# ParaGroup/WindFlow

Measured on NVIDIA H100. Metric: tuples/sec, Map_GPU->Filter_GPU->Ffat_Windows_GPU (CB win 4096 slide 64) pipeline, higher is better.
Workload: dtype i64+f64

## Files before the change

windflow_b200/csrc/wfb_kernels.cuh:

```cuda
#pragma once
#include <type_traits>
#include <cstdint>
#include <cuda.h>
#include <cuda_runtime.h>
#include "wfb_ptx.cuh"
#include "wfb_keys.cuh"

namespace wfb {

template <class P> using key_codec = KeyCodec<typename P::key_t>;
template <class P> using key_words_t = typename key_codec<P>::words_t;
template <class P>
__host__ __device__ __forceinline__ key_words_t<P> key_words(const typename P::tuple_t &t, const typename P::params_t &prm)
{
    return key_codec<P>::encode(P::key(t, prm));
}

constexpr int TILE = 256;
constexpr uint32_t OSW_TILE_POS = 4096;
#ifndef WFB_STAGES
#define WFB_STAGES 4
#endif
constexpr int STAGES = WFB_STAGES;
constexpr uint32_t FULL = 0xffffffffu;

enum { MODE_MAP = 0, MODE_FILTER = 1, MODE_INGEST = 2 };
constexpr uint32_t MAX_SHARDS = 8;

constexpr uint64_t ST_AGG = 1, ST_PREFIX = 2;
__host__ __device__ __forceinline__ uint64_t pack_state(uint32_t epoch, uint64_t status, uint32_t v)
{
    return (static_cast<uint64_t>(epoch & 0x3fffffffu) << 34) | (status << 32) | v;
}

struct DevBatch {
    const unsigned char *tuples;
    const uint64_t *ts;
    unsigned char *out;
    uint64_t *ts_out;
    uint32_t *n_out;
    uint64_t watermark;
    uint32_t n;
    uint32_t tile_begin;
};

struct Trigger { uint64_t key; uint64_t g; uint32_t slot; uint32_t last_pos; uint32_t obase; uint32_t pad; };

struct FfatDev {
    uint64_t *ht_keys;
    uint32_t *ht_slots;
    uint32_t ht_mask;
    uint32_t max_keys;
    uint32_t *n_slots;
    uint32_t *err_flags;
    unsigned long long *results_total;
    uint64_t defer_items;
    uint32_t dense;
    uint32_t grow;
    uint32_t key_div, key_rem;
    uint64_t *slot_key;
    uint64_t *cnt;
    unsigned char *acc;
    unsigned char *tree;
    uint32_t *seg_cnt;
    uint32_t *seg_off;
    struct Trigger *trig;
    uint32_t *n_trig;
    uint32_t trig_cap;
    uint32_t *heavy;
    uint32_t *n_heavy;
    uint32_t light_max;
    uint64_t win, slide, B;
    uint32_t nb;
    uint32_t pane;
    uint32_t wp, sp;
    uint32_t n_leaves;
    uint32_t log_leaves;
    uint32_t lazy;
};
constexpr uint64_t EMPTY_KEY = 0xffffffffffffffffull;
constexpr uint32_t INVALID_SLOT = 0xffffffffu;
constexpr uint32_t KEYS_GROW_FLAG = 8u;

struct TileArgs {
    const DevBatch *batches;
    DevBatch one;
    uint32_t nbatches;
    uint32_t num_tiles;
    uint64_t *tile_state;
    uint32_t *ticket;
    uint32_t ticket_base;
    uint32_t epoch;
    uint64_t tmap_base;
    uint32_t use_tmap;
    uint32_t max_ctas_per_sm;
    uint32_t sparse;
    uint32_t count_keys;
    uint16_t *wide_h16;
    uint32_t tiles_per_ticket;
    uint32_t pack_rank;
    const uint32_t *ext_slots;
    uint32_t inplace;
    uint32_t l2_hints;
    uint32_t nshards, region_cap;
    uint32_t shard_slots, shard_keys;
    uint32_t *shard_err;
    uint32_t *sort_ctl; uint32_t sort_passes, sort_shift, sort_dbits;
    unsigned char *lifted;
    uint32_t *slots;
    uint32_t *batch_off;
    uint32_t *n_total;
    FfatDev ff;
};

template <class T>
struct TileIO {
    static constexpr int TB = sizeof(T);
    static constexpr bool V16 = (TB % 16 == 0) && (TB / 16 == 1 || TB / 16 == 2 || TB / 16 == 4 || TB / 16 == 8);
    static constexpr int C = V16 ? TB / 16 : TB / 8;

    __device__ __forceinline__ static void load(const unsigned char *base, uint32_t idx, T &out)
    {
        if constexpr (V16) {
            uint4 v[C];
            const uint4 *p = reinterpret_cast<const uint4 *>(base + static_cast<size_t>(idx) * TB);
            const uint32_t rot = (C > 1) ? ((idx * C / 8) % C) : 0;
#pragma unroll
            for (int j = 0; j < C; j++) v[j] = p[(j + rot) & (C - 1)];
#pragma unroll
            for (int s = 1; s < C; s <<= 1) {
                if (rot & s) {
                    uint4 t[C];
#pragma unroll
                    for (int k = 0; k < C; k++) t[k] = v[(k - s) & (C - 1)];
#pragma unroll
                    for (int k = 0; k < C; k++) v[k] = t[k];
                }
            }
            uint4 *o = reinterpret_cast<uint4 *>(&out);
#pragma unroll
            for (int k = 0; k < C; k++) o[k] = v[k];
        } else {
            const uint64_t *p = reinterpret_cast<const uint64_t *>(base + static_cast<size_t>(idx) * TB);
            uint64_t *o = reinterpret_cast<uint64_t *>(&out);
#pragma unroll
            for (int k = 0; k < C; k++) o[k] = p[k];
        }
    }

    __device__ __forceinline__ static void store(unsigned char *base, uint32_t idx, const T &in)
    {
        if constexpr (V16) {
            uint4 v[C];
            const uint4 *src = reinterpret_cast<const uint4 *>(&in);
#pragma unroll
            for (int k = 0; k < C; k++) v[k] = src[k];
            const uint32_t rot = (C > 1) ? ((idx * C / 8) % C) : 0;
#pragma unroll
            for (int s = 1; s < C; s <<= 1) {
                if (rot & s) {
                    uint4 t[C];
#pragma unroll
                    for (int k = 0; k < C; k++) t[k] = v[(k + s) & (C - 1)];
#pragma unroll
                    for (int k = 0; k < C; k++) v[k] = t[k];
                }
            }
            uint4 *p = reinterpret_cast<uint4 *>(base + static_cast<size_t>(idx) * TB);
#pragma unroll
            for (int j = 0; j < C; j++) p[(j + rot) & (C - 1)] = v[j];
        } else {
            uint64_t *p = reinterpret_cast<uint64_t *>(base + static_cast<size_t>(idx) * TB);
            const uint64_t *s = reinterpret_cast<const uint64_t *>(&in);
#pragma unroll
            for (int k = 0; k < C; k++) p[k] = s[k];
        }
    }
};

__device__ __forceinline__ bool bulk_ok(const void *g, uint32_t bytes)
{
    return ((reinterpret_cast<uintptr_t>(g) | bytes) & 15u) == 0;
}

__device__ __forceinline__ uint64_t mix64(uint64_t x)
{
    x ^= x >> 33; x *= 0xff51afd7ed558ccdull; x ^= x >> 33; x *= 0xc4ceb9fe1a85ec53ull; x ^= x >> 33;
    return x;
}

template <class P>
__device__ __forceinline__ key_words_t<P> key_of_slot(const FfatDev &ff, uint32_t slot)
{
    if constexpr (key_codec<P>::words == 2) return reinterpret_cast<const Key128 *>(ff.slot_key)[slot];
    else return ff.dense ? (ff.key_div > 1 ? static_cast<uint64_t>(slot) * ff.key_div + ff.key_rem : static_cast<uint64_t>(slot)) : ff.slot_key[slot];
}
__device__ __forceinline__ uint64_t trig_word(uint64_t key) { return key; }
__device__ __forceinline__ uint64_t trig_word(const Key128 &) { return 0; }
template <class P>
__device__ __forceinline__ key_words_t<P> trig_key(const FfatDev &ff, const Trigger &tr)
{
    if constexpr (key_codec<P>::words == 2) return key_of_slot<P>(ff, tr.slot); else return tr.key;
}

__device__ __forceinline__ uint32_t slot_of_key(const FfatDev &ff, const Key128 &key)
{
    if (key.lo == EMPTY_KEY && key.hi == EMPTY_KEY) { atomicOr(ff.err_flags, 1u); return INVALID_SLOT; }
    uint32_t h = static_cast<uint32_t>(mix64(key.lo ^ mix64(key.hi))) & ff.ht_mask;
    for (uint32_t probe = 0; probe <= ff.ht_mask; probe++) {
        uint64_t *e = ff.ht_keys + 2 * static_cast<size_t>(h);
        Key128 k;
        ld_relaxed_v2u64(e, k.lo, k.hi);
        if (k.lo == EMPTY_KEY || k.hi == EMPTY_KEY) {
            atom_cas_b128(e, EMPTY_KEY, EMPTY_KEY, key.lo, key.hi, k.lo, k.hi);
            if (k.lo == EMPTY_KEY && k.hi == EMPTY_KEY) {
                uint32_t s = atomicAdd(ff.n_slots, 1u);
                if (s < ff.max_keys) reinterpret_cast<Key128 *>(ff.slot_key)[s] = key;
                else if (ff.grow) atomicOr(ff.err_flags, KEYS_GROW_FLAG);
                else { atomicOr(ff.err_flags, 1u); s = INVALID_SLOT - 1; }
                st_release_u32(&ff.ht_slots[h], s);
                return s >= ff.max_keys ? INVALID_SLOT : s;
            }
        }
        if (k == key) {
            uint32_t s;
            while ((s = ld_acquire_u32(&ff.ht_slots[h])) == INVALID_SLOT) { }
            if (s >= ff.max_keys) { if (ff.grow) atomicOr(ff.err_flags, KEYS_GROW_FLAG); return INVALID_SLOT; }
            return s;
        }
        h = (h + 1) & ff.ht_mask;
    }
    atomicOr(ff.err_flags, ff.grow ? KEYS_GROW_FLAG : 1u);
    return INVALID_SLOT;
}

__device__ __forceinline__ uint32_t slot_of_key(const FfatDev &ff, uint64_t key)
{
    if (ff.dense) {
        if (ff.key_div > 1) {
            if (key % ff.key_div != ff.key_rem) { atomicOr(ff.err_flags, 1u); return INVALID_SLOT; }
            key /= ff.key_div;
        }
        if (key >= ff.max_keys) { atomicOr(ff.err_flags, 1u); return INVALID_SLOT; }
        return static_cast<uint32_t>(key);
    }
    if (ff.grow && key == EMPTY_KEY) { atomicOr(ff.err_flags, 1u); return INVALID_SLOT; }
    uint32_t h = static_cast<uint32_t>(mix64(key)) & ff.ht_mask;
    for (uint32_t probe = 0; probe <= ff.ht_mask; probe++) {
        uint64_t k = ld_relaxed_u64(&ff.ht_keys[h]);
        if (k == EMPTY_KEY) {
            unsigned long long old = atomicCAS(reinterpret_cast<unsigned long long *>(&ff.ht_keys[h]),
                                               static_cast<unsigned long long>(EMPTY_KEY),
                                               static_cast<unsigned long long>(key));
            if (old == EMPTY_KEY) {
                uint32_t s = atomicAdd(ff.n_slots, 1u);
                if (s < ff.max_keys) ff.slot_key[s] = key;
                else if (ff.grow) atomicOr(ff.err_flags, KEYS_GROW_FLAG);
                else { atomicOr(ff.err_flags, 1u); s = INVALID_SLOT - 1; }
                st_release_u32(&ff.ht_slots[h], s);
                return s >= ff.max_keys ? INVALID_SLOT : s;
            }
            k = old;
        }
        if (k == key) {
            uint32_t s;
            while ((s = ld_acquire_u32(&ff.ht_slots[h])) == INVALID_SLOT) { }
            if (s >= ff.max_keys) { if (ff.grow) atomicOr(ff.err_flags, KEYS_GROW_FLAG); return INVALID_SLOT; }
            return s;
        }
        h = (h + 1) & ff.ht_mask;
    }
    atomicOr(ff.err_flags, ff.grow ? KEYS_GROW_FLAG : 1u);
    return INVALID_SLOT;
}

static __global__ void __launch_bounds__(256) k_key_table_rebuild(const uint64_t *__restrict__ old_keys, const uint32_t *__restrict__ old_slots,
                                                           uint32_t old_mask, uint64_t *new_keys, uint32_t *__restrict__ new_slots, uint32_t new_mask,
                                                           uint64_t *__restrict__ slot_key, uint32_t old_max_keys, uint32_t words, uint32_t *err_flags)
{
    if (blockIdx.x == 0 && threadIdx.x == 0) atomicAnd(err_flags, ~KEYS_GROW_FLAG);
    for (uint32_t i = blockIdx.x * blockDim.x + threadIdx.x; i <= old_mask; i += gridDim.x * blockDim.x) {
        uint32_t h;
        const uint32_t s = old_slots[i];
        if (words == 2) {
            const Key128 k = reinterpret_cast<const Key128 *>(old_keys)[i];
            if (k.lo == EMPTY_KEY && k.hi == EMPTY_KEY) continue;
            h = static_cast<uint32_t>(mix64(k.lo ^ mix64(k.hi))) & new_mask;
            for (;; h = (h + 1) & new_mask) {
                uint64_t lo, hi;
                atom_cas_b128(new_keys + 2 * static_cast<size_t>(h), EMPTY_KEY, EMPTY_KEY, k.lo, k.hi, lo, hi);
                if (lo == EMPTY_KEY && hi == EMPTY_KEY) break;
            }
            if (s >= old_max_keys) reinterpret_cast<Key128 *>(slot_key)[s] = k;
        } else {
            const uint64_t k = old_keys[i];
            if (k == EMPTY_KEY) continue;
            h = static_cast<uint32_t>(mix64(k)) & new_mask;
            while (atomicCAS(reinterpret_cast<unsigned long long *>(&new_keys[h]), static_cast<unsigned long long>(EMPTY_KEY),
                             static_cast<unsigned long long>(k)) != EMPTY_KEY) h = (h + 1) & new_mask;
            if (s >= old_max_keys) slot_key[s] = k;
        }
        new_slots[h] = s;
    }
}

constexpr uint32_t TP_THREADS = TILE + 64;
constexpr uint32_t TILE_SENTINEL = 0x7fffffffu;
enum { TF_SWZ = 1u, TF_FALLBACK = 2u, TF_TS_SMEM = 4u, TF_WIDE_LAST = 8u };

struct StageMeta {
    uint32_t tile, batch, first, cnt, flags, count;
    uint32_t wide, pad;
};

template <class P, int MODE>
struct TilePassSmem {
    using T = typename P::tuple_t;
    using R = typename P::result_t;
    static constexpr uint32_t rec_bytes = (MODE == MODE_INGEST && sizeof(R) > sizeof(T)) ? sizeof(R) : sizeof(T);
    static constexpr uint32_t tile_bytes = (TILE * rec_bytes + 1023u) & ~1023u;
    static constexpr uint32_t aux_bytes = (MODE == MODE_INGEST) ? TILE * 4u : (MODE == MODE_FILTER ? TILE * 16u : 0u);
    static constexpr uint32_t stage_bytes = tile_bytes + aux_bytes;
    static constexpr uint32_t hist_bytes = (MODE == MODE_INGEST) ? 4u * 256u * 4u : 0u;
    static constexpr uint32_t total = STAGES * stage_bytes + 1024  + 1024  + hist_bytes;
};

__device__ __forceinline__ void mbar_arrive(uint64_t *bar)
{
    asm volatile("mbarrier.arrive.shared::cta.b64 _, [%0];" ::"r"(smem_u32(bar)) : "memory");
}
__device__ __forceinline__ void tma_load_2d(void *smem_dst, const void *tmap, int32_t c0, int32_t c1, uint64_t *bar)
{
    asm volatile("cp.async.bulk.tensor.2d.shared::cluster.global.tile.mbarrier::complete_tx::bytes [%0], [%1, {%3, %4}], [%2];"
                 ::"r"(smem_u32(smem_dst)), "l"(tmap), "r"(smem_u32(bar)), "r"(c0), "r"(c1) : "memory");
}
__device__ __forceinline__ void tma_load_2d_hint(void *smem_dst, const void *tmap, int32_t c0, int32_t c1, uint64_t *bar, uint64_t policy)
{
    asm volatile("cp.async.bulk.tensor.2d.shared::cluster.global.tile.mbarrier::complete_tx::bytes.L2::cache_hint [%0], [%1, {%3, %4}], [%2], %5;"
                 ::"r"(smem_u32(smem_dst)), "l"(tmap), "r"(smem_u32(bar)), "r"(c0), "r"(c1), "l"(policy) : "memory");
}
__device__ __forceinline__ void tma_store_2d(const void *tmap, int32_t c0, int32_t c1, const void *smem_src)
{
    asm volatile("cp.async.bulk.tensor.2d.global.shared::cta.tile.bulk_group [%0, {%2, %3}], [%1];"
                 ::"l"(tmap), "r"(smem_u32(smem_src)), "r"(c0), "r"(c1) : "memory");
}
__device__ __forceinline__ void consumer_bar() { asm volatile("bar.sync 1, %0;" ::"n"(TILE) : "memory"); }

template <class P, int MODE>
__global__ void __launch_bounds__(TP_THREADS) k_tile_pass(const __grid_constant__ CUtensorMap tmap, const TileArgs a,
                                                          const __grid_constant__ typename P::params_t prm)
{
    using T = typename P::tuple_t;
    using R = typename P::result_t;
    using SM = TilePassSmem<P, MODE>;
    constexpr uint32_t TB = sizeof(T);
    constexpr uint32_t RB = sizeof(R);
    static_assert(TB % 8 == 0 && RB % 8 == 0, "records must be multiples of 8 bytes");
    constexpr bool CAN_SWZ = (TB == 64);

    extern __shared__ unsigned char smem_raw[];
    unsigned char *smem = reinterpret_cast<unsigned char *>((reinterpret_cast<uintptr_t>(smem_raw) + 1023) & ~static_cast<uintptr_t>(1023));
    unsigned char *ctl = smem + STAGES * SM::stage_bytes;
    uint64_t *full = reinterpret_cast<uint64_t *>(ctl);
    uint64_t *staged = full + STAGES;
    uint64_t *empty = staged + STAGES;
    StageMeta *meta = reinterpret_cast<StageMeta *>(empty + STAGES);
    uint32_t *warp_tot = reinterpret_cast<uint32_t *>(meta + STAGES);
    uint32_t *s_hist = reinterpret_cast<uint32_t *>(ctl + 1024);

    const uint32_t tid = threadIdx.x, lane = tid & 31, warp = tid >> 5;
    auto stage_buf = [&](uint32_t s) { return smem + s * SM::stage_bytes; };
    auto stage_aux = [&](uint32_t s) { return smem + s * SM::stage_bytes + SM::tile_bytes; };

    if (tid == 0) {
        for (int s = 0; s < STAGES; s++) { mbar_init(&full[s], 1); mbar_init(&staged[s], TILE / 32); mbar_init(&empty[s], 1); }
        mbar_fence_init();
    }
    if constexpr (MODE == MODE_INGEST) { for (uint32_t i = tid; i < 4u * 256u; i += TP_THREADS) s_hist[i] = 0; }
    __syncthreads();

    if (warp == 0) {
        if (lane == 0) {
            const uint64_t pol_first = l2_policy_evict_first();
            DevBatch b = a.one; uint32_t bi = 0, b_end = 0;
            bool have_batch = false;
            const uint32_t tpt = a.tiles_per_ticket ? a.tiles_per_ticket : 1u;
            uint32_t t_next = 0, t_end = 0, claim = 0;
            for (uint32_t it = 0;; it++) {
                const uint32_t s = it % STAGES, par = (it / STAGES) & 1u;
                mbar_wait(&empty[s], par ^ 1u);
                StageMeta &m = meta[s];
                if (t_next == t_end) {
                    claim = atomicAdd(a.ticket, 1u) - a.ticket_base;
                    t_next = claim * tpt;
                    if (claim >= (a.num_tiles + tpt - 1) / tpt) { m.tile = TILE_SENTINEL; mbar_arrive(&full[s]); break; }
                    t_end = min(t_next + tpt, a.num_tiles);
                }
                const uint32_t t = t_next++;
                if (a.batches != nullptr && !(have_batch && t >= b.tile_begin && t < b_end)) {
                    uint32_t lo = 0, hi = a.nbatches - 1;
                    while (lo < hi) { const uint32_t mid = (lo + hi + 1) >> 1; if (a.batches[mid].tile_begin <= t) lo = mid; else hi = mid - 1; }
                    bi = lo; b = a.batches[lo];
                    b_end = (lo + 1 < a.nbatches) ? a.batches[lo + 1].tile_begin : a.num_tiles;
                    have_batch = true;
                }
                const uint32_t first = (t - b.tile_begin) * TILE;
                const uint32_t cnt = min(static_cast<uint32_t>(TILE), b.n - first);
                const unsigned char *src = b.tuples + static_cast<size_t>(first) * TB;
                uint32_t flags = 0, tx = 0;
                const uint64_t off = reinterpret_cast<uint64_t>(src) - a.tmap_base;
                if (CAN_SWZ && a.use_tmap && cnt == TILE && (off & 63u) == 0 && (off >> 6) < 0x7fffff00ull) flags = TF_SWZ;
                else if (!bulk_ok(src, cnt * TB)) flags = TF_FALLBACK;
                if (!(flags & TF_FALLBACK)) tx += cnt * TB;
                const uint64_t *tsp = (MODE == MODE_FILTER && b.ts != nullptr) ? b.ts + first : nullptr;
                if (tsp != nullptr && bulk_ok(tsp, cnt * 8u)) { flags |= TF_TS_SMEM; tx += cnt * 8u; }
                if (t_next == t_end) flags |= TF_WIDE_LAST;
                m.tile = t; m.batch = bi; m.first = first; m.cnt = cnt; m.flags = flags; m.wide = claim;
                if (tx) mbar_expect_tx(&full[s], tx); else mbar_arrive(&full[s]);
                if (a.l2_hints) {
                    if (flags & TF_SWZ) tma_load_2d_hint(stage_buf(s), &tmap, 0, static_cast<int32_t>(off >> 6), &full[s], pol_first);
                    else if (!(flags & TF_FALLBACK)) bulk_g2s_hint(stage_buf(s), src, cnt * TB, &full[s], pol_first);
                } else if (flags & TF_SWZ) tma_load_2d(stage_buf(s), &tmap, 0, static_cast<int32_t>(off >> 6), &full[s]);
                else if (!(flags & TF_FALLBACK)) bulk_g2s(stage_buf(s), src, cnt * TB, &full[s]);
                if (flags & TF_TS_SMEM) bulk_g2s(stage_aux(s), tsp, cnt * 8u, &full[s]);
            }
        }
    } else if (warp <= TILE / 32) {
        const uint32_t ctid = tid - 32, cwarp = warp - 1;
        uint32_t wpar = 0;
        for (uint32_t it = 0;; it++) {
            const uint32_t s = it % STAGES, par = (it / STAGES) & 1u;
            unsigned char *buf = stage_buf(s);
            mbar_wait(&full[s], par);
            const StageMeta m = meta[s];
            if (m.tile == TILE_SENTINEL) {
                __syncwarp();
                if (lane == 0) mbar_arrive(&staged[s]);
                if constexpr (MODE == MODE_INGEST) {
                    if (a.sort_ctl != nullptr) {
                        consumer_bar();
                        for (uint32_t i = ctid; i < (a.sort_passes << a.sort_dbits); i += TILE) { const uint32_t c = s_hist[i]; if (c) atomicAdd(&a.sort_ctl[i], c); }
                    }
                }
                break;
            }
            DevBatch b;
            if (a.batches == nullptr) b = a.one; else b = a.batches[m.batch];
            const uint32_t cnt = m.cnt;
            const bool active = ctid < cnt;
            if (m.flags & TF_FALLBACK) {
                const uint64_t *src = reinterpret_cast<const uint64_t *>(b.tuples + static_cast<size_t>(m.first) * TB);
                uint64_t *dst = reinterpret_cast<uint64_t *>(buf);
                for (uint32_t w = ctid; w < cnt * (TB / 8); w += TILE) dst[w] = src[w];
                consumer_bar();
            }
            alignas(16) T tup;
            uint64_t ts = 0;
            bool keep = false;
            if (active) {
                if constexpr (CAN_SWZ) {
                    if (m.flags & TF_SWZ) {
                        const uint4 *p = reinterpret_cast<const uint4 *>(buf + static_cast<size_t>(ctid) * 64);
                        const uint32_t x = (ctid >> 1) & 3u;
                        uint4 *o = reinterpret_cast<uint4 *>(&tup);
#pragma unroll
                        for (uint32_t jj = 0; jj < 4; jj++) o[jj] = p[jj ^ x];
                    } else TileIO<T>::load(buf, ctid, tup);
                } else TileIO<T>::load(buf, ctid, tup);
                if constexpr (MODE == MODE_FILTER) {
                    if (b.ts != nullptr)
                        ts = (m.flags & TF_TS_SMEM) ? reinterpret_cast<const uint64_t *>(stage_aux(s))[ctid] : b.ts[m.first + ctid];
                }
                P::map(tup, prm);
                keep = (MODE == MODE_MAP) ? true : P::filter(tup, prm);
            }
            uint32_t slot = INVALID_SLOT;
            alignas(16) R res;
            if constexpr (MODE == MODE_INGEST) {
                if (keep) {
                    P::lift(tup, res, prm);
                    if (a.nshards && a.shard_slots) {
                        const uint64_t key = key_word0(key_words<P>(tup, prm)), q = key / a.nshards;
                        if (q < a.shard_keys) slot = static_cast<uint32_t>(key - q * a.nshards) * a.shard_slots + static_cast<uint32_t>(q);
                        else atomicOr(a.shard_err, 2u);
                    } else if (a.nshards) slot = static_cast<uint32_t>(key_word0(key_words<P>(tup, prm)) % a.nshards);
                    else {
                        if (a.ext_slots != nullptr) { slot = a.ext_slots[m.tile * TILE + ctid]; if (slot >= a.ff.max_keys) slot = INVALID_SLOT; }
                        else slot = slot_of_key(a.ff, key_words<P>(tup, prm));
                        if (slot != INVALID_SLOT && a.count_keys) atomicAdd(&a.ff.seg_cnt[slot], 1u);
                    }
                    if (a.wide_h16 != nullptr) {
                        if (slot != INVALID_SLOT) {
                            const uint32_t d = (slot >> a.sort_shift) & 1023u;
                            const uint32_t before = atomicAdd(&s_hist[wpar * 512u + (d >> 1)], 1u << ((d & 1u) * 16u));
                            if (a.pack_rank) slot |= ((before >> ((d & 1u) * 16u)) & 0xffffu) << 16;
                        }
                    } else if (a.sort_ctl != nullptr && !(a.sparse && slot == INVALID_SLOT)) {
                        for (uint32_t ps = 0; ps < a.sort_passes; ps++)
                            atomicAdd(&s_hist[(ps << a.sort_dbits) + ((slot >> (a.sort_shift + a.sort_dbits * ps)) & ((1u << a.sort_dbits) - 1u))], 1u);
                    }
                }
            }
            if constexpr (MODE == MODE_MAP) {
                consumer_bar();
                if (active) {
                    if constexpr (CAN_SWZ) {
                        if (m.flags & TF_SWZ) {
                            uint4 *p = reinterpret_cast<uint4 *>(buf + static_cast<size_t>(ctid) * 64);
                            const uint32_t x = (ctid >> 1) & 3u;
                            const uint4 *o = reinterpret_cast<const uint4 *>(&tup);
#pragma unroll
                            for (uint32_t jj = 0; jj < 4; jj++) p[jj ^ x] = o[jj];
                        } else TileIO<T>::store(buf, ctid, tup);
                    } else TileIO<T>::store(buf, ctid, tup);
                }
                if (ctid == 0) meta[s].count = cnt;
            } else {
                const uint32_t bal = __ballot_sync(FULL, keep);
                uint32_t *wt = warp_tot + (it & 1u) * (TILE / 32);
                if (lane == 0) wt[cwarp] = __popc(bal);
                consumer_bar();
                if constexpr (MODE == MODE_INGEST) {
                    if (a.wide_h16 != nullptr && (m.flags & TF_WIDE_LAST)) {
                        uint32_t *hrow = s_hist + wpar * 512u;
                        const uint2 c = reinterpret_cast<const uint2 *>(hrow)[ctid];
                        reinterpret_cast<uint2 *>(hrow)[ctid] = make_uint2(0, 0);
                        reinterpret_cast<uint2 *>(a.wide_h16 + static_cast<size_t>(m.wide) * 1024u)[ctid] = c;
                        wpar ^= 1u;
                    }
                }
                uint32_t wbase = 0, total = 0;
#pragma unroll
                for (uint32_t w = 0; w < TILE / 32; w++) { const uint32_t c = wt[w]; if (w < cwarp) wbase += c; total += c; }
                const uint32_t local = wbase + __popc(bal & lanemask_lt());
                if (ctid == 0) {
                    meta[s].count = total;
                    const uint32_t chain_begin = (MODE == MODE_FILTER) ? b.tile_begin : 0u;
                    if (m.tile != chain_begin && !(MODE == MODE_INGEST && a.sparse)) st_relaxed_u64(&a.tile_state[m.tile], pack_state(a.epoch, ST_AGG, total));
                }
                if (keep) {
                    if constexpr (MODE == MODE_FILTER) {
                        TileIO<T>::store(buf, local, tup);
                        if (b.ts_out != nullptr) reinterpret_cast<uint64_t *>(stage_aux(s) + TILE * 8)[local] = ts;
                    } else if (MODE == MODE_INGEST && a.inplace) {
                        reinterpret_cast<uint32_t *>(stage_aux(s))[ctid] = slot;
                    } else {
                        TileIO<R>::store(buf, local, res);
                        reinterpret_cast<uint32_t *>(stage_aux(s))[local] = slot;
                    }
                } else if (MODE == MODE_INGEST && a.inplace) reinterpret_cast<uint32_t *>(stage_aux(s))[ctid] = INVALID_SLOT;
            }
            fence_async_smem();
            __syncwarp();
            if (lane == 0) mbar_arrive(&staged[s]);
        }
    } else {
        for (uint32_t it = 0;; it++) {
            const uint32_t s = it % STAGES, par = (it / STAGES) & 1u;
            unsigned char *buf = stage_buf(s);
            mbar_wait(&staged[s], par);
            const StageMeta m = meta[s];
            if (m.tile == TILE_SENTINEL) break;
            DevBatch b;
            if (a.batches == nullptr) b = a.one; else b = a.batches[m.batch];
            const uint32_t t = m.tile, tile_count = m.count;
            uint32_t excl = 0;
            if (MODE == MODE_INGEST && a.sparse) {
                excl = t * TILE;
                if (lane == 0 && t == 0 && a.ff.n_trig != nullptr) { *a.ff.n_trig = 0; *a.ff.n_heavy = 0; }
            } else if constexpr (MODE != MODE_MAP) {
                const uint32_t chain_begin = (MODE == MODE_FILTER) ? b.tile_begin : 0u;
                if (t != chain_begin) {
                    int64_t idx = static_cast<int64_t>(t) - 1;
                    while (true) {
                        const int64_t my = idx - lane;
                        uint64_t w = pack_state(a.epoch, ST_PREFIX, 0);
                        bool valid;
                        do {
                            valid = true;
                            if (my >= static_cast<int64_t>(chain_begin)) {
                                w = ld_relaxed_u64(&a.tile_state[my]);
                                valid = ((w >> 34) == (a.epoch & 0x3fffffffu)) && (((w >> 32) & 3u) != 0);
                            }
                        } while (!__all_sync(FULL, valid));
                        const uint32_t status = static_cast<uint32_t>(w >> 32) & 3u;
                        const uint32_t pmask = __ballot_sync(FULL, status == ST_PREFIX);
                        const uint32_t firstp = pmask ? (__ffs(pmask) - 1) : 32;
                        uint32_t v = (lane <= firstp) ? static_cast<uint32_t>(w) : 0u;
#pragma unroll
                        for (int o = 16; o > 0; o >>= 1) v += __shfl_xor_sync(FULL, v, o);
                        excl += v;
                        if (pmask) break;
                        idx -= 32;
                    }
                }
                if (lane == 0) {
                    st_relaxed_u64(&a.tile_state[t], pack_state(a.epoch, ST_PREFIX, excl + tile_count));
                    if constexpr (MODE == MODE_FILTER) {
                        const uint32_t last_tile = b.tile_begin + (b.n + TILE - 1) / TILE - 1;
                        if (t == last_tile && b.n_out != nullptr) *b.n_out = excl + tile_count;
                    } else {
                        if (t == 0) { *a.ff.n_trig = 0; *a.ff.n_heavy = 0; }
                        if (t == b.tile_begin) a.batch_off[m.batch] = excl;
                        if (t == a.num_tiles - 1) { a.batch_off[a.nbatches] = excl + tile_count; *a.n_total = excl + tile_count; }
                    }
                }
            }
            unsigned char *dst;
            uint32_t bytes;
            if constexpr (MODE == MODE_MAP) { dst = b.out + static_cast<size_t>(m.first) * TB; bytes = m.cnt * TB; }
            else if constexpr (MODE == MODE_FILTER) { dst = b.out + static_cast<size_t>(excl) * TB; bytes = tile_count * TB; }
            else { dst = a.lifted + static_cast<size_t>(excl) * RB; bytes = a.inplace ? 0u : tile_count * RB; }
            if (MODE == MODE_MAP && (m.flags & TF_SWZ)) {
                if (lane == 0) tma_store_2d(&tmap, 0, static_cast<int32_t>((reinterpret_cast<uint64_t>(dst) - a.tmap_base) >> 6), buf);
            } else if (bulk_ok(dst, bytes)) {
                if (lane == 0 && bytes) {
                    if ((MODE == MODE_INGEST) && a.l2_hints) bulk_s2g_hint(dst, buf, bytes, l2_policy_evict_last());
                    else bulk_s2g(dst, buf, bytes);
                }
            } else {
                uint64_t *d8 = reinterpret_cast<uint64_t *>(dst);
                const uint64_t *s8 = reinterpret_cast<const uint64_t *>(buf);
                for (uint32_t w = lane; w < bytes / 8; w += 32) d8[w] = s8[w];
            }
            if constexpr (MODE == MODE_FILTER) {
                if (b.ts_out != nullptr) {
                    const uint64_t *sts = reinterpret_cast<const uint64_t *>(stage_aux(s) + TILE * 8);
                    for (uint32_t i = lane; i < tile_count; i += 32) b.ts_out[excl + i] = sts[i];
                }
            }
            if constexpr (MODE == MODE_INGEST) {
                const uint32_t *ssl = reinterpret_cast<const uint32_t *>(stage_aux(s));
                if (a.sparse) for (uint32_t i = lane; i < TILE; i += 32) a.slots[excl + i] = i < (a.inplace ? m.cnt : tile_count) ? ssl[i] : INVALID_SLOT;
                else for (uint32_t i = lane; i < tile_count; i += 32) a.slots[excl + i] = ssl[i];
            }
            __syncwarp();
            if (lane == 0) {
                bulk_commit();
                bulk_wait_read<0>();
                mbar_arrive(&empty[s]);
            }
        }
        if (lane == 0) bulk_wait_all<0>();
    }
}

template <class R>
__device__ __forceinline__ void ld_rec(const unsigned char *p, R &r)
{
    if constexpr (sizeof(R) % 16 == 0) {
        const uint4 *s = reinterpret_cast<const uint4 *>(p);
        uint4 *d = reinterpret_cast<uint4 *>(&r);
#pragma unroll
        for (uint32_t k = 0; k < sizeof(R) / 16; k++) d[k] = s[k];
    } else {
        const uint64_t *s = reinterpret_cast<const uint64_t *>(p);
        uint64_t *d = reinterpret_cast<uint64_t *>(&r);
#pragma unroll
        for (uint32_t k = 0; k < sizeof(R) / 8; k++) d[k] = s[k];
    }
}
template <class R>
__device__ __forceinline__ void st_rec(unsigned char *p, const R &r)
{
    if constexpr (sizeof(R) % 16 == 0) {
        uint4 *d = reinterpret_cast<uint4 *>(p);
        const uint4 *s = reinterpret_cast<const uint4 *>(&r);
#pragma unroll
        for (uint32_t k = 0; k < sizeof(R) / 16; k++) d[k] = s[k];
    } else {
        uint64_t *d = reinterpret_cast<uint64_t *>(p);
        const uint64_t *s = reinterpret_cast<const uint64_t *>(&r);
#pragma unroll
        for (uint32_t k = 0; k < sizeof(R) / 8; k++) d[k] = s[k];
    }
}
template <class R>
__device__ __forceinline__ R shfl_down_rec(const R &r, uint32_t delta)
{
    alignas(16) R o;
    const uint32_t *s = reinterpret_cast<const uint32_t *>(&r);
    uint32_t *d = reinterpret_cast<uint32_t *>(&o);
#pragma unroll
    for (uint32_t k = 0; k < sizeof(R) / 4; k++) d[k] = __shfl_down_sync(FULL, s[k], delta);
    return o;
}
template <class R>
__device__ __forceinline__ R shfl_rec(const R &r, uint32_t src)
{
    alignas(16) R o;
    const uint32_t *s = reinterpret_cast<const uint32_t *>(&r);
    uint32_t *d = reinterpret_cast<uint32_t *>(&o);
#pragma unroll
    for (uint32_t k = 0; k < sizeof(R) / 4; k++) d[k] = __shfl_sync(FULL, s[k], src);
    return o;
}

static __global__ void __launch_bounds__(1024) k_scan_u32(const uint32_t *in, uint32_t *out, uint32_t total, uint32_t *sum_out)
{
    __shared__ uint32_t warp_sums[32];
    const uint32_t tid = threadIdx.x, lane = tid & 31, warp = tid >> 5;
    const uint32_t per = (total + 1023) / 1024;
    const uint32_t begin = min(tid * per, total), end = min(begin + per, total);
    uint32_t sum = 0;
    for (uint32_t i = begin; i < end; i++) sum += in[i];
    uint32_t incl = sum;
#pragma unroll
    for (int o = 1; o < 32; o <<= 1) { const uint32_t v = __shfl_up_sync(FULL, incl, o); if (lane >= o) incl += v; }
    if (lane == 31) warp_sums[warp] = incl;
    __syncthreads();
    if (warp == 0) {
        uint32_t w = warp_sums[lane], wi = w;
#pragma unroll
        for (int o = 1; o < 32; o <<= 1) { const uint32_t v = __shfl_up_sync(FULL, wi, o); if (lane >= o) wi += v; }
        warp_sums[lane] = wi - w;
        if (lane == 31 && sum_out != nullptr) *sum_out = wi;
    }
    __syncthreads();
    uint32_t run = warp_sums[warp] + incl - sum;
    for (uint32_t i = begin; i < end; i++) { const uint32_t v = in[i]; out[i] = run; run += v; }
}


constexpr int OS_THREADS = 256;
constexpr int OS_MAX_PASSES = 8;
constexpr int OS_ITEMS = 8;

template <class K>
__global__ void __launch_bounds__(256) k_radix_ghist(const K *__restrict__ keys, const uint32_t *__restrict__ n_ptr, uint32_t n_host,
                                                     uint32_t passes, uint32_t *__restrict__ ctl, uint32_t base_shift)
{
    __shared__ uint32_t h[OS_MAX_PASSES * 256];
    const uint32_t n = n_ptr ? *n_ptr : n_host;
    for (uint32_t i = threadIdx.x; i < passes * 256; i += blockDim.x) h[i] = 0;
    __syncthreads();
    for (uint32_t i = blockIdx.x * blockDim.x + threadIdx.x; i < n; i += gridDim.x * blockDim.x) {
        const K k = keys[i];
        for (uint32_t p = 0; p < passes; p++) atomicAdd(&h[p * 256 + (static_cast<uint32_t>(k >> (base_shift + 8 * p)) & 255u)], 1u);
    }
    __syncthreads();
    for (uint32_t i = threadIdx.x; i < passes * 256; i += blockDim.x) if (h[i]) atomicAdd(&ctl[i], h[i]);
}

template <class K>
__global__ void __launch_bounds__(OS_THREADS) k_onesweep_pass(const K *__restrict__ keys_in, const uint32_t *__restrict__ vals_in,
                                                              K *__restrict__ keys_out, uint32_t *__restrict__ vals_out,
                                                              const uint32_t *__restrict__ n_ptr, uint32_t n_host, uint32_t pass,
                                                              uint32_t passes, uint32_t *__restrict__ ctl,
                                                              uint64_t *__restrict__ tile_state, uint32_t epoch,
                                                              uint32_t *__restrict__ seg_first, uint32_t seg_first_n,
                                                              uint32_t base_shift)
{
    __shared__ uint32_t cntw[OS_THREADS / 32][256];
    __shared__ uint32_t dig_off[256];
    __shared__ uint32_t bin_base[256];
    __shared__ uint32_t wsum[OS_THREADS / 32];
    __shared__ uint32_t s_tile;
    constexpr int OS_TILE = OS_THREADS * OS_ITEMS;
    __shared__ K skeys[OS_TILE];
    __shared__ uint32_t svals[OS_TILE];

    const uint32_t tid = threadIdx.x, lane = tid & 31, warp = tid >> 5;
    const uint32_t n = n_ptr ? *n_ptr : n_host;
    const uint32_t num_tiles = (n + OS_TILE - 1) / OS_TILE;
    const uint32_t shift = base_shift + 8 * pass;
    if (tid == 0) s_tile = atomicAdd(&ctl[passes * 256 + pass], 1u);
#pragma unroll
    for (int w = 0; w < OS_THREADS / 32; w++) cntw[w][tid] = 0;
    __syncthreads();
    const uint32_t tile = s_tile;
    if (tile >= num_tiles) return;
    const uint32_t start = tile * OS_TILE;

    K k[OS_ITEMS];
    uint32_t rk[OS_ITEMS];
#pragma unroll
    for (int r = 0; r < OS_ITEMS; r++) {
        const uint32_t idx = start + warp * (32 * OS_ITEMS) + r * 32 + lane;
        const bool valid = idx < n;
        k[r] = valid ? keys_in[idx] : K(0);
        const uint32_t d = valid ? (static_cast<uint32_t>(k[r] >> shift) & 255u) : 256u;
        const uint32_t mask = __match_any_sync(FULL, d);
        rk[r] = valid ? (cntw[warp][d] + __popc(mask & lanemask_lt())) : 0u;
        __syncwarp();
        if (valid && lane == static_cast<uint32_t>(__ffs(mask) - 1)) cntw[warp][d] += __popc(mask);
        __syncwarp();
    }
    __syncthreads();

    uint32_t total = 0;
#pragma unroll
    for (int w = 0; w < OS_THREADS / 32; w++) { const uint32_t c = cntw[w][tid]; cntw[w][tid] = total; total += c; }
    uint64_t *my_state = tile_state + static_cast<size_t>(tile) * 256 + tid;
    st_relaxed_u64(my_state, pack_state(epoch, tile == 0 ? ST_PREFIX : ST_AGG, total));
    const uint32_t gcount = ctl[pass * 256 + tid];
    uint32_t incl = gcount;
#pragma unroll
    for (int o = 1; o < 32; o <<= 1) { const uint32_t v = __shfl_up_sync(FULL, incl, o); if (lane >= o) incl += v; }
    if (lane == 31) wsum[warp] = incl;
    uint32_t tincl = total;
#pragma unroll
    for (int o = 1; o < 32; o <<= 1) { const uint32_t v = __shfl_up_sync(FULL, tincl, o); if (lane >= o) tincl += v; }
    __shared__ uint32_t twsum[OS_THREADS / 32];
    if (lane == 31) twsum[warp] = tincl;
    __syncthreads();
    uint32_t gbase = incl - gcount, tbase = tincl - total;
#pragma unroll
    for (uint32_t w = 0; w < OS_THREADS / 32; w++) if (w < warp) { gbase += wsum[w]; tbase += twsum[w]; }
    uint32_t excl = 0;
    if (tile > 0) {
        int64_t t2 = static_cast<int64_t>(tile) - 1;
        bool found = false;
        while (!found) {
            uint64_t w[8];
#pragma unroll
            for (int q = 0; q < 8; q++) w[q] = (t2 - q >= 0) ? ld_relaxed_u64(tile_state + static_cast<size_t>(t2 - q) * 256 + tid) : 0ull;
#pragma unroll
            for (int q = 0; q < 8; q++) {
                if (found || t2 - q < 0) continue;
                if ((w[q] >> 34) != (epoch & 0x3fffffffu) || ((w[q] >> 32) & 3u) == 0) { t2 -= q; goto next_round; }
                excl += static_cast<uint32_t>(w[q]);
                if (((w[q] >> 32) & 3u) == ST_PREFIX) found = true;
            }
            t2 -= 8;
        next_round:;
        }
        st_relaxed_u64(my_state, pack_state(epoch, ST_PREFIX, excl + total));
    }
    dig_off[tid] = tbase;
    bin_base[tid] = gbase + excl;
    __syncthreads();

#pragma unroll
    for (int r = 0; r < OS_ITEMS; r++) {
        const uint32_t idx = start + warp * (32 * OS_ITEMS) + r * 32 + lane;
        if (idx < n) {
            const uint32_t d = static_cast<uint32_t>(k[r] >> shift) & 255u;
            const uint32_t lp = dig_off[d] + cntw[warp][d] + rk[r];
            skeys[lp] = k[r];
            svals[lp] = vals_in ? vals_in[idx] : idx;
        }
    }
    __syncthreads();
    const uint32_t cnt = min(static_cast<uint32_t>(OS_TILE), n - start);
    for (uint32_t i = tid; i < cnt; i += OS_THREADS) {
        const K kk = skeys[i];
        const uint32_t d = static_cast<uint32_t>(kk >> shift) & 255u;
        const uint32_t dst = bin_base[d] + (i - dig_off[d]);
        keys_out[dst] = kk;
        vals_out[dst] = svals[i];
        if (seg_first != nullptr && static_cast<uint64_t>(kk) < seg_first_n) atomicMin(&seg_first[static_cast<uint32_t>(kk)], dst);
    }
}

template <class P>
__global__ void __launch_bounds__(256) k_slots_inplace(const TileArgs a, const typename P::params_t prm)
{
    using T = typename P::tuple_t;
    __shared__ uint32_t s_h[512];
    const uint32_t tid = threadIdx.x;
    const uint32_t npos = a.num_tiles * TILE;
    if (blockIdx.x == 0 && tid == 0 && a.ff.n_trig != nullptr) { *a.ff.n_trig = 0; *a.ff.n_heavy = 0; }
    auto slot_at = [&](uint32_t p) -> uint32_t {
        const uint32_t t = p / TILE;
        uint32_t lo = 0, hi = a.nbatches - 1;
        while (lo < hi) { const uint32_t mid = (lo + hi + 1) >> 1; if (a.batches[mid].tile_begin <= t) lo = mid; else hi = mid - 1; }
        const DevBatch &b = a.batches[lo];
        const uint32_t local = p - b.tile_begin * TILE;
        uint32_t slot = INVALID_SLOT;
        if (local < b.n) {
            if (a.ext_slots != nullptr) { slot = a.ext_slots[p]; if (slot >= a.ff.max_keys) slot = INVALID_SLOT; }
            else {
                const T *rec = reinterpret_cast<const T *>(b.tuples + static_cast<size_t>(local) * sizeof(T));
                slot = slot_of_key(a.ff, key_words<P>(*rec, prm));
            }
            if (slot != INVALID_SLOT && a.count_keys) atomicAdd(&a.ff.seg_cnt[slot], 1u);
        }
        return slot;
    };
    const uint32_t nwide = (npos + OSW_TILE_POS - 1) / OSW_TILE_POS;
    for (uint32_t wt = blockIdx.x; wt < nwide; wt += gridDim.x) {
        for (uint32_t i = tid; i < 512; i += blockDim.x) s_h[i] = 0;
        __syncthreads();
        for (uint32_t p = wt * OSW_TILE_POS + tid; p < min(npos, (wt + 1) * OSW_TILE_POS); p += blockDim.x) {
            uint32_t slot = slot_at(p);
            if (slot != INVALID_SLOT) {
                const uint32_t d = (slot >> a.sort_shift) & 1023u;
                const uint32_t before = atomicAdd(&s_h[d >> 1], 1u << ((d & 1u) * 16u));
                if (a.pack_rank) slot |= ((before >> ((d & 1u) * 16u)) & 0xffffu) << 16;
            }
            a.slots[p] = slot;
        }
        __syncthreads();
        for (uint32_t i = tid; i < 512; i += blockDim.x) reinterpret_cast<uint32_t *>(a.wide_h16 + static_cast<size_t>(wt) * 1024u)[i] = s_h[i];
        __syncthreads();
    }
}

#ifndef WFB_OSW_MINBLOCKS
#define WFB_OSW_MINBLOCKS 5
#endif
constexpr uint32_t OSW_BITS = 10, OSW_DIGITS = 1u << OSW_BITS;
constexpr uint32_t OSW_THREADS = 256, OSW_ITEMS = 16, OSW_TILE = OSW_THREADS * OSW_ITEMS;
static_assert(OSW_TILE == OSW_TILE_POS, "the tile pass files its digit counts per wide tile");

template <class K>
__global__ void __launch_bounds__(OSW_THREADS) k_wide_tile_hist(const K *__restrict__ keys, const uint32_t *__restrict__ n_ptr, uint32_t n_host,
                                                                uint32_t shift, uint32_t chunk_shift, uint16_t *__restrict__ H,
                                                                uint32_t *__restrict__ C, uint32_t *__restrict__ ctl_counts, uint32_t skip_invalid)
{
    static_assert(OSW_THREADS * 4 == OSW_DIGITS, "four digits per thread");
    __shared__ __align__(16) uint32_t h[OSW_DIGITS];
    const uint32_t tid = threadIdx.x, tile = blockIdx.x;
    const uint32_t n = n_ptr ? *n_ptr : n_host;
    const uint32_t start = tile * OSW_TILE;
    if (start >= n) return;
    reinterpret_cast<uint4 *>(h)[tid] = make_uint4(0, 0, 0, 0);
    __syncthreads();
#pragma unroll
    for (uint32_t r = 0; r < OSW_ITEMS; r++) {
        const uint32_t idx = start + r * OSW_THREADS + tid;
        if (idx < n) { const K kk = keys[idx]; if (!(skip_invalid && kk == static_cast<K>(~K(0)))) atomicAdd(&h[static_cast<uint32_t>(kk >> shift) & (OSW_DIGITS - 1u)], 1u); }
    }
    __syncthreads();
    const uint4 c = reinterpret_cast<const uint4 *>(h)[tid];
    reinterpret_cast<ushort4 *>(H + static_cast<size_t>(tile) * OSW_DIGITS)[tid] =
        make_ushort4(static_cast<uint16_t>(c.x), static_cast<uint16_t>(c.y), static_cast<uint16_t>(c.z), static_cast<uint16_t>(c.w));
    uint32_t *crow = C + static_cast<size_t>(tile >> chunk_shift) * OSW_DIGITS + tid * 4;
    if (c.x) atomicAdd(crow + 0, c.x);
    if (c.y) atomicAdd(crow + 1, c.y);
    if (c.z) atomicAdd(crow + 2, c.z);
    if (c.w) atomicAdd(crow + 3, c.w);
    if (ctl_counts != nullptr) {
        if (c.x) atomicAdd(ctl_counts + tid * 4 + 0, c.x);
        if (c.y) atomicAdd(ctl_counts + tid * 4 + 1, c.y);
        if (c.z) atomicAdd(ctl_counts + tid * 4 + 2, c.z);
        if (c.w) atomicAdd(ctl_counts + tid * 4 + 3, c.w);
    }
}

static __global__ void __launch_bounds__(OSW_THREADS) k_wide_chunk_sums16(const uint16_t *__restrict__ H, uint32_t tiles, uint32_t chunk_shift, uint32_t *__restrict__ C,
                                                                          uint32_t *__restrict__ ctl_counts = nullptr)
{
    const uint32_t chunk = blockIdx.x, tid = threadIdx.x;
    const uint32_t t0 = chunk << chunk_shift, t1 = min(tiles, t0 + (1u << chunk_shift));
    uint4 acc = make_uint4(0, 0, 0, 0);
    const ushort4 *row = reinterpret_cast<const ushort4 *>(H) + tid;
#pragma unroll 16
    for (uint32_t t = t0; t < t1; t++) { const ushort4 v = row[static_cast<size_t>(t) * (OSW_DIGITS / 4)]; acc.x += v.x; acc.y += v.y; acc.z += v.z; acc.w += v.w; }
    reinterpret_cast<uint4 *>(C + static_cast<size_t>(chunk) * OSW_DIGITS)[tid] = acc;
    if (ctl_counts != nullptr) {
        if (acc.x) atomicAdd(ctl_counts + tid * 4 + 0, acc.x);
        if (acc.y) atomicAdd(ctl_counts + tid * 4 + 1, acc.y);
        if (acc.z) atomicAdd(ctl_counts + tid * 4 + 2, acc.z);
        if (acc.w) atomicAdd(ctl_counts + tid * 4 + 3, acc.w);
    }
}

static __global__ void __launch_bounds__(OSW_THREADS) k_wide_tile_bases(const uint16_t *__restrict__ H, uint32_t tiles, uint32_t chunk_shift, uint32_t chunks,
                                                                        uint32_t *__restrict__ C, uint32_t *__restrict__ T, uint32_t *__restrict__ ctl_counts,
                                                                        uint32_t *__restrict__ done)
{
    static_assert(OSW_THREADS * 4 == OSW_DIGITS, "four digits per thread");
    constexpr uint32_t NW = OSW_THREADS / 32;
    __shared__ uint32_t wsum[NW];
    __shared__ uint32_t s_last;
    const uint32_t chunk = blockIdx.x, tid = threadIdx.x, lane = tid & 31, warp = tid >> 5;
    const uint32_t t0 = chunk << chunk_shift, t1 = min(tiles, t0 + (1u << chunk_shift));
    uint4 acc = make_uint4(0, 0, 0, 0);
    const ushort4 *row = reinterpret_cast<const ushort4 *>(H) + tid;
    uint4 *trow = reinterpret_cast<uint4 *>(T) + tid;
#pragma unroll 8
    for (uint32_t t = t0; t < t1; t++) {
        const ushort4 v = row[static_cast<size_t>(t) * (OSW_DIGITS / 4)];
        trow[static_cast<size_t>(t) * (OSW_DIGITS / 4)] = acc;
        acc.x += v.x; acc.y += v.y; acc.z += v.z; acc.w += v.w;
    }
    uint4 *C4 = reinterpret_cast<uint4 *>(C);
    C4[static_cast<size_t>(chunk) * (OSW_DIGITS / 4) + tid] = acc;
    __threadfence();
    __syncthreads();
    if (tid == 0) s_last = atomicAdd(done, 1u) == chunks - 1u;
    __syncthreads();
    if (!s_last) return;
    __threadfence();
    uint4 tot = make_uint4(0, 0, 0, 0);
#pragma unroll 8
    for (uint32_t c = 0; c < chunks; c++) { const uint4 v = __ldcg(C4 + static_cast<size_t>(c) * (OSW_DIGITS / 4) + tid); tot.x += v.x; tot.y += v.y; tot.z += v.z; tot.w += v.w; }
    reinterpret_cast<uint4 *>(ctl_counts)[tid] = tot;
    const uint32_t sum = tot.x + tot.y + tot.z + tot.w;
    uint32_t incl = sum;
#pragma unroll
    for (int o = 1; o < 32; o <<= 1) { const uint32_t v = __shfl_up_sync(FULL, incl, o); if (lane >= static_cast<uint32_t>(o)) incl += v; }
    if (lane == 31) wsum[warp] = incl;
    __syncthreads();
    uint32_t base = incl - sum;
#pragma unroll
    for (uint32_t q = 0; q < NW; q++) if (q < warp) base += wsum[q];
    uint4 run = make_uint4(base, base + tot.x, base + tot.x + tot.y, base + tot.x + tot.y + tot.z);
#pragma unroll 8
    for (uint32_t c = 0; c < chunks; c++) {
        uint4 *p = C4 + static_cast<size_t>(c) * (OSW_DIGITS / 4) + tid;
        const uint4 v = __ldcg(p);
        *p = run;
        run.x += v.x; run.y += v.y; run.z += v.z; run.w += v.w;
    }
    if (tid == 0) *done = 0;
}

#ifndef WFB_OSR_MINBLOCKS
#define WFB_OSR_MINBLOCKS 6
#endif
template <int RBYTES>
static __global__ void __launch_bounds__(OSW_THREADS, WFB_OSR_MINBLOCKS) k_wide_scatter_ranked(const uint32_t *__restrict__ packed, uint32_t *__restrict__ keys_out,
                                                                            uint32_t *__restrict__ vals_out, uint32_t n, uint32_t shift, uint32_t chunk_shift,
                                                                            const uint16_t *__restrict__ H, const uint32_t *__restrict__ Cx, const uint32_t *__restrict__ T,
                                                                            const unsigned char *__restrict__ payload_in, unsigned char *__restrict__ payload_out)
{
    constexpr uint32_t NW = OSW_THREADS / 32;
    constexpr uint32_t LPOS = OSW_TILE + OSW_DIGITS;
    constexpr uint32_t LPAD = 0x0fffu;
    static_assert(OSW_TILE <= 4096 && LPOS % (2 * OSW_THREADS) == 0, "16-bit packed position compare");
    __shared__ __align__(16) uint32_t sw[OSW_TILE];
    __shared__ __align__(16) uint32_t bin_base[OSW_DIGITS];
    __shared__ __align__(8) uint16_t cnt_row[OSW_DIGITS], cell_start[OSW_DIGITS];
    __shared__ __align__(4) uint16_t lpos[LPOS];
    __shared__ uint32_t wsum[NW];
    const uint32_t tid = threadIdx.x, lane = tid & 31, warp = tid >> 5, tile = blockIdx.x;
    const uint32_t start = tile * OSW_TILE;
    if (start >= n) return;
#pragma unroll
    for (uint32_t r = 0; r < OSW_ITEMS; r++) {
        const uint32_t i = r * OSW_THREADS + tid, idx = start + i;
        const uint32_t w = idx < n ? packed[idx] : INVALID_SLOT;
        sw[i] = w;
        if constexpr (RBYTES != 0)
            if (w != INVALID_SLOT) asm volatile("prefetch.global.L2 [%0];" ::"l"(payload_in + static_cast<size_t>(idx) * RBYTES));
    }
    {
        const uint4 cb = reinterpret_cast<const uint4 *>(Cx)[static_cast<size_t>(tile >> chunk_shift) * (OSW_DIGITS / 4) + tid];
        const uint4 tb = reinterpret_cast<const uint4 *>(T)[static_cast<size_t>(tile) * (OSW_DIGITS / 4) + tid];
        reinterpret_cast<uint4 *>(bin_base)[tid] = make_uint4(cb.x + tb.x, cb.y + tb.y, cb.z + tb.z, cb.w + tb.w);
        const ushort4 c = reinterpret_cast<const ushort4 *>(H)[static_cast<size_t>(tile) * (OSW_DIGITS / 4) + tid];
        reinterpret_cast<ushort4 *>(cnt_row)[tid] = c;
        const uint32_t p0 = (c.x + 1u) & ~1u, p1 = (c.y + 1u) & ~1u, p2 = (c.z + 1u) & ~1u, p3 = (c.w + 1u) & ~1u;
        const uint32_t sum = p0 + p1 + p2 + p3;
        uint32_t incl = sum;
#pragma unroll
        for (int o = 1; o < 32; o <<= 1) { const uint32_t v = __shfl_up_sync(FULL, incl, o); if (lane >= static_cast<uint32_t>(o)) incl += v; }
        if (lane == 31) wsum[warp] = incl;
#pragma unroll
        for (uint32_t i = 0; i < LPOS / (2 * OSW_THREADS); i++) reinterpret_cast<uint32_t *>(lpos)[i * OSW_THREADS + tid] = LPAD | (LPAD << 16);
        __syncthreads();
        uint32_t base = incl - sum;
#pragma unroll
        for (uint32_t q = 0; q < NW; q++) if (q < warp) base += wsum[q];
        reinterpret_cast<ushort4 *>(cell_start)[tid] = make_ushort4(static_cast<uint16_t>(base), static_cast<uint16_t>(base + p0), static_cast<uint16_t>(base + p0 + p1),
                                                                     static_cast<uint16_t>(base + p0 + p1 + p2));
    }
    __syncthreads();
#pragma unroll
    for (uint32_t r = 0; r < OSW_ITEMS; r++) {
        const uint32_t i = r * OSW_THREADS + tid, w = sw[i];
        if (w != INVALID_SLOT) lpos[cell_start[((w & 0xffffu) >> shift) & (OSW_DIGITS - 1u)] + (w >> 16)] = static_cast<uint16_t>(i);
    }
    __syncthreads();
#pragma unroll 2
    for (uint32_t e = tid; e < LPOS; e += OSW_THREADS) {
        const uint32_t mine = lpos[e], w = sw[mine];
        if (w == INVALID_SLOT) continue;
        const uint32_t slot = w & 0xffffu, d = (slot >> shift) & (OSW_DIGITS - 1u);
        const uint32_t cs = cell_start[d], cnt = cnt_row[d];
        if (e - cs >= cnt) continue;
        const uint32_t mm = (mine | (mine << 16)) + 0x7fff7fffu;
        const uint32_t *cell = reinterpret_cast<const uint32_t *>(lpos + cs);
        uint32_t less = 0;
        for (uint32_t j = 0; j < cnt; j += 2) less += __popc((mm - cell[j >> 1]) & 0x80008000u);
        const uint32_t dst = bin_base[d] + less;
        keys_out[dst] = slot;
        if (RBYTES == 0 || vals_out != nullptr) vals_out[dst] = start + mine;
        if constexpr (RBYTES != 0) {
            static_assert(RBYTES % 8 == 0, "record size");
            using W = typename std::conditional<RBYTES % 16 == 0, uint4, uint2>::type;
            const W *src = reinterpret_cast<const W *>(payload_in + static_cast<size_t>(start + mine) * RBYTES);
            W *dstp = reinterpret_cast<W *>(payload_out + static_cast<size_t>(dst) * RBYTES);
            W v[RBYTES / sizeof(W)];
#pragma unroll
            for (uint32_t q = 0; q < RBYTES / sizeof(W); q++) v[q] = src[q];
#pragma unroll
            for (uint32_t q = 0; q < RBYTES / sizeof(W); q++) dstp[q] = v[q];
        }
    }
}

static __global__ void k_shard_bin_counts(const uint32_t *__restrict__ bin_counts, uint32_t nshards, uint32_t bps, uint32_t *__restrict__ counts_out,
                                          uint64_t *__restrict__ send_meta, uint64_t watermark)
{
    const uint32_t d = threadIdx.x >> 5, lane = threadIdx.x & 31;
    uint32_t c = 0;
    if (d < nshards) for (uint32_t b = lane; b < bps; b += 32) c += bin_counts[d * bps + b];
#pragma unroll
    for (int o = 16; o > 0; o >>= 1) c += __shfl_xor_sync(FULL, c, o);
    if (lane == 0 && d < MAX_SHARDS) counts_out[d] = d < nshards ? c : 0u;
    if (lane == 0 && d < nshards && send_meta != nullptr) { send_meta[2 * d] = c; send_meta[2 * d + 1] = watermark; }
}

struct MgRuns { uint32_t off[MAX_SHARDS + 1]; };
constexpr uint32_t MG_THREADS = 256;
__device__ __forceinline__ uint32_t mg_run_start(const uint32_t *__restrict__ cnt, uint32_t s, uint32_t bps, uint32_t b, uint32_t *sh)
{
    uint32_t c = 0;
    for (uint32_t q = threadIdx.x; q < b; q += MG_THREADS) c += cnt[s * bps + q];
#pragma unroll
    for (int o = 16; o > 0; o >>= 1) c += __shfl_xor_sync(FULL, c, o);
    if ((threadIdx.x & 31) == 0) sh[threadIdx.x >> 5] = c;
    __syncthreads();
    uint32_t t = 0;
#pragma unroll
    for (uint32_t w = 0; w < MG_THREADS / 32; w++) t += sh[w];
    __syncthreads();
    return t;
}
static __global__ void __launch_bounds__(MG_THREADS) k_mg_count(const uint32_t *__restrict__ cnt, uint32_t nsrc, uint32_t bps, const MgRuns runs,
                                                                const uint32_t *__restrict__ recv_slots, uint32_t slot_mask, uint32_t shift2, uint32_t nsub,
                                                                uint32_t *__restrict__ cnt3, uint32_t *__restrict__ run_starts,
                                                                uint32_t *__restrict__ n_trig, uint32_t *__restrict__ n_heavy)
{
    __shared__ uint32_t sh[8], c[MAX_SHARDS];
    const uint32_t b = blockIdx.x, s = blockIdx.y, tid = threadIdx.x, lane = tid & 31;
    if (b == 0 && s == 0 && tid == 0) { *n_trig = 0; *n_heavy = 0; }
    if (tid < MAX_SHARDS) c[tid] = 0;
    const uint32_t rs = mg_run_start(cnt, s, bps, b, sh), m = cnt[s * bps + b];
    if (tid == 0) run_starts[s * bps + b] = rs;
    const uint32_t *sl = recv_slots + runs.off[s] + rs;
    for (uint32_t i0 = 0; i0 < m; i0 += MG_THREADS) {
        const uint32_t i = i0 + tid;
        const uint32_t j = i < m ? ((sl[i] & slot_mask) >> shift2) & (nsub - 1u) : nsub;
        for (uint32_t jj = 0; jj < nsub; jj++) { const uint32_t bal = __ballot_sync(FULL, j == jj); if (lane == 0 && bal) atomicAdd(&c[jj], __popc(bal)); }
    }
    __syncthreads();
    if (tid < nsub) cnt3[(b * nsub + tid) * nsrc + s] = c[tid];
}
static __global__ void __launch_bounds__(1024) k_mg_scan(const uint32_t *__restrict__ cnt3, uint32_t n, uint32_t nsrc, uint32_t *__restrict__ off3,
                                                         uint32_t *__restrict__ digit_counts)
{
    __shared__ uint32_t wsum[32];
    const uint32_t tid = threadIdx.x, lane = tid & 31, warp = tid >> 5;
    const uint32_t per = (n + 1023u) / 1024u, lo = tid * per;
    uint32_t v[MAX_SHARDS], sum = 0;
#pragma unroll
    for (uint32_t q = 0; q < MAX_SHARDS; q++) { v[q] = (q < per && lo + q < n) ? cnt3[lo + q] : 0u; sum += v[q]; }
    uint32_t incl = sum;
#pragma unroll
    for (int o = 1; o < 32; o <<= 1) { const uint32_t x = __shfl_up_sync(FULL, incl, o); if (lane >= static_cast<uint32_t>(o)) incl += x; }
    if (lane == 31) wsum[warp] = incl;
    __syncthreads();
    if (warp == 0) {
        uint32_t w = wsum[lane], wi = w;
#pragma unroll
        for (int o = 1; o < 32; o <<= 1) { const uint32_t x = __shfl_up_sync(FULL, wi, o); if (lane >= static_cast<uint32_t>(o)) wi += x; }
        wsum[lane] = wi - w;
    }
    __syncthreads();
    uint32_t run = wsum[warp] + incl - sum;
#pragma unroll
    for (uint32_t q = 0; q < MAX_SHARDS; q++) if (q < per && lo + q < n) { off3[lo + q] = run; run += v[q]; }
    for (uint32_t d = tid; d * nsrc < n; d += 1024) { uint32_t t = 0; for (uint32_t q = 0; q < nsrc; q++) t += cnt3[d * nsrc + q]; digit_counts[d] = t; }
}
static __global__ void __launch_bounds__(MG_THREADS) k_mg_split(const uint32_t *__restrict__ cnt, uint32_t nsrc, uint32_t bps, const MgRuns runs,
                                                                const uint32_t *__restrict__ recv_slots, uint32_t slot_mask, uint32_t shift2, uint32_t nsub,
                                                                const uint32_t *__restrict__ off3, const uint32_t *__restrict__ run_starts,
                                                                uint32_t *__restrict__ out_slots, uint32_t *__restrict__ out_pos)
{
    __shared__ uint32_t wc[MG_THREADS / 32][MAX_SHARDS], fill[MAX_SHARDS];
    const uint32_t b = blockIdx.x, s = blockIdx.y, tid = threadIdx.x, lane = tid & 31, warp = tid >> 5;
    const uint32_t m = cnt[s * bps + b], src0 = runs.off[s] + run_starts[s * bps + b];
    if (tid < nsub) fill[tid] = off3[(b * nsub + tid) * nsrc + s];
    __syncthreads();
    for (uint32_t i0 = 0; i0 < m; i0 += MG_THREADS) {
        const uint32_t i = i0 + tid;
        uint32_t slot = 0, j = nsub, before = 0;
        if (i < m) { slot = recv_slots[src0 + i] & slot_mask; j = (slot >> shift2) & (nsub - 1u); }
        for (uint32_t jj = 0; jj < nsub; jj++) {
            const uint32_t bal = __ballot_sync(FULL, j == jj);
            if (lane == 0) wc[warp][jj] = __popc(bal);
            if (j == jj) before = __popc(bal & lanemask_lt());
        }
        __syncthreads();
        if (i < m) {
            uint32_t dst = fill[j] + before;
            for (uint32_t w = 0; w < warp; w++) dst += wc[w][j];
            out_slots[dst] = slot; out_pos[dst] = src0 + i;
        }
        __syncthreads();
        if (tid < nsub) { uint32_t t = 0; for (uint32_t w = 0; w < MG_THREADS / 32; w++) t += wc[w][tid]; fill[tid] += t; }
        __syncthreads();
    }
}

template <class K, int RBYTES>
__global__ void __launch_bounds__(OSW_THREADS, WFB_OSW_MINBLOCKS) k_wide_scatter(const K *__restrict__ keys_in, K *__restrict__ keys_out, uint32_t *__restrict__ vals_out,
                                                              const uint32_t *__restrict__ n_ptr, uint32_t n_host, uint32_t shift,
                                                              uint32_t chunk_shift, const uint16_t *__restrict__ H, const uint32_t *__restrict__ C,
                                                              const uint32_t *__restrict__ ctl_counts,
                                                              const unsigned char *__restrict__ payload_in, unsigned char *__restrict__ payload_out,
                                                              uint32_t payload_bytes, uint32_t skip_invalid, uint32_t region_stride)
{
    constexpr uint32_t NW = OSW_THREADS / 32;
    __shared__ __align__(16) uint16_t cntw[NW][OSW_DIGITS];
    __shared__ uint32_t bin_base[OSW_DIGITS];
    __shared__ uint32_t wsum[NW];
    const uint32_t tid = threadIdx.x, lane = tid & 31, warp = tid >> 5, tile = blockIdx.x;
    const uint32_t n = n_ptr ? *n_ptr : n_host;
    const uint32_t start = tile * OSW_TILE;
    if (start >= n) return;
    {
        uint4 *z = reinterpret_cast<uint4 *>(&cntw[0][0]);
        for (uint32_t i = tid; i < NW * OSW_DIGITS / 8; i += OSW_THREADS) z[i] = make_uint4(0, 0, 0, 0);
    }
    uint32_t acc[4] = {0, 0, 0, 0};
    {
        const uint32_t chunk = tile >> chunk_shift;
        const uint4 *crow = reinterpret_cast<const uint4 *>(C) + tid;
#pragma unroll 8
        for (uint32_t c = 0; c < chunk; c++) { const uint4 v = crow[static_cast<size_t>(c) * (OSW_DIGITS / 4)]; acc[0] += v.x; acc[1] += v.y; acc[2] += v.z; acc[3] += v.w; }
        const ushort4 *hrow = reinterpret_cast<const ushort4 *>(H) + tid;
#pragma unroll 16
        for (uint32_t t = chunk << chunk_shift; t < tile; t++) { const ushort4 v = hrow[static_cast<size_t>(t) * (OSW_DIGITS / 4)]; acc[0] += v.x; acc[1] += v.y; acc[2] += v.z; acc[3] += v.w; }
    }
    const uint4 g4 = reinterpret_cast<const uint4 *>(ctl_counts)[tid];
    const uint32_t gsum = g4.x + g4.y + g4.z + g4.w;
// ... 176 lines not shown
        for (; i < n; i += stride) dst[i] = src[i];
    }
    {
        const uint32_t *src = a.slot_src[peer]; uint32_t *dst = a.slot_dst[peer]; const uint32_t n = a.slot_n[peer];
        for (uint32_t i = t; i < n; i += stride) dst[i] = src[i];
    }
    if (part == 0) for (uint32_t i = threadIdx.x; i < a.bin_n; i += MG_PUSH_THREADS) a.bin_dst[peer][i] = a.bin_src[peer][i];
}

static __global__ void k_shard_counts(const uint32_t *__restrict__ digit_counts, uint32_t nshards, uint32_t region_cap, uint32_t *__restrict__ counts_out)
{
    const uint32_t d = threadIdx.x;
    const uint32_t c = d < nshards ? digit_counts[d] : 0u;
    if (d < MAX_SHARDS) counts_out[d] = c;
    const uint32_t over = __ballot_sync(FULL, c > region_cap);
    if (d == 0) counts_out[MAX_SHARDS] = over ? 1u : 0u;
}


__device__ __forceinline__ uint32_t level_off(uint32_t n_leaves, uint32_t level);
__device__ __forceinline__ uint64_t batch_watermark(const uint32_t *__restrict__ batch_off, const DevBatch *__restrict__ batches,
                                                    uint32_t nbatches, uint32_t pos);
template <class P>
__device__ __forceinline__ void ffat_eval_window(const FfatDev &ff, const unsigned char *tree, key_words_t<P> key, uint64_t gwid, uint64_t wm,
                                                 uint32_t opos, unsigned char *__restrict__ out_res, uint64_t *__restrict__ out_ts,
                                                 uint32_t out_cap, const typename P::params_t &prm);

template <class P>
__global__ void __launch_bounds__(128) k_ffat_update_lanes(const FfatDev ff, const unsigned char *__restrict__ lifted,
                                                           const uint32_t *__restrict__ sorted_pos,
                                                           const uint32_t *__restrict__ batch_off, const DevBatch *__restrict__ batches,
                                                           uint32_t nbatches, unsigned char *__restrict__ out_res,
                                                           uint64_t *__restrict__ out_ts, uint32_t out_cap, uint32_t *__restrict__ n_out,
                                                           const typename P::params_t prm)
{
    using R = typename P::result_t;
    constexpr uint32_t RB = sizeof(R);
    constexpr uint32_t U = 4;
    const uint32_t nslots = ff.dense ? ff.max_keys : min(*ff.n_slots, ff.max_keys);
    const uint32_t n = ff.n_leaves, logn = ff.log_leaves;
    const uint64_t P_ = ff.pane;
    const uint64_t group_items = ff.slide * ff.nb;
    const size_t tree_stride = static_cast<size_t>(2 * n - 1) * RB;

    for (uint32_t base = blockIdx.x * blockDim.x; base < nslots; base += gridDim.x * blockDim.x) {
        const uint32_t slot = base + threadIdx.x;
        uint32_t m = (slot < nslots) ? ff.seg_cnt[slot] : 0u;
        if (m > ff.light_max) {
            const uint32_t hi = atomicAdd(ff.n_heavy, 1u);
            if (hi < ff.max_keys) ff.heavy[hi] = slot;
            m = 0;
        }
        const bool act = m > 0;
        uint32_t off = 0; uint64_t c = 0, g = 0, trig = 0;
        key_words_t<P> key{};
        alignas(16) R acc;
        unsigned char *tree = ff.tree + static_cast<size_t>(slot) * tree_stride;
        if (act) {
            off = ff.seg_off[slot]; c = ff.cnt[slot];
            key = key_of_slot<P>(ff, slot);
            if (c % P_ != 0) ld_rec<R>(ff.acc + static_cast<size_t>(slot) * RB, acc);
            g = (c < ff.B) ? 0 : 1 + (c - ff.B) / group_items;
            trig = ff.B + g * group_items;
        }
        uint32_t j = 0;
        while (__any_sync(FULL, act && j < m)) {
            bool completed = false;
            while (act && j < m && !completed) {
                uint32_t p[U];
                alignas(16) R it[U];
                const uint32_t k = min(U, m - j);
#pragma unroll
                for (uint32_t q = 0; q < U; q++) if (q < k) p[q] = sorted_pos[off + j + q];
#pragma unroll
                for (uint32_t q = 0; q < U; q++) if (q < k) ld_rec<R>(lifted + static_cast<size_t>(p[q]) * RB, it[q]);
#pragma unroll
                for (uint32_t q = 0; q < U; q++) {
                    if (q < k && !completed) {
                        if (c % P_ == 0) acc = it[q]; else P::comb(acc, it[q], acc, prm);
                        c++; j++;
                        completed = (c % P_ == 0);
                    }
                }
            }
            if (completed) {
                const uint32_t leaf = static_cast<uint32_t>((c / P_ - 1) & (n - 1));
                const uint32_t plev = ff.lazy ? 0u : logn;
                for (uint32_t l = 0; l < plev; l++)
                    asm volatile("prefetch.global.L2 [%0];" ::"l"(tree + static_cast<size_t>(level_off(n, l) + ((leaf >> l) ^ 1u)) * RB));
                alignas(16) R cur = acc;
                st_rec<R>(tree + static_cast<size_t>(leaf) * RB, cur);
                for (uint32_t l = 0; l < plev; l++) {
                    alignas(16) R s;
                    ld_rec<R>(tree + static_cast<size_t>(level_off(n, l) + ((leaf >> l) ^ 1u)) * RB, s);
                    alignas(16) R parent = cur;
                    if ((leaf >> l) & 1u) P::comb(s, cur, parent, prm); else P::comb(cur, s, parent, prm);
                    cur = parent;
                    st_rec<R>(tree + static_cast<size_t>(level_off(n, l + 1) + (leaf >> (l + 1))) * RB, cur);
                }
                if (c == trig) {
                    const uint32_t last_pos = sorted_pos[off + j - 1];
                    const uint32_t obase = atomicAdd(n_out, ff.nb);
                    bool deferred = (m - j) < ff.defer_items;
                    if (deferred) {
                        const uint32_t ti = atomicAdd(ff.n_trig, 1u);
                        if (ti < ff.trig_cap) { Trigger tr; tr.key = trig_word(key); tr.g = g; tr.slot = slot; tr.last_pos = last_pos; tr.obase = obase; tr.pad = 0; ff.trig[ti] = tr; }
                        else deferred = false;
                    }
                    if (!deferred) {
                        const uint64_t wm = batch_watermark(batch_off, batches, nbatches, last_pos);
                        for (uint32_t i = 0; i < ff.nb; i++)
                            ffat_eval_window<P>(ff, tree, key, g * ff.nb + i, wm, obase + i, out_res, out_ts, out_cap, prm);
                    }
                    g++; trig += group_items;
                }
            }
        }
        if (act) {
            ff.cnt[slot] = c;
            if (c % P_ != 0) st_rec<R>(ff.acc + static_cast<size_t>(slot) * RB, acc);
            ff.seg_cnt[slot] = 0;
            ff.seg_off[slot] = 0xffffffffu;
        }
    }
}

#ifdef WFB_BK_TRACE
__device__ unsigned long long g_bk_trace[1024 * 8];
__device__ __forceinline__ unsigned long long bk_now() { unsigned long long t; asm volatile("mov.u64 %0, %%globaltimer;" : "=l"(t)); return t; }
#define BK_TRACE_STATE unsigned long long bk_t = 0
#define BK_MARK(i) do { if (threadIdx.x == 0) { const unsigned long long t_ = bk_now(); unsigned long long *r_ = g_bk_trace + blockIdx.x * 8; \
    if ((i) == 0) { r_[0] = t_; for (int q_ = 1; q_ < 8; q_++) r_[q_] = 0; } else if ((i) == 7) r_[7] = t_; else r_[i] += t_ - bk_t; bk_t = t_; } } while (0)
#else
#define BK_TRACE_STATE do { } while (0)
#define BK_MARK(i) do { } while (0)
#endif
constexpr uint32_t BK_KEYS = 64;
constexpr uint32_t BK_THREADS = 128;
#ifndef WFB_BK_REC_BYTES
#define WFB_BK_REC_BYTES 16384
#endif
constexpr uint32_t BK_REC_BYTES = WFB_BK_REC_BYTES;
constexpr uint32_t BK_CNT_U = 16;
__device__ __forceinline__ uint32_t bk_opaque(uint32_t v) { asm volatile("" : "+r"(v)); return v; }
template <uint32_t RB>
constexpr uint32_t bk_items_per_thread() { return BK_REC_BYTES / (BK_THREADS * RB) < 1 ? 1 : (BK_REC_BYTES / (BK_THREADS * RB) > 8 ? 8 : BK_REC_BYTES / (BK_THREADS * RB)); }
#ifndef WFB_BK_MINBLOCKS
#define WFB_BK_MINBLOCKS 4
#endif
#ifndef WFB_BK_MINBLOCKS_LAZY
#define WFB_BK_MINBLOCKS_LAZY 4
#endif

template <class P, bool LAZY>
__global__ void __launch_bounds__(BK_THREADS, LAZY ? WFB_BK_MINBLOCKS_LAZY : WFB_BK_MINBLOCKS) k_ffat_update_buckets(const FfatDev ff, const unsigned char *__restrict__ lifted,
                                                                       const uint32_t *__restrict__ bk_slots, const uint32_t *__restrict__ bk_pos,
                                                                       const uint32_t *__restrict__ digit_counts, uint32_t shift, uint32_t moved,
                                                                       const uint32_t *__restrict__ batch_off, const DevBatch *__restrict__ batches,
                                                                       uint32_t nbatches, unsigned char *__restrict__ out_res,
                                                                       uint64_t *__restrict__ out_ts, uint32_t out_cap, uint32_t *__restrict__ n_out,
                                                                       const typename P::params_t prm)
{
    using R = typename P::result_t;
    constexpr uint32_t RB = sizeof(R);
    constexpr uint32_t NW = BK_THREADS / 32;
    constexpr uint32_t DPT = OSW_DIGITS / BK_THREADS;
    constexpr uint32_t IT = bk_items_per_thread<RB>();
    constexpr uint32_t CAP = BK_THREADS * IT;
    constexpr uint32_t NCOL = IT * NW;
    constexpr uint32_t CS = NCOL + 2;
    constexpr uint32_t CPB = (RB % 16 == 0) ? 16 : 8;
    constexpr uint32_t BK_SIBL = RB <= 32 ? 8 : (RB <= 48 ? 4 : (RB <= 128 ? 2 : 1));
    static_assert(DPT % 4 == 0 && BK_KEYS == 64 && BK_THREADS == 128 && RB % 8 == 0, "layout");
    __shared__ __align__(16) unsigned char s_rec[CAP * RB];
    __shared__ uint32_t s_idx[CAP];
    __shared__ uint32_t s_lslot[CAP], s_lpos[CAP];
    __shared__ __align__(16) uint16_t s_col[BK_KEYS][CS];
    __shared__ uint32_t kcnt[BK_KEYS], koff[BK_KEYS];
    __shared__ uint32_t kleft[BK_KEYS];
    __shared__ uint32_t kcp[BK_KEYS], kleaf[BK_KEYS];
    __shared__ uint64_t kc[BK_KEYS], kg[BK_KEYS], ktt[BK_KEYS];
    __shared__ __align__(16) unsigned char kacc[BK_KEYS * RB];
    __shared__ __align__(16) unsigned char s_sib[LAZY ? 16 : BK_KEYS * BK_SIBL * RB];
    __shared__ uint32_t s_heavy[BK_KEYS];
    __shared__ uint32_t ksegb[BK_KEYS];
    __shared__ uint32_t seg_desc[BK_THREADS];
    __shared__ uint32_t misc[NW], s_boff[2], s_nheavy, s_hnext, s_nseg;

    const uint32_t tid = threadIdx.x, lane = tid & 31, warp = tid >> 5;
    const uint32_t bucket = blockIdx.x;
    const uint32_t kpc = min(BK_KEYS, 1u << shift);
    const uint32_t key_lo = bucket << shift;
    const uint32_t n = ff.n_leaves, logn = ff.log_leaves;
    const uint32_t P32 = static_cast<uint32_t>(ff.pane);
    const uint64_t group_items = ff.slide * ff.nb;
    const size_t tree_stride = static_cast<size_t>(2 * n - 1) * RB;
    BK_TRACE_STATE;

    BK_MARK(0);
    uint32_t my_total = 0;
    uint64_t st_c = 0;
    const bool has_key = tid < kpc && key_lo + tid < ff.max_keys;
    if (has_key) {
        const uint32_t slot = key_lo + tid;
        st_c = ff.cnt[slot];
#pragma unroll
        for (uint32_t q = 0; q < RB / CPB; q++) cp_async<CPB>(kacc + tid * RB + q * CPB, ff.acc + static_cast<size_t>(slot) * RB + q * CPB);
    }
    if (tid < BK_KEYS) kleft[tid] = 0;
    {
        uint32_t cc[DPT];
#pragma unroll
        for (uint32_t q = 0; q < DPT / 4; q++) {
            const uint4 v = reinterpret_cast<const uint4 *>(digit_counts)[tid * (DPT / 4) + q];
            cc[4 * q] = v.x; cc[4 * q + 1] = v.y; cc[4 * q + 2] = v.z; cc[4 * q + 3] = v.w;
        }
        uint32_t sum = 0;
#pragma unroll
        for (uint32_t q = 0; q < DPT; q++) sum += cc[q];
        uint32_t incl = sum;
#pragma unroll
        for (int o = 1; o < 32; o <<= 1) { const uint32_t v = __shfl_up_sync(FULL, incl, o); if (lane >= static_cast<uint32_t>(o)) incl += v; }
        if (lane == 31) misc[warp] = incl;
        __syncthreads();
        if (tid == bucket / DPT) {
            uint32_t base = incl - sum;
            for (uint32_t w = 0; w < warp; w++) base += misc[w];
            for (uint32_t q = bucket - bucket % DPT; q < bucket; q++) base += digit_counts[q];
            s_boff[0] = base; s_boff[1] = base + digit_counts[bucket];
        }
        __syncthreads();
    }
    const uint32_t bbeg = s_boff[0], bend = s_boff[1];
    const auto fetch_list = [&](uint32_t at, uint32_t end) {
#pragma unroll
        for (uint32_t r = 0; r < IT; r++) {
            const uint32_t i = r * BK_THREADS + tid;
            if (at + i < end) {
                cp_async<4>(s_lslot + i, bk_slots + at + i);
                if (!moved) cp_async<4>(s_lpos + i, bk_pos + at + i);
            }
        }
    };
    fetch_list(bbeg, bend);
    for (uint32_t base = bbeg; base < bend; base += BK_CNT_U * BK_THREADS) {
        uint32_t lk[BK_CNT_U];
#pragma unroll
        for (uint32_t q = 0; q < BK_CNT_U; q++) {
            const uint32_t i = base + q * BK_THREADS + tid;
            lk[q] = i < bend ? bk_slots[i] - key_lo : 0xffffffffu;
        }
#pragma unroll
        for (uint32_t q = 0; q < BK_CNT_U; q++) if (lk[q] < kpc) atomicAdd(&kleft[lk[q]], 1u);
    }
    __syncthreads();
    if (tid < BK_KEYS) {
        const uint32_t m = has_key ? kleft[tid] : 0u;
        my_total = m;
        const uint64_t c = st_c;
        uint64_t g = 0, tt = 0; uint32_t cp = 0, leaf = 0;
        if (m) {
            cp = static_cast<uint32_t>(c % P32); leaf = static_cast<uint32_t>((c / P32) & (n - 1));
            if (c < ff.B) { g = 0; tt = ff.B - c; }
            else { g = 1 + (c - ff.B) / group_items; tt = ff.B + g * group_items - c; }
        }
        kleft[tid] = m; kc[tid] = c; kg[tid] = g; ktt[tid] = tt; kcp[tid] = cp; kleaf[tid] = leaf;
    }
    const uint32_t any_items = __syncthreads_or(my_total != 0);
    BK_MARK(1);
    if (!any_items) { cp_async_wait_all(); BK_MARK(7); return; }
    if (moved)
        for (size_t o = static_cast<size_t>(tid) * 128; o < static_cast<size_t>(bend - bbeg) * RB; o += BK_THREADS * 128)
            asm volatile("prefetch.global.L2 [%0];" ::"l"(lifted + static_cast<size_t>(bbeg) * RB + o));

    for (uint32_t cursor = s_boff[0]; cursor < s_boff[1]; cursor = s_boff[0]) {
        const uint32_t nsel = min(CAP, s_boff[1] - cursor);
        uint32_t ek[IT], ep[IT];
        cp_async_wait_all();
#pragma unroll
        for (uint32_t r = 0; r < IT; r++) {
            const uint32_t i = r * BK_THREADS + tid;
            ek[r] = BK_KEYS; ep[r] = cursor + i;
            if (i < nsel) {
                const uint32_t lk = s_lslot[i] - key_lo;
                if (!moved) ep[r] = s_lpos[i];
                if (lk < kpc) ek[r] = lk;
            }
        }
        {
            uint32_t *z = reinterpret_cast<uint32_t *>(&s_col[0][0]);
            for (uint32_t i = tid; i < BK_KEYS * CS / 2; i += BK_THREADS) z[i] = 0;
        }
        __syncthreads();
        fetch_list(cursor + CAP, s_boff[1]);
#pragma unroll
        for (uint32_t r = 0; r < IT; r++) {
            const uint32_t k = ek[r];
            const uint32_t peers = __match_any_sync(FULL, k);
            const uint32_t rank = __popc(peers & lanemask_lt());
            if (k < BK_KEYS && rank == 0) s_col[k][r * NW + warp] = static_cast<uint16_t>(__popc(peers));
            ek[r] = k | rank << 8;
        }
        __syncthreads();
        BK_MARK(2);
        if (warp == 0) {
            uint32_t a0 = 0, a1 = 0;
#pragma unroll
            for (uint32_t c = 0; c < NCOL; c++) {
                const uint32_t v0 = s_col[lane][c], v1 = s_col[lane + 32][c];
                s_col[lane][c] = static_cast<uint16_t>(a0); s_col[lane + 32][c] = static_cast<uint16_t>(a1);
                a0 += v0; a1 += v1;
            }
            uint32_t i0 = a0, i1 = a1;
#pragma unroll
            for (int o = 1; o < 32; o <<= 1) {
                const uint32_t v0 = __shfl_up_sync(FULL, i0, o), v1 = __shfl_up_sync(FULL, i1, o);
                if (lane >= static_cast<uint32_t>(o)) { i0 += v0; i1 += v1; }
            }
            const uint32_t t0 = __shfl_sync(FULL, i0, 31);
            kcnt[lane] = a0; kcnt[lane + 32] = a1;
            koff[lane] = i0 - a0; koff[lane + 32] = t0 + i1 - a1;
            const uint32_t c0 = kcp[lane], c1 = kcp[lane + 32];
            const uint32_t f0 = min(a0, P32 - c0), f1 = min(a1, P32 - c1);
            const uint32_t n0 = a0 ? 1u + (a0 - f0 + P32 - 1) / P32 : 0u, n1 = a1 ? 1u + (a1 - f1 + P32 - 1) / P32 : 0u;
            uint32_t s0 = n0, s1 = n1;
#pragma unroll
            for (int o = 1; o < 32; o <<= 1) {
                const uint32_t v0 = __shfl_up_sync(FULL, s0, o), v1 = __shfl_up_sync(FULL, s1, o);
                if (lane >= static_cast<uint32_t>(o)) { s0 += v0; s1 += v1; }
            }
            const uint32_t st0 = __shfl_sync(FULL, s0, 31), nseg = st0 + __shfl_sync(FULL, s1, 31);
            ksegb[lane] = s0 - n0; ksegb[lane + 32] = st0 + s1 - n1;
            const bool fallback = nseg > BK_THREADS;
            const bool h0 = fallback && a0 != 0, h1 = fallback && a1 != 0;
            const uint32_t b0 = __ballot_sync(FULL, h0), b1 = __ballot_sync(FULL, h1);
            if (h0) s_heavy[__popc(b0 & lanemask_lt())] = lane;
            if (h1) s_heavy[__popc(b0) + __popc(b1 & lanemask_lt())] = lane + 32;
            if (lane == 0) { s_nheavy = __popc(b0) + __popc(b1); s_hnext = 0; s_nseg = fallback ? 0u : nseg; }
        }
        __syncthreads();
#pragma unroll
        for (uint32_t r = 0; r < IT; r++) {
            const uint32_t k = ek[r] & 255u;
            if (k < BK_KEYS) {
                const uint32_t at = koff[k] + s_col[k][r * NW + warp] + (ek[r] >> 8);
                s_idx[at] = ep[r];
                const unsigned char *src = lifted + static_cast<size_t>(ep[r]) * RB;
#pragma unroll
                for (uint32_t q = 0; q < RB / CPB; q++) {
                    if constexpr (CPB == 16) cp_async_cg16(s_rec + at * RB + q * CPB, src + q * CPB);
                    else cp_async<CPB>(s_rec + at * RB + q * CPB, src + q * CPB);
                }
            }
        }
        const uint32_t nseg = s_nseg;
        bool sib_staged = false;
        if (tid < BK_KEYS && nseg != 0) {
            const uint32_t m = kcnt[tid];
            if (m != 0) {
                const uint32_t cp0 = kcp[tid], first = min(m, P32 - cp0), ns = 1u + (m - first + P32 - 1) / P32, sb = ksegb[tid];
                for (uint32_t j = 0; j < ns; j++) seg_desc[sb + j] = tid | (j << 8);
                if (!LAZY && cp0 + first == P32) {
                    const uint32_t leaf = kleaf[tid];
                    const unsigned char *tr = ff.tree + static_cast<size_t>(key_lo + tid) * tree_stride;
                    for (uint32_t l = 0; l < min(logn, BK_SIBL); l++) {
                        const unsigned char *src = tr + static_cast<size_t>(level_off(n, l) + ((leaf >> l) ^ 1u)) * RB;
                        unsigned char *dst = s_sib + (tid * BK_SIBL + l) * RB;
#pragma unroll
                        for (uint32_t q = 0; q < RB / CPB; q++) cp_async<CPB>(dst + q * CPB, src + q * CPB);
                    }
                    sib_staged = true;
                }
            }
        }
        cp_async_wait_all();
        __syncthreads();
        BK_MARK(3);
        if (tid < nseg) {
            const uint32_t d = seg_desc[tid], k = d & 255u, j = d >> 8;
            const uint32_t m = kcnt[k], cp0 = kcp[k], first = min(m, P32 - cp0);
            const uint32_t start = j == 0 ? 0u : first + (j - 1) * P32;
            const uint32_t seg = j == 0 ? first : min(P32, m - start);
            unsigned char *rp = s_rec + (koff[k] + start) * RB;
            alignas(16) R acc;
            uint32_t i = 1;
            if (j == 0 && cp0 != 0) { ld_rec<R>(kacc + k * RB, acc); i = 0; }
            else ld_rec<R>(rp, acc);
#pragma unroll 4
            for (; i < seg; i++) { alignas(16) R it; ld_rec<R>(rp + i * RB, it); P::comb(acc, it, acc, prm); }
            st_rec<R>(rp, acc);
        }
        __syncthreads();
        BK_MARK(4);
        if (tid < BK_KEYS && nseg != 0) {
            const uint32_t k = bk_opaque(tid), m = kcnt[k];
            const uint32_t cp0 = kcp[k];
            uint32_t leafi = kleaf[k], new_cp = cp0, consumed = 0;
            uint64_t g = kg[k], tt = ktt[k];
            while (__any_sync(FULL, consumed < m)) {
                bool eval_now = false;
                uint32_t ev_obase = 0, ev_pos = 0;
                uint64_t ev_g = 0;
                if (consumed < m) {
                    const uint32_t open = consumed == 0 ? cp0 : 0u;
                    const uint32_t len = min(m - consumed, P32 - open);
                    alignas(16) R cur;
                    ld_rec<R>(s_rec + (koff[k] + consumed) * RB, cur);
                    consumed += len;
                    const bool completes = open + len == P32;
                    if (!completes) { st_rec<R>(kacc + k * RB, cur); new_cp = open + len; }
                    else {
                        new_cp = 0;
                        const uint32_t slot = key_lo + k, leaf = leafi;
                        unsigned char *tree = ff.tree + static_cast<size_t>(slot) * tree_stride;
                        leafi = (leafi + 1) & (n - 1);
                        st_rec<R>(tree + static_cast<size_t>(leaf) * RB, cur);
                        for (uint32_t l0 = 0; l0 < (LAZY ? 0u : logn); l0 += 4) {
                            alignas(16) R sbl[4];
#pragma unroll
                            for (uint32_t q = 0; q < 4; q++) {
                                const uint32_t l = l0 + q;
                                if (l < logn) {
                                    if (sib_staged && l < BK_SIBL) ld_rec<R>(s_sib + (k * BK_SIBL + l) * RB, sbl[q]);
                                    else ld_rec<R>(tree + static_cast<size_t>(level_off(n, l) + ((leaf >> l) ^ 1u)) * RB, sbl[q]);
                                }
                            }
#pragma unroll
                            for (uint32_t q = 0; q < 4; q++) {
                                const uint32_t l = l0 + q;
                                if (l < logn) {
                                    alignas(16) R parent = cur;
                                    if ((leaf >> l) & 1u) P::comb(sbl[q], cur, parent, prm); else P::comb(cur, sbl[q], parent, prm);
                                    cur = parent;
                                    st_rec<R>(tree + static_cast<size_t>(level_off(n, l + 1) + (leaf >> (l + 1))) * RB, cur);
                                }
                            }
                        }
                        sib_staged = false;
// ... 1208 lines not shown
```

windflow_b200/csrc/wfb_launch.cuh:

```cuda
#pragma once
#include <type_traits>
#include <algorithm>
#include <cstring>
#include <cuda.h>
#include <cuda_runtime.h>
#include "../../include/wfb200.h"
#include "wfb_kernels.cuh"

#define WFB_CK(call) do { cudaError_t e__ = (call); if (e__ != cudaSuccess) return static_cast<int>(e__); } while (0)

namespace wfb {

inline int num_sms()
{
    static int n = 0;
    if (n == 0) { int dev = 0; if (cudaGetDevice(&dev) == cudaSuccess) cudaDeviceGetAttribute(&n, cudaDevAttrMultiProcessorCount, dev); }
    return n;
}


typedef CUresult (*PFN_encodeTiled)(CUtensorMap *, CUtensorMapDataType, cuuint32_t, void *, const cuuint64_t *, const cuuint64_t *,
                                    const cuuint32_t *, const cuuint32_t *, CUtensorMapInterleave, CUtensorMapSwizzle,
                                    CUtensorMapL2promotion, CUtensorMapFloatOOBfill);
inline PFN_encodeTiled get_encode_tiled()
{
    static PFN_encodeTiled fn = nullptr;
    static bool tried = false;
    if (!tried) {
        tried = true;
        void *p = nullptr;
        cudaDriverEntryPointQueryResult q;
        if (cudaGetDriverEntryPoint("cuTensorMapEncodeTiled", &p, cudaEnableDefault, &q) == cudaSuccess && q == cudaDriverEntryPointSuccess)
            fn = reinterpret_cast<PFN_encodeTiled>(p);
        cudaGetLastError();
    }
    return fn;
}

inline bool make_tuple_tmap(CUtensorMap *m, uint64_t base, uint64_t end)
{
    std::memset(m, 0, sizeof(*m));
    PFN_encodeTiled enc = get_encode_tiled();
    if (!enc || (base & 63u) || end <= base) return false;
    const uint64_t rows = (end - base) / 64;
    if (rows == 0 || rows > 0xffffffffull) return false;
    cuuint64_t gdim[2] = {64, rows};
    cuuint64_t gstr[1] = {64};
    cuuint32_t box[2] = {64, TILE};
    cuuint32_t estr[2] = {1, 1};
    return enc(m, CU_TENSOR_MAP_DATA_TYPE_UINT8, 2, reinterpret_cast<void *>(base), gdim, gstr, box, estr, CU_TENSOR_MAP_INTERLEAVE_NONE,
               CU_TENSOR_MAP_SWIZZLE_64B, CU_TENSOR_MAP_L2_PROMOTION_L2_128B, CU_TENSOR_MAP_FLOAT_OOB_FILL_NONE) == CUDA_SUCCESS;
}

struct ProgramOps {
    uint32_t tuple_bytes, result_bytes, params_bytes, reserved;
    int (*tile_pass)(int mode, TileArgs &a, const void *params, uint32_t want_grid, cudaStream_t s, uint32_t *grid_used,
                     uint64_t span_begin, uint64_t span_end);
    int (*ffat_update)(const FfatDev &ff, const unsigned char *lifted, const uint32_t *sorted_pos, const uint32_t *batch_off,
                       const DevBatch *batches, uint32_t nbatches, unsigned char *out_res, uint64_t *out_ts,
                       uint32_t out_cap, uint32_t *n_out, uint32_t grid, cudaStream_t s, const void *params, uint32_t lanes_grid);
    int (*ffat_buckets)(const FfatDev &ff, const unsigned char *lifted, const uint32_t *bk_slots, const uint32_t *bk_pos,
                        const uint32_t *digit_counts, uint32_t shift, uint32_t moved, const uint32_t *batch_off, const DevBatch *batches,
                        uint32_t nbatches, unsigned char *out_res, uint64_t *out_ts, uint32_t out_cap, uint32_t *n_out, cudaStream_t s,
                        const void *params);
    int (*ffat_windows)(const FfatDev &ff, const uint32_t *batch_off, const DevBatch *batches, uint32_t nbatches,
                        unsigned char *out_res, uint64_t *out_ts, uint32_t out_cap, uint32_t grid, cudaStream_t s, const void *params, uint32_t *n_out);
    int (*extract_keys)(const unsigned char *tuples, uint32_t n, uint64_t *keys, uint32_t *dest, uint32_t num_shards, cudaStream_t s,
                        const void *params);
    int (*reduce_segments)(const unsigned char *tuples, const uint64_t *ts, const uint32_t *sidx, const uint32_t *seg_begin,
                           const uint32_t *n_keys, unsigned char *out_tuples, uint64_t *out_ts, uint32_t n, cudaStream_t s, const void *params);
    int (*reduce_all)(const unsigned char *tuples, const uint64_t *ts, uint32_t n, unsigned char *out_tuple, uint64_t *out_ts, cudaStream_t s,
                      const void *params);
    int (*gather)(const unsigned char *tuples, const uint64_t *ts, const uint32_t *perm, uint32_t n, unsigned char *out_tuples,
                  uint64_t *out_ts, cudaStream_t s);
    int (*tb_lift)(const unsigned char *tuples, const uint64_t *ts, uint32_t n, const FfatDev &ff, const TbDev &tb, uint64_t first_incomplete,
                   unsigned char *lifted, uint64_t *ckeys, cudaStream_t s, const void *params);
    int (*tb_reduce)(const unsigned char *lifted, const uint64_t *skeys, const uint32_t *sidx, const uint32_t *seg_begin, const uint32_t *n_segs,
                     unsigned char *part, uint32_t n, uint32_t kbits, uint32_t max_keys, cudaStream_t s, const void *params);
    int (*tb_merge)(const uint64_t *skeys, const uint32_t *seg_begin, const uint32_t *n_segs, const unsigned char *part, const FfatDev &ff,
                    const TbDev &tb, uint32_t n, cudaStream_t s, const void *params);
    int (*tb_pop_write)(const FfatDev &ff, const TbDev &tb, uint64_t first_incomplete, const uint32_t *offs, unsigned char *popped,
                        uint32_t *popped_slots, uint32_t popped_cap, uint32_t max_present, cudaStream_t s, const void *params);
    const void *(*lifted_ops)();
    int (*slots_inplace)(const TileArgs &a, const void *params, cudaStream_t s);
    uint32_t state_bytes, reserved2;
    int (*ks_slots)(const DevBatch *batches, const uint32_t *boff, uint32_t nb, uint32_t total, const FfatDev &ff, uint32_t *slots, cudaStream_t s,
                    const void *params);
    int (*ks_apply)(int filter, const FfatDev &ff, const DevBatch *batches, const uint32_t *boff, uint32_t nb, const uint32_t *bk_slots,
                    const uint32_t *bk_pos, const uint32_t *digit_counts, uint32_t shift, unsigned char *states, unsigned char *keep, cudaStream_t s,
                    const void *params);
    int (*ks_apply_runs)(int filter, const FfatDev &ff, const DevBatch *batches, const uint32_t *boff, uint32_t nb, uint32_t n,
                         const uint32_t *sorted_slots, const uint32_t *sorted_pos, unsigned char *states, unsigned char *keep, cudaStream_t s,
                         const void *params);
    int (*flag_scatter)(const unsigned char *keep, const uint32_t *tile_base, const uint32_t *boff, uint32_t nb, uint32_t n,
                        const uint32_t *rank_start, const DevBatch *batches, cudaStream_t s);
    int (*extract_keys_batches)(const DevBatch *batches, const uint32_t *boff, uint32_t nb, uint32_t total, uint32_t key_bits, uint64_t *keys,
                                cudaStream_t s, const void *params);
    int (*reduce_segments_batches)(const DevBatch *batches, const uint32_t *boff, const uint64_t *skeys, const uint32_t *sidx,
                                   const uint32_t *seg_begin, const uint32_t *first_seg, const uint32_t *n_segs, uint32_t key_bits,
                                   uint32_t total, uint32_t *long_list, uint32_t *n_long, cudaStream_t s, const void *params);
    uint32_t key_bytes, key_kind, key_size;
    int (*key_order_words)(const DevBatch *batches, const uint32_t *boff, uint32_t nb, const unsigned char *tuples, uint32_t total, uint64_t *lo,
                           uint64_t *hi, cudaStream_t s, const void *params);
};

template <class P, class = void> struct program_passthrough : std::false_type {};
template <class P> struct program_passthrough<P, std::void_t<decltype(P::passthrough)>> : std::integral_constant<bool, P::passthrough && std::is_same<typename P::tuple_t, typename P::result_t>::value> {};

template <class P>
inline typename P::params_t load_params(const void *params)
{
    typename P::params_t prm;
    if (params) std::memcpy(&prm, params, sizeof(prm)); else std::memset(&prm, 0, sizeof(prm));
    return prm;
}

template <class P, int MODE>
int launch_tile_pass(TileArgs &a, const void *params, uint32_t want_grid, cudaStream_t s, uint32_t *grid_used,
                     uint64_t span_begin, uint64_t span_end)
{
    static int max_grid = -1;
    constexpr uint32_t smem = TilePassSmem<P, MODE>::total;
    if (max_grid < 0) {
        WFB_CK(cudaFuncSetAttribute(k_tile_pass<P, MODE>, cudaFuncAttributeMaxDynamicSharedMemorySize, static_cast<int>(smem)));
        int per_sm = 0;
        WFB_CK(cudaOccupancyMaxActiveBlocksPerMultiprocessor(&per_sm, k_tile_pass<P, MODE>, TP_THREADS, smem));
        if (per_sm < 1) per_sm = 1;
        max_grid = per_sm * wfb::num_sms();
    }
    uint32_t grid = std::max(1u, std::min(want_grid, static_cast<uint32_t>(max_grid)));
    if (a.max_ctas_per_sm) grid = std::max(1u, std::min(grid, a.max_ctas_per_sm * static_cast<uint32_t>(wfb::num_sms())));
    const typename P::params_t prm = load_params<P>(params);
    alignas(64) CUtensorMap tmap;
    a.use_tmap = 0; a.tmap_base = span_begin;
    if (sizeof(typename P::tuple_t) == 64 && make_tuple_tmap(&tmap, span_begin, span_end)) a.use_tmap = 1;
    else std::memset(&tmap, 0, sizeof(tmap));
    k_tile_pass<P, MODE><<<grid, TP_THREADS, smem, s>>>(tmap, a, prm);
    WFB_CK(cudaGetLastError());
    *grid_used = grid;
    return 0;
}

template <class P>
int tile_pass_dispatch(int mode, TileArgs &a, const void *params, uint32_t want_grid, cudaStream_t s, uint32_t *grid_used,
                       uint64_t span_begin, uint64_t span_end)
{
    switch (mode) {
    case MODE_MAP: return launch_tile_pass<P, MODE_MAP>(a, params, want_grid, s, grid_used, span_begin, span_end);
    case MODE_FILTER: return launch_tile_pass<P, MODE_FILTER>(a, params, want_grid, s, grid_used, span_begin, span_end);
    case MODE_INGEST: return launch_tile_pass<P, MODE_INGEST>(a, params, want_grid, s, grid_used, span_begin, span_end);
    }
    return WFB_E_BADARG;
}

template <class P>
int ffat_update_dispatch(const FfatDev &ff, const unsigned char *lifted, const uint32_t *sorted_pos, const uint32_t *batch_off,
                         const DevBatch *batches, uint32_t nbatches, unsigned char *out_res, uint64_t *out_ts,
                         uint32_t out_cap, uint32_t *n_out, uint32_t grid, cudaStream_t s, const void *params, uint32_t lanes_grid)
{
    const typename P::params_t prm = load_params<P>(params);
    k_ffat_update_lanes<P><<<lanes_grid, 128, 0, s>>>(ff, lifted, sorted_pos, batch_off, batches, nbatches, out_res, out_ts, out_cap, n_out, prm);
    k_ffat_update<P><<<std::max(1u, std::min(grid, static_cast<uint32_t>(wfb::num_sms()) * 2u)), 256, 0, s>>>(
        ff, lifted, sorted_pos, batch_off, batches, nbatches, out_res, out_ts, out_cap, n_out, prm);
    WFB_CK(cudaGetLastError());
    return 0;
}

template <class P>
int ffat_buckets_dispatch(const FfatDev &ff, const unsigned char *lifted, const uint32_t *bk_slots, const uint32_t *bk_pos,
                          const uint32_t *digit_counts, uint32_t shift, uint32_t moved, const uint32_t *batch_off, const DevBatch *batches,
                          uint32_t nbatches, unsigned char *out_res, uint64_t *out_ts, uint32_t out_cap, uint32_t *n_out, cudaStream_t s,
                          const void *params)
{
    if (ff.lazy) k_ffat_update_buckets<P, true><<<OSW_DIGITS, BK_THREADS, 0, s>>>(ff, lifted, bk_slots, bk_pos, digit_counts, shift, moved, batch_off, batches,
                                                                                 nbatches, out_res, out_ts, out_cap, n_out, load_params<P>(params));
    else k_ffat_update_buckets<P, false><<<OSW_DIGITS, BK_THREADS, 0, s>>>(ff, lifted, bk_slots, bk_pos, digit_counts, shift, moved, batch_off, batches,
                                                                          nbatches, out_res, out_ts, out_cap, n_out, load_params<P>(params));
    WFB_CK(cudaGetLastError());
    return 0;
}

template <class P>
int ffat_windows_dispatch(const FfatDev &ff, const uint32_t *batch_off, const DevBatch *batches, uint32_t nbatches,
                          unsigned char *out_res, uint64_t *out_ts, uint32_t out_cap, uint32_t grid, cudaStream_t s, const void *params, uint32_t *n_out)
{
    if (ff.lazy) {
        const size_t per_warp = static_cast<size_t>(2) * ff.n_leaves * sizeof(typename P::result_t);
        const uint32_t wpb = static_cast<uint32_t>(std::max<size_t>(1, std::min<size_t>(4, (32u << 10) / per_warp)));
        k_ffat_windows_lazy<P><<<grid, 32 * wpb, wpb * per_warp, s>>>(ff, batch_off, batches, nbatches, out_res, out_ts, out_cap, load_params<P>(params), n_out);
    } else
    k_ffat_windows<P><<<grid, 256, 0, s>>>(ff, batch_off, batches, nbatches, out_res, out_ts, out_cap, load_params<P>(params), n_out);
    WFB_CK(cudaGetLastError());
    return 0;
}

inline uint32_t grid_for(uint32_t n, uint32_t per_block) { return std::max(1u, std::min((n + per_block - 1) / per_block, static_cast<uint32_t>(wfb::num_sms()) * 16u)); }

template <class P>
int extract_keys_dispatch(const unsigned char *tuples, uint32_t n, uint64_t *keys, uint32_t *dest, uint32_t num_shards, cudaStream_t s,
                          const void *params)
{
    k_extract_keys<P><<<grid_for(n, 256), 256, 0, s>>>(tuples, n, keys, dest, num_shards, load_params<P>(params));
    WFB_CK(cudaGetLastError());
    return 0;
}
template <class P>
int reduce_segments_dispatch(const unsigned char *tuples, const uint64_t *ts, const uint32_t *sidx, const uint32_t *seg_begin,
                             const uint32_t *n_keys, unsigned char *out_tuples, uint64_t *out_ts, uint32_t n, cudaStream_t s,
                             const void *params)
{
    k_reduce_segments<P><<<grid_for(n, 8), 256, 0, s>>>(tuples, ts, sidx, seg_begin, n_keys, out_tuples, out_ts, load_params<P>(params));
    WFB_CK(cudaGetLastError());
    return 0;
}
template <class P>
int slots_inplace_dispatch(const TileArgs &a, const void *params, cudaStream_t s)
{
    const uint32_t npos = a.num_tiles * TILE;
    k_slots_inplace<P><<<std::max(1u, std::min((npos + 2047u) / 2048u, static_cast<uint32_t>(wfb::num_sms()) * 8u)), 256, 0, s>>>(a, load_params<P>(params));
    WFB_CK(cudaGetLastError());
    return 0;
}

template <class P, class = void> struct program_has_state : std::false_type {};
template <class P> struct program_has_state<P, std::void_t<typename P::state_t>> : std::true_type {};

template <class P>
int ks_slots_dispatch(const DevBatch *batches, const uint32_t *boff, uint32_t nb, uint32_t total, const FfatDev &ff, uint32_t *slots, cudaStream_t s,
                      const void *params)
{
    k_ks_slots<P><<<grid_for(total, 256), 256, 0, s>>>(batches, boff, nb, total, ff, slots, load_params<P>(params));
    WFB_CK(cudaGetLastError());
    return 0;
}
template <class P>
int ks_apply_dispatch(int filter, const FfatDev &ff, const DevBatch *batches, const uint32_t *boff, uint32_t nb, const uint32_t *bk_slots,
                      const uint32_t *bk_pos, const uint32_t *digit_counts, uint32_t shift, unsigned char *states, unsigned char *keep, cudaStream_t s,
                      const void *params)
{
    if constexpr (program_has_state<P>::value) {
        if (filter) k_ks_apply<P, true><<<OSW_DIGITS, KS_THREADS, 0, s>>>(ff, batches, boff, nb, bk_slots, bk_pos, digit_counts, shift, states, keep, load_params<P>(params));
        else k_ks_apply<P, false><<<OSW_DIGITS, KS_THREADS, 0, s>>>(ff, batches, boff, nb, bk_slots, bk_pos, digit_counts, shift, states, keep, load_params<P>(params));
        WFB_CK(cudaGetLastError());
        return 0;
    } else return WFB_E_UNSUPPORTED;
}
template <class P>
int ks_apply_runs_dispatch(int filter, const FfatDev &ff, const DevBatch *batches, const uint32_t *boff, uint32_t nb, uint32_t n,
                           const uint32_t *sorted_slots, const uint32_t *sorted_pos, unsigned char *states, unsigned char *keep, cudaStream_t s,
                           const void *params)
{
    if constexpr (program_has_state<P>::value) {
        if (filter) k_ks_apply_runs<P, true><<<grid_for(n, 256), 256, 0, s>>>(ff, batches, boff, nb, n, sorted_slots, sorted_pos, states, keep, load_params<P>(params));
        else k_ks_apply_runs<P, false><<<grid_for(n, 256), 256, 0, s>>>(ff, batches, boff, nb, n, sorted_slots, sorted_pos, states, keep, load_params<P>(params));
        WFB_CK(cudaGetLastError());
        return 0;
    } else return WFB_E_UNSUPPORTED;
}
template <class P>
int flag_scatter_dispatch(const unsigned char *keep, const uint32_t *tile_base, const uint32_t *boff, uint32_t nb, uint32_t n,
                          const uint32_t *rank_start, const DevBatch *batches, cudaStream_t s)
{
    k_flag_scatter<P><<<(n + SEGT - 1) / SEGT, 256, 0, s>>>(keep, tile_base, boff, nb, n, rank_start, batches);
    WFB_CK(cudaGetLastError());
    return 0;
}
template <class P> constexpr uint32_t program_state_bytes() { if constexpr (program_has_state<P>::value) return sizeof(typename P::state_t); else return 0; }

template <class P>
int tb_lift_dispatch(const unsigned char *tuples, const uint64_t *ts, uint32_t n, const FfatDev &ff, const TbDev &tb, uint64_t first_incomplete,
                     unsigned char *lifted, uint64_t *ckeys, cudaStream_t s, const void *params)
{
    k_tb_lift<P><<<grid_for(n, 256), 256, 0, s>>>(tuples, ts, n, ff, tb, first_incomplete, lifted, ckeys, load_params<P>(params));
    WFB_CK(cudaGetLastError());
    return 0;
}
template <class P>
int tb_reduce_dispatch(const unsigned char *lifted, const uint64_t *skeys, const uint32_t *sidx, const uint32_t *seg_begin, const uint32_t *n_segs,
                       unsigned char *part, uint32_t n, uint32_t kbits, uint32_t max_keys, cudaStream_t s, const void *params)
{
    k_tb_reduce<P><<<grid_for(n, 128), 128, 0, s>>>(lifted, skeys, sidx, seg_begin, n_segs, part, kbits, max_keys, load_params<P>(params));
    WFB_CK(cudaGetLastError());
    return 0;
}
template <class P>
int tb_merge_dispatch(const uint64_t *skeys, const uint32_t *seg_begin, const uint32_t *n_segs, const unsigned char *part, const FfatDev &ff,
                      const TbDev &tb, uint32_t n, cudaStream_t s, const void *params)
{
    k_tb_merge<P><<<grid_for(n, 128), 128, 0, s>>>(skeys, seg_begin, n_segs, part, ff, tb, load_params<P>(params));
    WFB_CK(cudaGetLastError());
    return 0;
}
template <class P>
int tb_pop_write_dispatch(const FfatDev &ff, const TbDev &tb, uint64_t first_incomplete, const uint32_t *offs, unsigned char *popped,
                          uint32_t *popped_slots, uint32_t popped_cap, uint32_t max_present, cudaStream_t s, const void *params)
{
    k_tb_pop_write<P><<<grid_for(max_present, 128), 128, 0, s>>>(ff, tb, first_incomplete, offs, popped, popped_slots, popped_cap, load_params<P>(params));
    WFB_CK(cudaGetLastError());
    return 0;
}
template <class P>
int extract_keys_batches_dispatch(const DevBatch *batches, const uint32_t *boff, uint32_t nb, uint32_t total, uint32_t key_bits, uint64_t *keys,
                                  cudaStream_t s, const void *params)
{
    k_extract_keys_batches<P><<<grid_for(total, 256), 256, 0, s>>>(batches, boff, nb, total, key_bits, keys, load_params<P>(params));
    WFB_CK(cudaGetLastError());
    return 0;
}
template <class P>
int key_order_words_dispatch(const DevBatch *batches, const uint32_t *boff, uint32_t nb, const unsigned char *tuples, uint32_t total, uint64_t *lo,
                             uint64_t *hi, cudaStream_t s, const void *params)
{
    k_key_order_words<P><<<grid_for(total, 256), 256, 0, s>>>(batches, boff, nb, tuples, total, lo, hi, load_params<P>(params));
    WFB_CK(cudaGetLastError());
    return 0;
}
template <class P>
int reduce_segments_batches_dispatch(const DevBatch *batches, const uint32_t *boff, const uint64_t *skeys, const uint32_t *sidx,
                                     const uint32_t *seg_begin, const uint32_t *first_seg, const uint32_t *n_segs, uint32_t key_bits,
                                     uint32_t total, uint32_t *long_list, uint32_t *n_long, cudaStream_t s, const void *params)
{
    k_reduce_segments_batches_short<P><<<grid_for(total, 128), 128, 0, s>>>(batches, boff, skeys, sidx, seg_begin, first_seg, n_segs, key_bits,
                                                                            long_list, n_long, load_params<P>(params));
    k_reduce_segments_batches<P><<<std::max(1u, std::min(grid_for(total / RB_LONG + 1, 8), static_cast<uint32_t>(wfb::num_sms()) * 8u)), 256, 0, s>>>(
        batches, boff, skeys, sidx, seg_begin, first_seg, n_segs, key_bits, long_list, n_long, load_params<P>(params));
    WFB_CK(cudaGetLastError());
    return 0;
}
template <class P>
int reduce_all_dispatch(const unsigned char *tuples, const uint64_t *ts, uint32_t n, unsigned char *out_tuple, uint64_t *out_ts, cudaStream_t s,
// ... 99 lines not shown
```

windflow_b200/csrc/wfb_lib.cu:

```cuda
#include <cstdio>
#include <cstdlib>
#include <cstring>
#include <ctime>
#include <mutex>
#include <vector>
#include <algorithm>
#include <new>
#include <cuda.h>
#include <cuda_runtime.h>
#include "../../include/wfb200.h"
#include "wfb_kernels.cuh"
#include "wfb_launch.cuh"
#include "wfb_programs.cuh"

using namespace wfb;

#define CK(call) do { cudaError_t e__ = (call); if (e__ != cudaSuccess) return static_cast<int>(e__); } while (0)

namespace {

int g_num_sms = 0;

int device_ready()
{
// ... 286 lines not shown
    }
    int64_t grown_bytes() const { int64_t d = 0; for (const Array &a : arrays) if (a.counted) d += static_cast<int64_t>(a.bytes) - static_cast<int64_t>(a.old_bytes); return d; }
    int alloc()
    {
        for (Array &a : arrays)
            if (cudaMalloc(&a.fresh, a.bytes) != cudaSuccess) { cudaGetLastError(); release(); return WFB_E_CAPACITY; }
        return 0;
    }
    void release() { for (Array &a : arrays) { cudaFree(a.fresh); a.fresh = nullptr; } }
    int fill(cudaStream_t s)
    {
        for (Array &a : arrays) {
            const size_t keep = a.copy ? a.old_bytes : 0;
            if (keep) CK(cudaMemcpyAsync(a.fresh, *a.ptr, keep, cudaMemcpyDeviceToDevice, s));
            if (a.fill >= 0 && a.bytes > keep) CK(cudaMemsetAsync(static_cast<unsigned char *>(a.fresh) + keep, a.fill, a.bytes - keep, s));
        }
        return 0;
    }
    void commit() { for (Array &a : arrays) { cudaFree(*a.ptr); *a.ptr = a.fresh; a.fresh = nullptr; } }
};

struct GrowCheck {
    uint32_t *host = nullptr; cudaEvent_t ev = nullptr;
    int init() { CK(cudaMallocHost(reinterpret_cast<void **>(&host), 2 * sizeof(uint32_t))); CK(cudaEventCreateWithFlags(&ev, cudaEventDisableTiming)); return 0; }
    void destroy() { if (host) cudaFreeHost(host); if (ev) cudaEventDestroy(ev); host = nullptr; ev = nullptr; }
};

template <class AddState, class Derive>
int grow_keys(FfatDev &ff, uint32_t key_bytes, GrowCheck &gc, uint32_t ceiling, uint32_t limit, cudaStream_t s, bool *grew, AddState add_state,
              Derive derive)
{
    *grew = false;
    CK(cudaMemcpyAsync(gc.host, ff.n_slots, 2 * sizeof(uint32_t), cudaMemcpyDeviceToHost, s));
    CK(cudaEventRecord(gc.ev, s));
    CK(cudaEventSynchronize(gc.ev));
    if (!(gc.host[1] & KEYS_GROW_FLAG)) return 0;
    const uint32_t old = ff.max_keys;
    uint64_t cap = 1; while (cap < 2ull * std::max(gc.host[0], old)) cap <<= 1;
    if (cap > ceiling && old < ceiling && gc.host[0] <= ceiling) cap = ceiling;
    if (cap > limit) return WFB_E_CAPACITY;
    uint64_t entries = 1; while (entries < 2 * cap) entries <<= 1;
    GrowPlan plan;
    plan.add(ff.ht_keys, static_cast<size_t>(key_bytes) * (ff.ht_mask + 1ull), key_bytes * entries, false, 0xff);
    plan.add(ff.ht_slots, sizeof(uint32_t) * (ff.ht_mask + 1ull), sizeof(uint32_t) * entries, false, 0xff);
    plan.add(ff.slot_key, static_cast<size_t>(key_bytes) * old, static_cast<size_t>(key_bytes) * cap, true, -1);
    int rc = add_state(plan, static_cast<uint32_t>(cap)); if (rc) return rc;
    rc = plan.alloc(); if (rc) return rc;
    rc = plan.fill(s);
    if (!rc) {
        k_key_table_rebuild<<<grid_for(ff.ht_mask + 1, 256), 256, 0, s>>>(ff.ht_keys, ff.ht_slots, ff.ht_mask, plan.fresh(ff.ht_keys), plan.fresh(ff.ht_slots),
                                                                        static_cast<uint32_t>(entries - 1), plan.fresh(ff.slot_key), old, key_bytes / 8, ff.err_flags);
        rc = static_cast<int>(cudaGetLastError());
    }
    if (!rc) rc = static_cast<int>(cudaStreamSynchronize(s));
    if (rc) { cudaStreamSynchronize(s); plan.release(); return rc; }
    plan.commit();
    ff.ht_mask = static_cast<uint32_t>(entries - 1); ff.max_keys = static_cast<uint32_t>(cap);
    rc = derive(static_cast<uint32_t>(cap), plan); if (rc) return rc;
    *grew = true;
    return 0;
}

}

struct wfb_engine {
    int prog = 0;
    const ProgramOps *ops = nullptr;
    std::vector<unsigned char> params;
    const void *pp() const { return params.empty() ? nullptr : params.data(); }
    TileScratch ts;
    uint64_t launches = 0;
    uint32_t key_bits = 64;
    uint32_t cap = 0;
    uint64_t *keysA = nullptr, *keysB = nullptr;
    uint32_t *idxA = nullptr, *idxB = nullptr, *destA = nullptr, *destB = nullptr;
    uint32_t *head = nullptr, *seg_begin = nullptr;
    unsigned char *sh_lifted = nullptr; uint32_t *sh_dest = nullptr, *sh_ctl = nullptr; uint64_t sh_cap = 0;
    uint32_t *rb_off = nullptr, *rb_first = nullptr, *rb_total = nullptr; uint32_t rb_cap = 0;
    uint32_t *rb_long = nullptr; uint32_t rb_long_cap = 0;
    RadixSorter sorter;
    uint64_t *wlo = nullptr, *whi = nullptr; uint32_t *wperm = nullptr; uint32_t wcap = 0;

    int ensure_sort(uint32_t n, cudaStream_t s)
    {
        if (n <= cap) return 0;
        CK(cudaStreamSynchronize(s));
        cudaFree(keysA); cudaFree(keysB); cudaFree(idxA); cudaFree(idxB); cudaFree(destA); cudaFree(destB);
        cudaFree(head); cudaFree(seg_begin);
        cap = std::max(n, 2 * cap);
        CK(cudaMalloc(&keysA, sizeof(uint64_t) * cap)); CK(cudaMalloc(&keysB, sizeof(uint64_t) * cap));
        CK(cudaMalloc(&idxA, sizeof(uint32_t) * cap)); CK(cudaMalloc(&idxB, sizeof(uint32_t) * cap));
        CK(cudaMalloc(&destA, sizeof(uint32_t) * cap)); CK(cudaMalloc(&destB, sizeof(uint32_t) * cap));
        CK(cudaMalloc(&head, sizeof(uint32_t) * cap)); CK(cudaMalloc(&seg_begin, sizeof(uint32_t) * (static_cast<size_t>(cap) + 1)));
        return 0;
    }
    int sort64(uint32_t n, uint32_t bits, cudaStream_t s, const uint64_t **skeys, const uint32_t **sidx)
    {
        const uint64_t before = sorter.launches;
        int rc = sorter.sort<uint64_t>(keysA, keysB, idxA, idxB, nullptr, n, n, (bits + 7) / 8, s, skeys, sidx);
        launches += sorter.launches - before;
        return rc;
    }
    int rank_keys(const DevBatch *batches, const uint32_t *boff, uint32_t nb, const void *tuples, uint32_t n, cudaStream_t s)
    {
        const bool two = ops->key_bytes == 16;
        const uint32_t bits = 8u * ops->key_size, lo_bits = std::min(bits, 64u), hi_bits = two ? bits - 64u : 0u;
        if (n > wcap) {
            CK(cudaStreamSynchronize(s));
            cudaFree(wlo); cudaFree(whi); cudaFree(wperm); wlo = whi = nullptr; wperm = nullptr;
            wcap = std::max(n, cap);
            CK(cudaMalloc(&wlo, sizeof(uint64_t) * wcap));
            if (two) { CK(cudaMalloc(&whi, sizeof(uint64_t) * wcap)); CK(cudaMalloc(&wperm, sizeof(uint32_t) * wcap)); }
        }
        int rc = ops->key_order_words(batches, boff, nb, static_cast<const unsigned char *>(tuples), n, wlo, whi, s, pp()); if (rc) return rc;
        CK(cudaMemcpyAsync(keysA, wlo, sizeof(uint64_t) * n, cudaMemcpyDeviceToDevice, s));
        const uint64_t *sk; const uint32_t *perm;
        rc = sort64(n, lo_bits, s, &sk, &perm); if (rc) return rc;
        const uint32_t g = grid_for(n, 256);
        if (two) {
            CK(cudaMemcpyAsync(wperm, perm, sizeof(uint32_t) * n, cudaMemcpyDeviceToDevice, s));
            k_gather_u64<<<g, 256, 0, s>>>(whi, wperm, n, keysA);
            const uint32_t *p2;
            rc = sort64(n, hi_bits, s, &sk, &p2); if (rc) return rc;
            k_compose_perm<<<g, 256, 0, s>>>(wperm, p2, n, destA);
            perm = destA;
            launches += 2;
        }
        k_rank_heads<<<g, 256, 0, s>>>(wlo, whi, perm, n, head);
        k_scan_u32<<<1, 1024, 0, s>>>(head, head, n, nullptr);
        k_rank_scatter<<<g, 256, 0, s>>>(wlo, whi, perm, head, n, boff, nb, keysA);
        CK(cudaGetLastError());
        launches += 4;
        return 0;
    }
    void free_sort()
    {
        cudaFree(keysA); cudaFree(keysB); cudaFree(idxA); cudaFree(idxB); cudaFree(destA); cudaFree(destB);
        cudaFree(head); cudaFree(seg_begin);
        cudaFree(sh_lifted); cudaFree(sh_dest); cudaFree(sh_ctl);
        cudaFree(rb_off); cudaFree(rb_first); cudaFree(rb_total); cudaFree(rb_long);
        cudaFree(wlo); cudaFree(whi); cudaFree(wperm);
        sorter.destroy();
    }
};

struct SegScratch {
    uint32_t cap = 0;
    unsigned char *lifted = nullptr, *lifted_sorted = nullptr;
    uint32_t *slotsA = nullptr, *slotsB = nullptr, *posA = nullptr, *posB = nullptr;
    uint32_t *batch_off = nullptr; uint32_t batch_off_cap = 0;
    DevBatch *d_batches = nullptr; uint32_t batch_cap = 0;
    uint32_t *n_total = nullptr;
    uint16_t *h16 = nullptr; uint32_t h16_tiles = 0;
    const unsigned char *lifted_src = nullptr;
    uint32_t *seg_cnt = nullptr;
    Trigger *trig = nullptr; uint32_t *n_trig = nullptr; uint32_t trig_cap = 0;
    uint32_t *n_heavy = nullptr;
    uint32_t *sort_ctl = nullptr;
    unsigned char *res = nullptr; uint64_t *res_ts = nullptr; uint32_t *res_n = nullptr; uint32_t res_cap = 0;
    cudaEvent_t ev_ingest = nullptr, ev_done = nullptr;
    bool pending = false;
    uint32_t nbatches = 0, total = 0;

    void destroy()
    {
        cudaFree(lifted); cudaFree(lifted_sorted); cudaFree(slotsA); cudaFree(slotsB); cudaFree(posA); cudaFree(posB);
        cudaFree(batch_off); cudaFree(d_batches); cudaFree(n_total); cudaFree(seg_cnt); cudaFree(trig); cudaFree(sort_ctl);
        cudaFree(res); cudaFree(res_ts); cudaFree(h16);
        if (ev_ingest) cudaEventDestroy(ev_ingest);
        if (ev_done) cudaEventDestroy(ev_done);
    }
};

struct wfb_ffat {
    int prog = 0;
    const ProgramOps *ops = nullptr;
    std::vector<unsigned char> params;
    const void *pp() const { return params.empty() ? nullptr : params.data(); }
    FfatDev ff{};
    TileScratch ts;
    uint32_t sort_passes = 1;
    SegScratch seg[2];
    RadixSorter sorter;
    bool pipelined = false;
    uint64_t call_no = 0;
    cudaStream_t s2 = nullptr;
    uint64_t launches = 0;
    size_t state_bytes = 0;
    int win_type = 0;
    TbDev tb{};
    wfb_ffat *cb = nullptr;
    uint64_t tb_lateness = 0;
    uint32_t tb_cap = 0, tb_pop_cap = 0;
    uint64_t *tb_kA = nullptr, *tb_kB = nullptr; uint32_t *tb_iA = nullptr, *tb_iB = nullptr;
    unsigned char *tb_lifted = nullptr, *tb_part = nullptr, *tb_popped = nullptr;
    uint32_t *tb_popped_slots = nullptr;
    bool shares_slot_key = false;
    uint32_t *own_n_slots = nullptr;
    uint32_t *tb_head = nullptr, *tb_seg = nullptr, *tb_misc = nullptr;
    GrowCheck growc;
    uint32_t *mg_scratch = nullptr;
    bool append_results = false;
    bool buckets = true;
    uint32_t bucket_shift = 0;
    bool bucket_move = false;
    bool timing = false;
    std::vector<cudaEvent_t> tev;
    uint32_t tev_used = 0;
    static constexpr uint32_t TEV_MAX = 512;
    void mark(int which, cudaStream_t s)
    {
        if (!timing || tev_used >= TEV_MAX) return;
        cudaEventRecord(tev[tev_used * 4 + which], s);
    }
};

extern "C" {

int wfb_abi_version(void) { return WFB_ABI_VERSION; }

const char *wfb_error_string(int code)
{
    switch (code) {
    case 0: return "success";
    case WFB_E_BADARG: return "wfb: bad argument";
    case WFB_E_NOPROG: return "wfb: unknown program id";
    case WFB_E_CAPACITY: return "wfb: capacity exceeded (keys or results)";
    case WFB_E_NOGPU: return "wfb: no CUDA device (libwfb200 has no CPU fallback)";
    case WFB_E_UNSUPPORTED: return "wfb: not supported";
    }
    if (code > 0) return cudaGetErrorString(static_cast<cudaError_t>(code));
    return "wfb: unknown error";
}

int wfb_device_count(void)
{
    int n = 0;
    if (cudaGetDeviceCount(&n) != cudaSuccess) { cudaGetLastError(); return 0; }
    return n;
}

int wfb_program_register(const void *ops, size_t ops_bytes)
{
    if (!ops || ops_bytes != sizeof(ProgramOps)) return WFB_E_BADARG;
    std::lock_guard<std::mutex> lock(registry_mutex());
    std::vector<ProgramOps> &t = registry();
    if (t.size() >= 4096) return WFB_E_CAPACITY;
    t.reserve(4096);
    t.push_back(*static_cast<const ProgramOps *>(ops));
    return static_cast<int>(t.size()) - 1;
}

int wfb_program_info(int prog, wfb_program_info_t *info)
{
    const ProgramOps *o = program(prog);
    if (!o) return WFB_E_NOPROG;
    if (!info) return WFB_E_BADARG;
    info->tuple_bytes = o->tuple_bytes; info->result_bytes = o->result_bytes; info->key_bytes = o->key_bytes; info->key_kind = o->key_kind;
    return 0;
}

int wfb_engine_create(wfb_engine_t **e, int prog)
{
    if (!e) return WFB_E_BADARG;
    const ProgramOps *o = program(prog);
    if (!o) return WFB_E_NOPROG;
    int rc = device_ready(); if (rc) return rc;
    wfb_engine *g = new (std::nothrow) wfb_engine();
    if (!g) return WFB_E_BADARG;
    g->prog = prog; g->ops = o;
    rc = g->ts.init(); if (rc) { delete g; return rc; }
    *e = g;
    return 0;
}

int wfb_engine_destroy(wfb_engine_t *e)
{
    if (!e) return 0;
    cudaDeviceSynchronize();
    e->ts.destroy();
    e->free_sort();
    delete e;
    return 0;
}

uint64_t wfb_engine_launches(const wfb_engine_t *e) { return e ? e->launches : 0; }

int wfb_engine_set_params(wfb_engine_t *e, const void *params, size_t bytes)
{
    if (!e || !params || bytes != e->ops->params_bytes) return WFB_E_BADARG;
    e->params.assign(static_cast<const unsigned char *>(params), static_cast<const unsigned char *>(params) + bytes);
    return 0;
}

static int run_single(wfb_engine_t *e, int mode, const wfb_functors_t *f, const DevBatch &b, cudaStream_t s)
{
    const uint32_t num_tiles = tiles_of(b.n);
    int rc = e->ts.enter(s); if (rc) return rc;
    rc = e->ts.ensure_tiles(num_tiles); if (rc) return rc;
    TileArgs a; std::memset(&a, 0, sizeof(a));
    a.batches = nullptr; a.one = b; a.nbatches = 1; a.num_tiles = num_tiles;
    e->ts.next_launch(a);
    uint32_t grid = 0;
    const uint64_t sb = reinterpret_cast<uint64_t>(b.tuples);
    rc = e->ops->tile_pass(mode, a, f, num_tiles, s, &grid, sb, sb + static_cast<uint64_t>(b.n) * e->ops->tuple_bytes); if (rc) return rc;
    e->ts.launched(num_tiles, grid);
    e->launches++;
    return 0;
}

int wfb_map(wfb_engine_t *e, const wfb_functors_t *f, void *tuples, uint32_t n, void *stream)
{
    if (!e || !f || (!tuples && n)) return WFB_E_BADARG;
    if (n == 0) return 0;
    DevBatch b; std::memset(&b, 0, sizeof(b));
    b.tuples = static_cast<const unsigned char *>(tuples); b.out = static_cast<unsigned char *>(tuples); b.n = n;
    return run_single(e, MODE_MAP, f, b, static_cast<cudaStream_t>(stream));
}

int wfb_map_filter(wfb_engine_t *e, const wfb_functors_t *f, const void *tuples_in, const uint64_t *ts_in, uint32_t n,
                   void *tuples_out, uint64_t *ts_out, uint32_t *n_out_dev, void *stream)
// ... 732 lines not shown
    h->prog = prog; h->ops = o; h->win_type = win_type;
    rc = h->ts.init(); if (rc) { delete h; return rc; }
    FfatDev &ff = h->ff;
    ff.win = win; ff.slide = slide; ff.nb = wins_per_batch;
    ff.B = static_cast<uint64_t>(wins_per_batch - 1) * slide + win;
    const uint64_t pane = gcd_u64(win, slide);
    const uint64_t bp = ff.B / pane;
    if (pane > 0xffffffffull || bp > (1ull << 30)) { delete h; return WFB_E_BADARG; }
    ff.pane = static_cast<uint32_t>(pane); ff.wp = static_cast<uint32_t>(win / pane); ff.sp = static_cast<uint32_t>(slide / pane);
    const uint64_t spare_min = std::min<uint64_t>(bp, 32);
    uint32_t n = 1, lg = 0; while (n < bp + spare_min) { n <<= 1; lg++; }
    ff.n_leaves = n; ff.log_leaves = lg;
    ff.defer_items = (static_cast<uint64_t>(n) - bp + 1) * pane;
    ff.max_keys = max_keys; ff.dense = (flags & WFB_FFAT_DENSE_KEYS) ? 1u : 0u;
    uint32_t cap = 1; while (cap < 2ull * max_keys) cap <<= 1;
    ff.ht_mask = cap - 1;
    const size_t RB = o->result_bytes;
    const size_t tree_bytes = static_cast<size_t>(max_keys) * (2ull * n - 1) * RB;
    size_t total = 0;
#define ALLOC(ptr, bytes) do { cudaError_t e_ = cudaMalloc(reinterpret_cast<void **>(&(ptr)), (bytes)); if (e_ != cudaSuccess) { wfb_ffat_destroy(h); return static_cast<int>(e_); } total += (bytes); } while (0)
    if (!ff.dense) {
        ALLOC(ff.ht_keys, static_cast<size_t>(o->key_bytes) * cap);
        ALLOC(ff.ht_slots, sizeof(uint32_t) * cap);
        CK(cudaMemset(ff.ht_keys, 0xff, static_cast<size_t>(o->key_bytes) * cap));
        CK(cudaMemset(ff.ht_slots, 0xff, sizeof(uint32_t) * cap));
    }
    ALLOC(ff.n_slots, sizeof(uint32_t) * 4);
    h->own_n_slots = ff.n_slots;
    ff.err_flags = ff.n_slots + 1;
    ff.results_total = reinterpret_cast<unsigned long long *>(ff.n_slots + 2);
    CK(cudaMemset(ff.n_slots, 0, sizeof(uint32_t) * 4));
    ALLOC(ff.slot_key, static_cast<size_t>(o->key_bytes) * max_keys);
    ALLOC(ff.cnt, sizeof(uint64_t) * max_keys);
    CK(cudaMemset(ff.cnt, 0, sizeof(uint64_t) * max_keys));
    ALLOC(ff.acc, RB * max_keys);
    CK(cudaMemset(ff.acc, 0, RB * max_keys));
    ALLOC(ff.tree, tree_bytes);
    CK(cudaMemset(ff.tree, 0, tree_bytes));
    ALLOC(ff.seg_off, sizeof(uint32_t) * (static_cast<size_t>(max_keys) + 1));
    CK(cudaMemset(ff.seg_off, 0xff, sizeof(uint32_t) * (static_cast<size_t>(max_keys) + 1)));
    ALLOC(ff.heavy, sizeof(uint32_t) * max_keys);
    ff.light_max = 256;
    h->pipelined = (flags & WFB_FFAT_PIPELINED) != 0;
    for (int p = 0; p < (h->pipelined ? 2 : 1); p++) {
        SegScratch &g = h->seg[p];
        ALLOC(g.seg_cnt, sizeof(uint32_t) * max_keys);
        CK(cudaMemset(g.seg_cnt, 0, sizeof(uint32_t) * max_keys));
        ALLOC(g.n_total, sizeof(uint32_t) * 4);
        CK(cudaMemset(g.n_total, 0, sizeof(uint32_t) * 4));
        g.n_trig = g.n_total + 1; g.res_n = nullptr; g.n_heavy = g.n_total + 3;
        ALLOC(g.sort_ctl, sizeof(uint32_t) * RadixSorter::CTL_WORDS);
        CK(cudaEventCreateWithFlags(&g.ev_ingest, cudaEventDisableTiming));
        CK(cudaEventCreateWithFlags(&g.ev_done, cudaEventDisableTiming));
    }
    if (h->pipelined) CK(cudaStreamCreateWithFlags(&h->s2, cudaStreamNonBlocking));
#undef ALLOC
    if (flags & WFB_KEYS_GROW) { ff.grow = 1; rc = h->growc.init(); if (rc) { wfb_ffat_destroy(h); return rc; } }
    { const char *e = std::getenv("WFB_BUCKET_MOVE"); h->bucket_move = e && std::atoi(e) != 0; }
    ffat_derive_paths(h);
    {
        const bool fits = h->buckets && static_cast<size_t>(2) * ff.n_leaves * RB <= (32u << 10);
        const bool pays = static_cast<uint64_t>(ff.n_leaves) <= 2ull * std::max(1u, ff.log_leaves) * ff.sp * ff.nb;
        ff.lazy = (fits && pays) ? 1u : 0u;
    }
    h->state_bytes = total;
    *hh = h;
    return 0;
}

int wfb_ffat_destroy(wfb_ffat_t *h)
{
    if (!h) return 0;
    cudaDeviceSynchronize();
    FfatDev &ff = h->ff;
    cudaFree(ff.ht_keys); cudaFree(ff.ht_slots); cudaFree(h->own_n_slots); if (!h->shares_slot_key) cudaFree(ff.slot_key); cudaFree(ff.cnt);
    cudaFree(ff.acc); cudaFree(ff.tree); cudaFree(ff.seg_off); cudaFree(ff.heavy); cudaFree(h->mg_scratch);
    for (int p = 0; p < 2; p++) h->seg[p].destroy();
    h->sorter.destroy();
    if (h->cb) wfb_ffat_destroy(h->cb);
    cudaFree(h->tb.first); cudaFree(h->tb.num); cudaFree(h->tb.num_new); cudaFree(h->tb.trig); cudaFree(h->tb.done); cudaFree(h->tb.ring);
    cudaFree(h->tb.present); cudaFree(h->tb.cnt); cudaFree(h->tb_misc);
    cudaFree(h->tb_kA); cudaFree(h->tb_kB); cudaFree(h->tb_iA); cudaFree(h->tb_iB); cudaFree(h->tb_lifted); cudaFree(h->tb_part);
    cudaFree(h->tb_popped); cudaFree(h->tb_popped_slots); cudaFree(h->tb_head); cudaFree(h->tb_seg);
    if (h->s2) cudaStreamDestroy(h->s2);
    for (auto &e : h->tev) cudaEventDestroy(e);
    h->ts.destroy(); h->growc.destroy();
    delete h;
    cudaGetLastError();
    return 0;
}

uint64_t wfb_ffat_launches(const wfb_ffat_t *h) { return h ? h->launches : 0; }

int wfb_ffat_set_params(wfb_ffat_t *h, const void *params, size_t bytes)
{
    if (!h || !params || bytes != h->ops->params_bytes) return WFB_E_BADARG;
    h->params.assign(static_cast<const unsigned char *>(params), static_cast<const unsigned char *>(params) + bytes);
    if (h->cb) h->cb->params = h->params;
    return 0;
}
uint64_t wfb_ffat_state_bytes(const wfb_ffat_t *h) { return h ? h->state_bytes : 0; }
uint32_t wfb_ffat_key_capacity(const wfb_ffat_t *h) { return h ? h->ff.max_keys : 0; }
int wfb_ffat_set_key_shard(wfb_ffat_t *h, uint32_t num_shards, uint32_t shard)
{
    if (!h || num_shards == 0 || shard >= num_shards || !h->ff.dense || h->call_no != 0) return WFB_E_BADARG;
    if (h->win_type == 1) {
        if (h->cb == nullptr || h->cb->call_no != 0) return WFB_E_BADARG;
        h->cb->ff.key_div = num_shards; h->cb->ff.key_rem = shard;
    }
    h->ff.key_div = num_shards; h->ff.key_rem = shard;
    return 0;
}

static double host_now_us() { timespec t; clock_gettime(CLOCK_MONOTONIC, &t); return t.tv_sec * 1e6 + t.tv_nsec * 1e-3; }
static int ffat_ensure_segment(wfb_ffat *h, SegScratch &g, uint32_t total, uint32_t nbatches, cudaStream_t s)
{
    if (total > g.cap) {
        CK(cudaStreamSynchronize(s));
        if (h->s2) CK(cudaStreamSynchronize(h->s2));
        cudaFree(g.lifted); cudaFree(g.lifted_sorted); cudaFree(g.slotsA); cudaFree(g.slotsB); cudaFree(g.posA); cudaFree(g.posB);
        cudaFree(g.trig); cudaFree(g.res); cudaFree(g.res_ts);
        g.cap = std::max(total, 2 * g.cap);
        const size_t RB = h->ops->result_bytes;
        CK(cudaMalloc(&g.lifted, static_cast<size_t>(g.cap) * RB));
        if (h->bucket_move) CK(cudaMalloc(&g.lifted_sorted, static_cast<size_t>(g.cap) * RB));
        CK(cudaMalloc(&g.slotsA, sizeof(uint32_t) * g.cap)); CK(cudaMalloc(&g.slotsB, sizeof(uint32_t) * g.cap));
        CK(cudaMalloc(&g.posA, sizeof(uint32_t) * g.cap)); CK(cudaMalloc(&g.posB, sizeof(uint32_t) * g.cap));
        g.trig_cap = ffat_trig_cap(h, g.cap, h->ff.max_keys);
        CK(cudaMalloc(&g.trig, sizeof(Trigger) * g.trig_cap));
        if (h->pipelined) {
            g.res_cap = static_cast<uint32_t>(std::min<uint64_t>(static_cast<uint64_t>(g.trig_cap) * h->ff.nb, 0x7fffffffull));
            CK(cudaMalloc(&g.res, static_cast<size_t>(g.res_cap) * RB));
            CK(cudaMalloc(&g.res_ts, sizeof(uint64_t) * g.res_cap));
            g.res_n = g.n_total + 2;
        }
    }
    if (nbatches + 1 > g.batch_off_cap) {
        CK(cudaStreamSynchronize(s));
        if (h->s2) CK(cudaStreamSynchronize(h->s2));
        cudaFree(g.batch_off); cudaFree(g.d_batches);
        g.batch_off_cap = std::max(nbatches + 1, 2 * g.batch_off_cap);
        CK(cudaMalloc(&g.batch_off, sizeof(uint32_t) * g.batch_off_cap));
        CK(cudaMalloc(&g.d_batches, sizeof(DevBatch) * g.batch_off_cap));
    }
    return 0;
}

static int ffat_window_phase(wfb_ffat *h, SegScratch &g, const FfatDev &ff, unsigned char *out, uint64_t *out_ts, uint32_t out_cap,
                             uint32_t *n_out, cudaStream_t s)
{
    const uint32_t *sorted_slots, *sorted_pos;
    const uint64_t before = h->sorter.launches;
    int rc;
    if (h->buckets) {
        const uint32_t *counts = nullptr;
        rc = h->sorter.sort_wide<uint32_t>(g.slotsA, g.slotsB, g.posB, nullptr, g.total, g.total, h->bucket_shift, s, g.sort_ctl, &counts,
                                           h->bucket_move ? g.lifted : nullptr, h->bucket_move ? g.lifted_sorted : nullptr,
                                           static_cast<uint32_t>(h->ops->result_bytes), true, 0, 0, h->pipelined ? g.h16 : nullptr);
        if (rc) return rc;
        h->launches += h->sorter.launches - before;
        h->mark(2, s);
        rc = h->ops->ffat_buckets(ff, h->bucket_move ? g.lifted_sorted : g.lifted_src, g.slotsB, g.posB, counts, h->bucket_shift, h->bucket_move ? 1u : 0u, g.batch_off, g.d_batches, g.nbatches, out, out_ts,
                                  out_cap, n_out, s, h->pp());
        if (rc) return rc;
        h->launches += 1;
    } else {
        rc = h->sorter.sort<uint32_t>(g.slotsA, g.slotsB, g.posA, g.posB, g.n_total, 0, g.total, h->sort_passes, s, &sorted_slots,
                                      &sorted_pos, g.sort_ctl, ff.seg_off, ff.max_keys);
        if (rc) return rc;
        h->launches += h->sorter.launches - before;
        h->mark(2, s);
        uint32_t ugrid = std::max(1u, std::min((ff.max_keys + 7) / 8, static_cast<uint32_t>(g_num_sms) * 8u));
        rc = h->ops->ffat_update(ff, g.lifted, sorted_pos, g.batch_off, g.d_batches, g.nbatches, out, out_ts, out_cap, n_out, ugrid, s, h->pp(),
                                 std::max(1u, std::min((ff.max_keys + 127u) / 128u, static_cast<uint32_t>(g_num_sms) * 16u)));
        if (rc) return rc;
        h->launches += 2;
    }
    rc = h->ops->ffat_windows(ff, g.batch_off, g.d_batches, g.nbatches, out, out_ts, out_cap, static_cast<uint32_t>(g_num_sms) * 4u, s, h->pp(), n_out);
    if (rc) return rc;
    h->launches += 1;
    return 0;
}

static int ffat_deliver(wfb_ffat *h, SegScratch &g, unsigned char *out, uint64_t *out_ts, uint32_t out_cap, uint32_t *n_out, cudaStream_t s)
{
    if (!g.pending) { CK(cudaMemsetAsync(n_out, 0, sizeof(uint32_t), s)); return 0; }
    CK(cudaStreamWaitEvent(s, g.ev_done, 0));
    k_copy_results<<<static_cast<uint32_t>(g_num_sms) * 2u, 256, 0, s>>>(g.res, g.res_ts, g.res_n, h->ops->result_bytes, out, out_ts,
                                                                          out_cap, n_out, h->ff.err_flags);
    CK(cudaGetLastError());
    h->launches++;
    g.pending = false;
    return 0;
}

int wfb_ffat_process_cb(wfb_ffat_t *h, const wfb_functors_t *pre, const wfb_batch_t *batches_h, uint32_t nbatches,
                        void *out_results, uint64_t *out_ts, uint32_t out_capacity, uint32_t *n_out_dev, void *stream)
{
    return ffat_process_cb_impl(h, pre, batches_h, nbatches, out_results, out_ts, out_capacity, n_out_dev, stream, nullptr);
}

static int ffat_process_cb_impl(wfb_ffat_t *h, const void *pre, const wfb_batch_t *batches_h, uint32_t nbatches,
                                void *out_results, uint64_t *out_ts, uint32_t out_capacity, uint32_t *n_out_dev, void *stream,
                                const uint32_t *ext_slots)
{
    if (!h || !n_out_dev || (nbatches && !batches_h) || (out_capacity && !out_results)) return WFB_E_BADARG;
    if (h->win_type != 0) return WFB_E_BADARG;
    cudaStream_t s = static_cast<cudaStream_t>(stream);
    int rc = h->ts.enter(s); if (rc) return rc;
    unsigned char *out = static_cast<unsigned char *>(out_results);
    const uint32_t par = h->pipelined ? static_cast<uint32_t>(h->call_no & 1u) : 0u;
    SegScratch &g = h->seg[par];
    SegScratch &prev = h->seg[h->pipelined ? (par ^ 1u) : 0u];

    std::vector<DevBatch> hb;
    hb.reserve(nbatches);
    uint64_t total = 0; uint32_t tiles = 0;
    uint64_t span_begin = ~0ull, span_end = 0;
    for (uint32_t i = 0; i < nbatches; i++) {
        if (batches_h[i].n == 0) continue;
        if (!batches_h[i].tuples) return WFB_E_BADARG;
        DevBatch b; std::memset(&b, 0, sizeof(b));
        b.tuples = static_cast<const unsigned char *>(batches_h[i].tuples); b.ts = batches_h[i].ts;
        b.watermark = batches_h[i].watermark; b.n = batches_h[i].n; b.tile_begin = tiles;
        tiles += tiles_of(b.n); total += b.n;
        const uint64_t p0 = reinterpret_cast<uint64_t>(b.tuples);
        span_begin = std::min(span_begin, p0); span_end = std::max(span_end, p0 + static_cast<uint64_t>(b.n) * h->ops->tuple_bytes);
        hb.push_back(b);
    }
    if (total > 0x7fffffffull) return WFB_E_BADARG;
    if (total == 0) {
        if (h->pipelined) return ffat_deliver(h, prev, out, out_ts, out_capacity, n_out_dev, s);
        if (!h->append_results) CK(cudaMemsetAsync(n_out_dev, 0, sizeof(uint32_t), s));
        return 0;
    }
    nbatches = static_cast<uint32_t>(hb.size());
    FfatDev ff;
    const auto ingest = [&]() -> int {
        const bool sparse = h->buckets;
        const uint64_t seg_cap = sparse ? static_cast<uint64_t>(tiles) * TILE : total;
        if (seg_cap > 0x7fffffffull) return WFB_E_BADARG;
        rc = ffat_ensure_segment(h, g, static_cast<uint32_t>(seg_cap), nbatches, s); if (rc) return rc;
        rc = h->ts.ensure_tiles(tiles); if (rc) return rc;
        { int rc_ = h->ts.stage.h2d(g.d_batches, hb.data(), sizeof(DevBatch) * nbatches, s); if (rc_) return rc_; }
        g.nbatches = nbatches; g.total = static_cast<uint32_t>(seg_cap);
        if (sparse) {
            std::vector<uint32_t> boff(nbatches + 1);
            for (uint32_t i = 0; i < nbatches; i++) boff[i] = hb[i].tile_begin * TILE;
            boff[nbatches] = tiles * TILE;
            { int rc_ = h->ts.stage.h2d(g.batch_off, boff.data(), sizeof(uint32_t) * (nbatches + 1), s); if (rc_) return rc_; }
        }

        ff = h->ff;
        ff.seg_cnt = g.seg_cnt; ff.trig = g.trig; ff.n_trig = g.n_trig; ff.trig_cap = g.trig_cap; ff.n_heavy = g.n_heavy;

        const uint32_t npasses = h->buckets ? 1u : h->sort_passes;
        rc = h->buckets ? RadixSorter::prepare_wide(g.sort_ctl, s) : RadixSorter::prepare(g.sort_ctl, npasses, s); if (rc) return rc;
        h->mark(0, s);
        TileArgs a; std::memset(&a, 0, sizeof(a));
        a.sort_ctl = g.sort_ctl; a.sort_passes = npasses; a.sort_shift = h->buckets ? h->bucket_shift : 0u; a.sort_dbits = h->buckets ? OSW_BITS : 8u;
        a.batches = g.d_batches; a.nbatches = nbatches; a.num_tiles = tiles;
        a.lifted = g.lifted; a.slots = g.slotsA; a.batch_off = g.batch_off; a.n_total = g.n_total; a.ff = ff;
        g.lifted_src = g.lifted;
        if (sparse && !h->pipelined && !h->bucket_move && (h->ops->reserved & 1u)) {
            const unsigned char *base = hb[0].tuples;
            bool ok = (reinterpret_cast<uintptr_t>(base) & 15u) == 0;
            for (uint32_t i = 0; ok && i < nbatches; i++) ok = hb[i].tuples == base + static_cast<size_t>(hb[i].tile_begin) * TILE * h->ops->tuple_bytes;
            if (ok) { a.inplace = 1; g.lifted_src = base; a.ext_slots = ext_slots; }
        }
        if (ext_slots != nullptr && !a.inplace) {
            if (sparse) return WFB_E_UNSUPPORTED;
            if (nbatches != 1 || !(h->ops->reserved & 1u)) return WFB_E_BADARG;
            a.ext_slots = ext_slots;
        }
        h->ts.next_launch(a);
        a.max_ctas_per_sm = h->pipelined ? 2u : 0u;
        a.l2_hints = 1;
        a.sparse = sparse ? 1u : 0u;
        a.count_keys = h->buckets ? 0u : 1u;
        uint32_t claims = tiles;
        if (sparse) {
            if (h->pipelined && (g.total + OSW_TILE - 1) / OSW_TILE > h->sorter.wide_tiles) CK(cudaStreamSynchronize(h->s2));
            rc = h->sorter.ensure_wide(g.total, s, &a.wide_h16); if (rc) return rc;
            if (h->pipelined) {
                const uint32_t wt = (g.total + OSW_TILE - 1) / OSW_TILE;
                if (wt > g.h16_tiles) {
                    CK(cudaStreamSynchronize(s)); CK(cudaStreamSynchronize(h->s2));
                    cudaFree(g.h16);
                    g.h16_tiles = std::max(wt, 2 * g.h16_tiles);
                    CK(cudaMalloc(&g.h16, sizeof(uint16_t) * OSW_DIGITS * g.h16_tiles));
                }
                a.wide_h16 = g.h16;
            }
            a.tiles_per_ticket = OSW_TILE_POS / TILE;
            a.sort_ctl = nullptr;
            a.pack_rank = 1;
            claims = (tiles + a.tiles_per_ticket - 1) / a.tiles_per_ticket;
        }
        if (a.inplace && h->ops->slots_inplace) {
            rc = h->ops->slots_inplace(a, pre ? static_cast<const void *>(pre) : h->pp(), s); if (rc) return rc;
        } else {
            uint32_t grid = 0;
            rc = h->ops->tile_pass(MODE_INGEST, a, pre ? static_cast<const void *>(pre) : h->pp(), claims, s, &grid, span_begin, span_end); if (rc) return rc;
            h->ts.launched(claims, grid);
        }
        h->launches++;
        h->mark(1, s);
        return 0;
    };
    rc = ingest(); if (rc) return rc;
    for (bool grew = h->ff.grow != 0; grew; ) {
        rc = ffat_grow(h, s, &grew); if (rc) return rc;
        if (grew) { rc = ingest(); if (rc) return rc; h->launches++; }
    }

    if (!h->pipelined) {
        if (!h->append_results) CK(cudaMemsetAsync(n_out_dev, 0, sizeof(uint32_t), s));
        rc = ffat_window_phase(h, g, ff, out, out_ts, out_capacity, n_out_dev, s); if (rc) return rc;
        h->mark(3, s);
    } else {
        CK(cudaEventRecord(g.ev_ingest, s));
        rc = ffat_deliver(h, prev, out, out_ts, out_capacity, n_out_dev, s); if (rc) return rc;
        CK(cudaStreamWaitEvent(h->s2, g.ev_ingest, 0));
        CK(cudaMemsetAsync(g.res_n, 0, sizeof(uint32_t), h->s2));
        rc = ffat_window_phase(h, g, ff, g.res, g.res_ts, g.res_cap, g.res_n, h->s2); if (rc) return rc;
        h->mark(3, h->s2);
        CK(cudaEventRecord(g.ev_done, h->s2));
        g.pending = true;
    }
    if (h->timing && h->tev_used < wfb_ffat::TEV_MAX) h->tev_used++;
    h->call_no++;
    return 0;
}

static int ffat_process_prebucketed(wfb_ffat *h, const unsigned char *records, const uint32_t *recv_slots, const uint32_t *bins, uint32_t nsrc,
                                    uint32_t bps, const uint32_t *offs_h, const uint64_t *wms_h, uint32_t slot_mask, uint32_t shift,
                                    void *out_results, uint64_t *out_ts, uint32_t out_capacity, uint32_t *n_out_dev, cudaStream_t s, bool append, uint32_t items)
{
    if (!h || !n_out_dev || nsrc == 0 || nsrc > MAX_SHARDS || bps == 0 || bps > OSW_DIGITS || (1u << shift) > BK_KEYS) return WFB_E_BADARG;
    if (h->win_type != 0 || h->pipelined || !h->buckets) return WFB_E_UNSUPPORTED;
    int rc = h->ts.enter(s); if (rc) return rc;
    SegScratch &g = h->seg[0];
    const uint32_t total = items;
    if (!append) CK(cudaMemsetAsync(n_out_dev, 0, sizeof(uint32_t), s));
    if (total == 0) return 0;
    rc = ffat_ensure_segment(h, g, total, nsrc, s); if (rc) return rc;
    std::vector<DevBatch> hb(nsrc);
    for (uint32_t i = 0; i < nsrc; i++) {
        std::memset(&hb[i], 0, sizeof(DevBatch));
        hb[i].tuples = records + static_cast<size_t>(offs_h[i]) * h->ops->result_bytes; hb[i].n = offs_h[i + 1] - offs_h[i]; hb[i].watermark = wms_h[i];
    }
    { int rc_ = h->ts.stage.h2d(g.d_batches, hb.data(), sizeof(DevBatch) * nsrc, s); if (rc_) return rc_; }
    { int rc_ = h->ts.stage.h2d(g.batch_off, offs_h, sizeof(uint32_t) * (nsrc + 1), s); if (rc_) return rc_; }
    g.nbatches = nsrc; g.total = total; g.lifted_src = records;
    FfatDev ff = h->ff;
    ff.seg_cnt = g.seg_cnt; ff.trig = g.trig; ff.n_trig = g.n_trig; ff.trig_cap = g.trig_cap; ff.n_heavy = g.n_heavy;
    rc = RadixSorter::prepare_wide(g.sort_ctl, s); if (rc) return rc;
    h->mark(0, s); h->mark(1, s);
    MgRuns runs;
    for (uint32_t i = 0; i <= MAX_SHARDS; i++) runs.off[i] = offs_h[std::min(i, nsrc)];
    uint32_t nsub = 1, shift2 = shift;
    while (nsub * 2 * bps <= OSW_DIGITS && nsub * 2 <= MAX_SHARDS && shift2 > 0) { nsub *= 2; shift2--; }
    if (!h->mg_scratch) CK(cudaMalloc(&h->mg_scratch, sizeof(uint32_t) * 3 * OSW_DIGITS * MAX_SHARDS));
    uint32_t *cnt3 = h->mg_scratch, *off3 = cnt3 + OSW_DIGITS * MAX_SHARDS, *run_starts = off3 + OSW_DIGITS * MAX_SHARDS;
    const dim3 grid(bps, nsrc);
    k_mg_count<<<grid, MG_THREADS, 0, s>>>(bins, nsrc, bps, runs, recv_slots, slot_mask, shift2, nsub, cnt3, run_starts, g.n_trig, g.n_heavy);
    k_mg_scan<<<1, 1024, 0, s>>>(cnt3, bps * nsub * nsrc, nsrc, off3, g.sort_ctl);
    k_mg_split<<<grid, MG_THREADS, 0, s>>>(bins, nsrc, bps, runs, recv_slots, slot_mask, shift2, nsub, off3, run_starts, g.slotsB, g.posB);
    CK(cudaGetLastError());
    h->mark(2, s);
    rc = h->ops->ffat_buckets(ff, records, g.slotsB, g.posB, g.sort_ctl, shift2, 0u, g.batch_off, g.d_batches, nsrc, static_cast<unsigned char *>(out_results), out_ts,
                              out_capacity, n_out_dev, s, h->pp());
    if (rc) return rc;
    rc = h->ops->ffat_windows(ff, g.batch_off, g.d_batches, nsrc, static_cast<unsigned char *>(out_results), out_ts, out_capacity, static_cast<uint32_t>(g_num_sms) * 4u, s,
                              h->pp(), n_out_dev);
    if (rc) return rc;
    h->mark(3, s);
    h->launches += 5;
    if (h->timing && h->tev_used < wfb_ffat::TEV_MAX) h->tev_used++;
    h->call_no++;
    return 0;
}

int wfb_ffat_flush(wfb_ffat_t *h, void *out_results, uint64_t *out_ts, uint32_t out_capacity, uint32_t *n_out_dev, void *stream)
{
    if (!h || !n_out_dev || (out_capacity && !out_results)) return WFB_E_BADARG;
    cudaStream_t s = static_cast<cudaStream_t>(stream);
    if (!h->pipelined) { CK(cudaMemsetAsync(n_out_dev, 0, sizeof(uint32_t), s)); return 0; }
    int rc = h->ts.enter(s); if (rc) return rc;
    SegScratch &last = h->seg[(h->call_no + 1) & 1u];
    return ffat_deliver(h, last, static_cast<unsigned char *>(out_results), out_ts, out_capacity, n_out_dev, s);
}

int wfb_ffat_timing(wfb_ffat_t *h, int enable, float *ms_h, uint32_t *calls_h)
{
    if (!h) return WFB_E_BADARG;
    float acc[4] = {0, 0, 0, 0};
    if (h->tev_used) {
        CK(cudaEventSynchronize(h->tev[(h->tev_used - 1) * 4 + 3]));
        for (uint32_t i = 0; i < h->tev_used; i++) {
            float a = 0, b = 0, c = 0, d = 0;
            cudaEvent_t *e = &h->tev[i * 4];
            CK(cudaEventElapsedTime(&a, e[0], e[1]));
            CK(cudaEventElapsedTime(&b, e[1], e[2]));
            CK(cudaEventElapsedTime(&c, e[2], e[3]));
            CK(cudaEventElapsedTime(&d, e[0], e[3]));
            acc[0] += a; acc[1] += b; acc[2] += c; acc[3] += d;
        }
    }
    if (ms_h) for (int i = 0; i < 4; i++) ms_h[i] = acc[i];
    if (calls_h) *calls_h = h->tev_used;
    h->tev_used = 0;
    if (enable && h->tev.empty()) {
        h->tev.resize(wfb_ffat::TEV_MAX * 4);
        for (auto &e : h->tev) CK(cudaEventCreate(&e));
    }
    h->timing = enable != 0;
    return 0;
}

int wfb_ffat_stats(wfb_ffat_t *h, uint32_t *n_keys_h, uint32_t *err_flags_h, void *stream)
{
    if (!h) return WFB_E_BADARG;
    uint32_t v[2] = {0, 0};
    if (h->s2) CK(cudaStreamSynchronize(h->s2));
    CK(cudaMemcpyAsync(v, h->ff.n_slots, sizeof(v), cudaMemcpyDeviceToHost, static_cast<cudaStream_t>(stream)));
    CK(cudaStreamSynchronize(static_cast<cudaStream_t>(stream)));
    if (n_keys_h) *n_keys_h = v[0];
    if (err_flags_h) *err_flags_h = v[1];
    if (h->cb && err_flags_h) { uint32_t e2 = 0; int rc = wfb_ffat_stats(h->cb, nullptr, &e2, stream); if (rc) return rc; *err_flags_h |= e2; }
    return 0;
}

int wfb_ffat_results_total(wfb_ffat_t *h, uint64_t *total_h, void *stream)
{
    if (!h || !total_h) return WFB_E_BADARG;
    const wfb_ffat *src = h->cb ? h->cb : h;
    unsigned long long v = 0;
    if (src->s2) CK(cudaStreamSynchronize(src->s2));
    if (src->ff.results_total == nullptr) { *total_h = 0; return 0; }
    CK(cudaMemcpyAsync(&v, src->ff.results_total, sizeof(v), cudaMemcpyDeviceToHost, static_cast<cudaStream_t>(stream)));
    CK(cudaStreamSynchronize(static_cast<cudaStream_t>(stream)));
    *total_h = v;
    return 0;
}

}
#include <dlfcn.h>
namespace {
struct Nccl {
    struct Id { char b[128]; };
    typedef int (*GetUniqueId_t)(void *);
    typedef int (*CommInitRank_t)(void **, int, Id, int);
    typedef int (*CommDestroy_t)(void *);
    typedef int (*SendRecv_t)(void *, size_t, int, int, void *, cudaStream_t);
    typedef int (*Group_t)();
    typedef const char *(*ErrStr_t)(int);
    void *lib = nullptr;
    GetUniqueId_t GetUniqueId = nullptr; CommInitRank_t CommInitRank = nullptr; CommDestroy_t CommDestroy = nullptr;
    SendRecv_t Send = nullptr, Recv = nullptr; Group_t GroupStart = nullptr, GroupEnd = nullptr;
    bool ok = false;
    Nccl()
    {
        const char *names[] = {std::getenv("WFB_NCCL_LIB"), "libnccl.so.2", "libnccl.so"};
        for (const char *n : names) { if (n && (lib = dlopen(n, RTLD_NOW | RTLD_GLOBAL))) break; }
        if (!lib) return;
        GetUniqueId = reinterpret_cast<GetUniqueId_t>(dlsym(lib, "ncclGetUniqueId"));
        CommInitRank = reinterpret_cast<CommInitRank_t>(dlsym(lib, "ncclCommInitRank"));
        CommDestroy = reinterpret_cast<CommDestroy_t>(dlsym(lib, "ncclCommDestroy"));
        Send = reinterpret_cast<SendRecv_t>(dlsym(lib, "ncclSend")); Recv = reinterpret_cast<SendRecv_t>(dlsym(lib, "ncclRecv"));
        GroupStart = reinterpret_cast<Group_t>(dlsym(lib, "ncclGroupStart")); GroupEnd = reinterpret_cast<Group_t>(dlsym(lib, "ncclGroupEnd"));
        ok = GetUniqueId && CommInitRank && CommDestroy && Send && Recv && GroupStart && GroupEnd;
    }
};
Nccl &nccl() { static Nccl n; return n; }
constexpr int NCCL_UINT8 = 1;
#define NK(call) do { int r__ = (call); if (r__ != 0) return 1000 + r__; } while (0)

__global__ void k_mg_meta(const uint32_t *__restrict__ counts, uint64_t watermark, uint32_t nranks, uint64_t *__restrict__ send_meta)
{
    const uint32_t d = threadIdx.x;
    if (d < nranks) { send_meta[2 * d] = counts[d]; send_meta[2 * d + 1] = watermark; }
}

__global__ void k_mg_pre_append(unsigned long long *results_total, const uint32_t *n_out) { if (results_total) *results_total -= *n_out; }

struct MgSlot {
    unsigned char *regions = nullptr; uint32_t region_cap = 0;
    uint32_t *vslots = nullptr;
    uint32_t *bins = nullptr;
    uint32_t *recv_slots = nullptr, *recv_bins = nullptr; size_t recv_slots_cap = 0;
    unsigned char *ce_buf = nullptr;
    unsigned char *peer[MAX_SHARDS] = {};
    uint32_t offs[MAX_SHARDS + 1] = {}; uint64_t wms[MAX_SHARDS] = {};
    uint32_t *counts = nullptr;
    uint64_t *send_meta = nullptr, *recv_meta = nullptr;
    uint32_t *h_counts = nullptr; uint64_t *h_recv = nullptr;
    unsigned char *recv = nullptr; size_t recv_bytes = 0;
    cudaEvent_t ev_src = nullptr, ev_meta = nullptr, ev_a2a = nullptr, ev_done = nullptr, ev_self = nullptr, ev_fork = nullptr;
    bool used = false, done_recorded = false, exchanged = false;
    cudaEvent_t tr[8] = {}; bool tr_valid = false;
};
}

struct wfb_mg {
    int nranks = 1, rank = 0;
    void *comm = nullptr;
    wfb_engine_t *eng = nullptr;
    wfb_ffat_t *ffat = nullptr;
    size_t rb = 0;
    MgSlot slot[4];
    cudaStream_t cs = nullptr;
    cudaStream_t cs2 = nullptr;
    uint64_t step_no = 0;
    MgSlot *pend[3] = {nullptr, nullptr, nullptr}; int npend = 0;
    std::vector<wfb_batch_t> chunks;
    bool ce = false, ce_tried = false; uint64_t ce_cap = 0, peer_cap[MAX_SHARDS] = {};
    unsigned char *ce_msg = nullptr;
    cudaEvent_t ev_flush = nullptr;
    static constexpr int CE_STREAMS = 4;
    cudaStream_t ce_s[CE_STREAMS] = {}; cudaEvent_t ce_ev[CE_STREAMS] = {};
    uint32_t *tok = nullptr;
    cudaEvent_t last_done = nullptr;
    double host_acc[3] = {}; uint64_t host_n = 0;
// ... 509 lines not shown
```

Before: 15.07 billion.

## Build per-wide-tile digit cells in tile pass and skip the separate wide sort

The ingest tile pass now lays out each 4096-position wide tile into digit-ordered cells in shared memory and writes a per-digit cell descriptor table. The bucket-update kernel reads slots directly through these cells using a binary search over cell starts, so the separate radix sort_wide launches before the bucket kernel are no longer needed. This removes the global sort passes and their extra memory traffic, at the cost of more shared memory per tile-pass block, extra barriers inside the consumer warps, and a per-element binary search in the bucket kernel. The tile pass also gains a minimum-blocks launch bound.

```diff
diff --git a/windflow_b200/csrc/wfb_kernels.cuh b/windflow_b200/csrc/wfb_kernels.cuh
--- a/windflow_b200/csrc/wfb_kernels.cuh
+++ b/windflow_b200/csrc/wfb_kernels.cuh
@@ -18,6 +18,8 @@
 
 constexpr int TILE = 256;
 constexpr uint32_t OSW_TILE_POS = 4096;
+constexpr uint32_t OSW_BITS = 10, OSW_DIGITS = 1u << OSW_BITS;
+constexpr uint32_t CELLS_MAX_WIDE = 2048;
 #ifndef WFB_STAGES
 #define WFB_STAGES 4
 #endif
@@ -99,6 +101,8 @@
     uint16_t *wide_h16;
     uint32_t tiles_per_ticket;
     uint32_t pack_rank;
+    uint32_t *cells;
+    uint32_t cells_stride;
     const uint32_t *ext_slots;
     uint32_t inplace;
     uint32_t l2_hints;
@@ -305,6 +309,7 @@
 }
 
 constexpr uint32_t TP_THREADS = TILE + 64;
+constexpr uint32_t TP_MINBLOCKS = 3;
 constexpr uint32_t TILE_SENTINEL = 0x7fffffffu;
 enum { TF_SWZ = 1u, TF_FALLBACK = 2u, TF_TS_SMEM = 4u, TF_WIDE_LAST = 8u };
 
@@ -323,6 +328,8 @@
     static constexpr uint32_t stage_bytes = tile_bytes + aux_bytes;
     static constexpr uint32_t hist_bytes = (MODE == MODE_INGEST) ? 4u * 256u * 4u : 0u;
     static constexpr uint32_t total = STAGES * stage_bytes + 1024  + 1024  + hist_bytes;
+    static constexpr uint32_t cell_lpos = OSW_TILE_POS + OSW_DIGITS;
+    static constexpr uint32_t cells_bytes = (MODE == MODE_INGEST) ? OSW_TILE_POS * 4u + cell_lpos * 2u + OSW_DIGITS * 4u + 32u : 0u;
 };
 
 __device__ __forceinline__ void mbar_arrive(uint64_t *bar)
@@ -346,8 +353,74 @@
 }
 __device__ __forceinline__ void consumer_bar() { asm volatile("bar.sync 1, %0;" ::"n"(TILE) : "memory"); }
 
+__device__ __forceinline__ uint32_t cell_entries_below(const uint16_t *cell16, uint32_t cnt, uint32_t mine)
+{
+    const uint32_t mm = (mine | (mine << 16)) + 0x7fff7fffu;
+    const uint32_t *cell = reinterpret_cast<const uint32_t *>(cell16);
+    uint32_t less = 0;
+    for (uint32_t j = 0; j < cnt; j += 2) less += __popc((mm - cell[j >> 1]) & 0x80008000u);
+    return less;
+}
+
+__device__ __forceinline__ void wide_cells_layout(const TileArgs &a, uint32_t wide, uint32_t lim, uint32_t *row, const uint32_t *sw,
+                                                  uint16_t *lpos, uint32_t *cstart, uint32_t *wsum, uint32_t ctid)
+{
+    constexpr uint32_t LPOS = OSW_TILE_POS + OSW_DIGITS;
+    constexpr uint32_t LPAD = 0x0fffu;
+    constexpr uint32_t NW = TILE / 32;
+    static_assert(TILE * 4 == OSW_DIGITS && LPOS % (2 * TILE) == 0 && OSW_TILE_POS == 16 * TILE, "layout");
+    const uint32_t lane = ctid & 31u, warp = ctid >> 5;
+    consumer_bar();
+    const uint2 cw = reinterpret_cast<const uint2 *>(row)[ctid];
+    const uint32_t c0 = cw.x & 0xffffu, c1 = cw.x >> 16, c2 = cw.y & 0xffffu, c3 = cw.y >> 16;
+    const uint32_t p0 = ((c0 + 1u) & ~1u) | (c0 << 16), p1 = ((c1 + 1u) & ~1u) | (c1 << 16);
+    const uint32_t p2 = ((c2 + 1u) & ~1u) | (c2 << 16), p3 = ((c3 + 1u) & ~1u) | (c3 << 16);
+    const uint32_t sum = p0 + p1 + p2 + p3;
+    uint32_t incl = sum;
+#pragma unroll
+    for (int o = 1; o < 32; o <<= 1) { const uint32_t v = __shfl_up_sync(FULL, incl, o); if (lane >= static_cast<uint32_t>(o)) incl += v; }
+    if (lane == 31) wsum[warp] = incl;
+#pragma unroll
+    for (uint32_t i = 0; i < LPOS / (2 * TILE); i++) reinterpret_cast<uint32_t *>(lpos)[i * TILE + ctid] = LPAD | (LPAD << 16);
+    consumer_bar();
+    uint32_t base = incl - sum;
+#pragma unroll
+    for (uint32_t q = 0; q < NW; q++) if (q < warp) base += wsum[q];
+    const uint32_t s0 = base, s1 = s0 + p0, s2 = s1 + p1, s3 = s2 + p2;
+    reinterpret_cast<uint4 *>(cstart)[ctid] = make_uint4(s0, s1, s2, s3);
+    uint32_t *col = a.cells + wide + static_cast<size_t>(4u * ctid) * a.cells_stride;
+    col[0] = (s0 >> 16) | (c0 << 16);
+    col[a.cells_stride] = (s1 >> 16) | (c1 << 16);
+    col[2u * a.cells_stride] = (s2 >> 16) | (c2 << 16);
+    col[3u * a.cells_stride] = (s3 >> 16) | (c3 << 16);
+    consumer_bar();
+#pragma unroll 4
+    for (uint32_t r = 0; r < OSW_TILE_POS / TILE; r++) {
+        const uint32_t i = r * TILE + ctid;
+        if (i < lim) {
+            const uint32_t w = sw[i];
+            if (w != INVALID_SLOT) lpos[(cstart[((w & 0xffffu) >> a.sort_shift) & (OSW_DIGITS - 1u)] & 0xffffu) + (w >> 16)] = static_cast<uint16_t>(i);
+        }
+    }
+    consumer_bar();
+    uint32_t *region = a.slots + static_cast<size_t>(wide) * OSW_TILE_POS;
+#pragma unroll 2
+    for (uint32_t e = ctid; e < LPOS; e += TILE) {
+        const uint32_t mine = lpos[e];
+        if (mine >= lim) continue;
+        const uint32_t w = sw[mine];
+        if (w == INVALID_SLOT) continue;
+        const uint32_t slot = w & 0xffffu, d = (slot >> a.sort_shift) & (OSW_DIGITS - 1u);
+        const uint32_t cs = cstart[d], start = cs & 0xffffu, cnt = (row[d >> 1] >> ((d & 1u) * 16u)) & 0xffffu;
+        if (e - start >= cnt) continue;
+        region[(cs >> 16) + cell_entries_below(lpos + start, cnt, mine)] = slot | (mine << 16);
+    }
+    consumer_bar();
+    reinterpret_cast<uint2 *>(row)[ctid] = make_uint2(0, 0);
+}
+
 template <class P, int MODE>
-__global__ void __launch_bounds__(TP_THREADS) k_tile_pass(const __grid_constant__ CUtensorMap tmap, const TileArgs a,
+__global__ void __launch_bounds__(TP_THREADS, TP_MINBLOCKS) k_tile_pass(const __grid_constant__ CUtensorMap tmap, const TileArgs a,
                                                           const __grid_constant__ typename P::params_t prm)
 {
     using T = typename P::tuple_t;
@@ -367,6 +440,11 @@
     StageMeta *meta = reinterpret_cast<StageMeta *>(empty + STAGES);
     uint32_t *warp_tot = reinterpret_cast<uint32_t *>(meta + STAGES);
     uint32_t *s_hist = reinterpret_cast<uint32_t *>(ctl + 1024);
+    uint32_t *c_words = reinterpret_cast<uint32_t *>(ctl + 1024 + SM::hist_bytes);
+    uint16_t *c_lpos = reinterpret_cast<uint16_t *>(c_words + OSW_TILE_POS);
+    uint32_t *c_start = reinterpret_cast<uint32_t *>(c_lpos + SM::cell_lpos);
+    uint32_t *c_wsum = c_start + OSW_DIGITS;
+    const bool wide = a.wide_h16 != nullptr || a.cells != nullptr;
 
     const uint32_t tid = threadIdx.x, lane = tid & 31, warp = tid >> 5;
     auto stage_buf = [&](uint32_t s) { return smem + s * SM::stage_bytes; };
@@ -489,7 +567,7 @@
                         else slot = slot_of_key(a.ff, key_words<P>(tup, prm));
                         if (slot != INVALID_SLOT && a.count_keys) atomicAdd(&a.ff.seg_cnt[slot], 1u);
                     }
-                    if (a.wide_h16 != nullptr) {
+                    if (wide) {
                         if (slot != INVALID_SLOT) {
                             const uint32_t d = (slot >> a.sort_shift) & 1023u;
                             const uint32_t before = atomicAdd(&s_hist[wpar * 512u + (d >> 1)], 1u << ((d & 1u) * 16u));
@@ -546,9 +624,17 @@
                         reinterpret_cast<uint32_t *>(stage_aux(s))[ctid] = slot;
                     } else {
                         TileIO<R>::store(buf, local, res);
-                        reinterpret_cast<uint32_t *>(stage_aux(s))[local] = slot;
+                        if (MODE == MODE_INGEST && a.cells != nullptr) c_words[(m.tile & 15u) * TILE + local] = slot;
+                        else reinterpret_cast<uint32_t *>(stage_aux(s))[local] = slot;
                     }
                 } else if (MODE == MODE_INGEST && a.inplace) reinterpret_cast<uint32_t *>(stage_aux(s))[ctid] = INVALID_SLOT;
+                if (MODE == MODE_INGEST && a.cells != nullptr) {
+                    if (ctid >= total) c_words[(m.tile & 15u) * TILE + ctid] = INVALID_SLOT;
+                    if (m.flags & TF_WIDE_LAST) {
+                        wide_cells_layout(a, m.wide, ((m.tile & 15u) + 1u) * TILE, s_hist + wpar * 512u, c_words, c_lpos, c_start, c_wsum, ctid);
+                        wpar ^= 1u;
+                    }
+                }
             }
             fence_async_smem();
             __syncwarp();
@@ -631,7 +717,8 @@
             }
             if constexpr (MODE == MODE_INGEST) {
                 const uint32_t *ssl = reinterpret_cast<const uint32_t *>(stage_aux(s));
-                if (a.sparse) for (uint32_t i = lane; i < TILE; i += 32) a.slots[excl + i] = i < (a.inplace ? m.cnt : tile_count) ? ssl[i] : INVALID_SLOT;
+                if (a.cells != nullptr) { }
+                else if (a.sparse) for (uint32_t i = lane; i < TILE; i += 32) a.slots[excl + i] = i < (a.inplace ? m.cnt : tile_count) ? ssl[i] : INVALID_SLOT;
                 else for (uint32_t i = lane; i < tile_count; i += 32) a.slots[excl + i] = ssl[i];
             }
             __syncwarp();
@@ -900,7 +987,6 @@
 #ifndef WFB_OSW_MINBLOCKS
 #define WFB_OSW_MINBLOCKS 5
 #endif
-constexpr uint32_t OSW_BITS = 10, OSW_DIGITS = 1u << OSW_BITS;
 constexpr uint32_t OSW_THREADS = 256, OSW_ITEMS = 16, OSW_TILE = OSW_THREADS * OSW_ITEMS;
 static_assert(OSW_TILE == OSW_TILE_POS, "the tile pass files its digit counts per wide tile");
 
@@ -1072,11 +1158,7 @@
         const uint32_t slot = w & 0xffffu, d = (slot >> shift) & (OSW_DIGITS - 1u);
         const uint32_t cs = cell_start[d], cnt = cnt_row[d];
         if (e - cs >= cnt) continue;
-        const uint32_t mm = (mine | (mine << 16)) + 0x7fff7fffu;
-        const uint32_t *cell = reinterpret_cast<const uint32_t *>(lpos + cs);
-        uint32_t less = 0;
-        for (uint32_t j = 0; j < cnt; j += 2) less += __popc((mm - cell[j >> 1]) & 0x80008000u);
-        const uint32_t dst = bin_base[d] + less;
+        const uint32_t dst = bin_base[d] + cell_entries_below(lpos + cs, cnt, mine);
         keys_out[dst] = slot;
         if (RBYTES == 0 || vals_out != nullptr) vals_out[dst] = start + mine;
         if constexpr (RBYTES != 0) {
@@ -1559,10 +1641,14 @@
 #define WFB_BK_MINBLOCKS_LAZY 4
 #endif
 
-template <class P, bool LAZY>
+constexpr uint32_t BK_CELL_PT = CELLS_MAX_WIDE / BK_THREADS;
+__host__ __device__ constexpr uint32_t bk_cells_smem(uint32_t nwide) { return (nwide + 1u) * 4u + ((nwide * 2u + 15u) & ~15u); }
+
+template <class P, bool LAZY, bool CELLS>
 __global__ void __launch_bounds__(BK_THREADS, LAZY ? WFB_BK_MINBLOCKS_LAZY : WFB_BK_MINBLOCKS) k_ffat_update_buckets(const FfatDev ff, const unsigned char *__restrict__ lifted,
                                                                        const uint32_t *__restrict__ bk_slots, const uint32_t *__restrict__ bk_pos,
-                                                                       const uint32_t *__restrict__ digit_counts, uint32_t shift, uint32_t moved,
+                                                                       const uint32_t *__restrict__ digit_counts, const uint32_t *__restrict__ cells,
+                                                                       uint32_t cells_stride, uint32_t nwide, uint32_t shift, uint32_t moved,
                                                                        const uint32_t *__restrict__ batch_off, const DevBatch *__restrict__ batches,
                                                                        uint32_t nbatches, unsigned char *__restrict__ out_res,
                                                                        uint64_t *__restrict__ out_ts, uint32_t out_cap, uint32_t *__restrict__ n_out,
@@ -1593,6 +1679,9 @@
     __shared__ uint32_t ksegb[BK_KEYS];
     __shared__ uint32_t seg_desc[BK_THREADS];
     __shared__ uint32_t misc[NW], s_boff[2], s_nheavy, s_hnext, s_nseg;
+    extern __shared__ __align__(16) uint32_t bk_cell_smem[];
+    uint32_t *s_cstart = bk_cell_smem;
+    uint16_t *s_coff = reinterpret_cast<uint16_t *>(bk_cell_smem + nwide + 1);
 
     const uint32_t tid = threadIdx.x, lane = tid & 31, warp = tid >> 5;
     const uint32_t bucket = blockIdx.x;
@@ -1615,7 +1704,34 @@
         for (uint32_t q = 0; q < RB / CPB; q++) cp_async<CPB>(kacc + tid * RB + q * CPB, ff.acc + static_cast<size_t>(slot) * RB + q * CPB);
     }
     if (tid < BK_KEYS) kleft[tid] = 0;
-    {
+    if constexpr (CELLS) {
+        static_assert(BK_CELL_PT % 4 == 0, "uint4 loads");
+        const uint32_t c0 = tid * BK_CELL_PT;
+        const uint4 *col = reinterpret_cast<const uint4 *>(cells + static_cast<size_t>(bucket) * cells_stride + c0);
+        uint32_t dsc[BK_CELL_PT];
+#pragma unroll
+        for (uint32_t q = 0; q < BK_CELL_PT / 4; q++) {
+            uint4 v = make_uint4(0, 0, 0, 0);
+            if (c0 + 4 * q < nwide) v = col[q];
+            dsc[4 * q] = v.x; dsc[4 * q + 1] = v.y; dsc[4 * q + 2] = v.z; dsc[4 * q + 3] = v.w;
+        }
+        uint32_t sum = 0;
+#pragma unroll
+        for (uint32_t q = 0; q < BK_CELL_PT; q++) { if (c0 + q >= nwide) dsc[q] = 0; sum += dsc[q] >> 16; }
+        uint32_t incl = sum;
+#pragma unroll
+        for (int o = 1; o < 32; o <<= 1) { const uint32_t v = __shfl_up_sync(FULL, incl, o); if (lane >= static_cast<uint32_t>(o)) incl += v; }
+        if (lane == 31) misc[warp] = incl;
+        __syncthreads();
+        uint32_t run = incl - sum;
+#pragma unroll
+        for (uint32_t w = 0; w < NW; w++) if (w < warp) run += misc[w];
+#pragma unroll
+        for (uint32_t q = 0; q < BK_CELL_PT; q++)
+            if (c0 + q < nwide) { s_cstart[c0 + q] = run; s_coff[c0 + q] = static_cast<uint16_t>(dsc[q] & 0xffffu); run += dsc[q] >> 16; }
+        if (tid == BK_THREADS - 1) { s_cstart[nwide] = run; s_boff[0] = 0; s_boff[1] = run; }
+        __syncthreads();
+    } else {
         uint32_t cc[DPT];
 #pragma unroll
         for (uint32_t q = 0; q < DPT / 4; q++) {
@@ -1639,13 +1755,26 @@
         __syncthreads();
     }
     const uint32_t bbeg = s_boff[0], bend = s_boff[1];
+    const auto cell_of = [&](uint32_t j) {
+        uint32_t c = 0;
+#pragma unroll
+        for (uint32_t b = CELLS_MAX_WIDE / 2; b; b >>= 1) if (c + b < nwide && s_cstart[c + b] <= j) c += b;
+        return c;
+    };
+    const auto word_of = [&](uint32_t j, uint32_t c) { return bk_slots + static_cast<size_t>(c) * OSW_TILE_POS + s_coff[c] + (j - s_cstart[c]); };
     const auto fetch_list = [&](uint32_t at, uint32_t end) {
 #pragma unroll
         for (uint32_t r = 0; r < IT; r++) {
             const uint32_t i = r * BK_THREADS + tid;
             if (at + i < end) {
-                cp_async<4>(s_lslot + i, bk_slots + at + i);
-                if (!moved) cp_async<4>(s_lpos + i, bk_pos + at + i);
+                if constexpr (CELLS) {
+                    const uint32_t c = cell_of(at + i);
+                    cp_async<4>(s_lslot + i, word_of(at + i, c));
+                    s_lpos[i] = c;
+                } else {
+                    cp_async<4>(s_lslot + i, bk_slots + at + i);
+                    if (!moved) cp_async<4>(s_lpos + i, bk_pos + at + i);
+                }
             }
         }
     };
@@ -1655,7 +1784,8 @@
 #pragma unroll
         for (uint32_t q = 0; q < BK_CNT_U; q++) {
             const uint32_t i = base + q * BK_THREADS + tid;
-            lk[q] = i < bend ? bk_slots[i] - key_lo : 0xffffffffu;
+            if constexpr (CELLS) lk[q] = i < bend ? (*word_of(i, cell_of(i)) & 0xffffu) - key_lo : 0xffffffffu;
+            else lk[q] = i < bend ? bk_slots[i] - key_lo : 0xffffffffu;
         }
 #pragma unroll
         for (uint32_t q = 0; q < BK_CNT_U; q++) if (lk[q] < kpc) atomicAdd(&kleft[lk[q]], 1u);
@@ -1689,8 +1819,10 @@
             const uint32_t i = r * BK_THREADS + tid;
             ek[r] = BK_KEYS; ep[r] = cursor + i;
             if (i < nsel) {
-                const uint32_t lk = s_lslot[i] - key_lo;
-                if (!moved) ep[r] = s_lpos[i];
+                uint32_t sl = s_lslot[i];
+                if constexpr (CELLS) { ep[r] = s_lpos[i] * OSW_TILE_POS + (sl >> 16); sl &= 0xffffu; }
+                else if (!moved) ep[r] = s_lpos[i];
+                const uint32_t lk = sl - key_lo;
                 if (lk < kpc) ek[r] = lk;
             }
         }
diff --git a/windflow_b200/csrc/wfb_launch.cuh b/windflow_b200/csrc/wfb_launch.cuh
--- a/windflow_b200/csrc/wfb_launch.cuh
+++ b/windflow_b200/csrc/wfb_launch.cuh
@@ -60,7 +60,8 @@
                        const DevBatch *batches, uint32_t nbatches, unsigned char *out_res, uint64_t *out_ts,
                        uint32_t out_cap, uint32_t *n_out, uint32_t grid, cudaStream_t s, const void *params, uint32_t lanes_grid);
     int (*ffat_buckets)(const FfatDev &ff, const unsigned char *lifted, const uint32_t *bk_slots, const uint32_t *bk_pos,
-                        const uint32_t *digit_counts, uint32_t shift, uint32_t moved, const uint32_t *batch_off, const DevBatch *batches,
+                        const uint32_t *digit_counts, const uint32_t *cells, uint32_t cells_stride, uint32_t nwide,
+                        uint32_t shift, uint32_t moved, const uint32_t *batch_off, const DevBatch *batches,
                         uint32_t nbatches, unsigned char *out_res, uint64_t *out_ts, uint32_t out_cap, uint32_t *n_out, cudaStream_t s,
                         const void *params);
     int (*ffat_windows)(const FfatDev &ff, const uint32_t *batch_off, const DevBatch *batches, uint32_t nbatches,
@@ -119,16 +120,18 @@
 int launch_tile_pass(TileArgs &a, const void *params, uint32_t want_grid, cudaStream_t s, uint32_t *grid_used,
                      uint64_t span_begin, uint64_t span_end)
 {
-    static int max_grid = -1;
-    constexpr uint32_t smem = TilePassSmem<P, MODE>::total;
-    if (max_grid < 0) {
-        WFB_CK(cudaFuncSetAttribute(k_tile_pass<P, MODE>, cudaFuncAttributeMaxDynamicSharedMemorySize, static_cast<int>(smem)));
+    static int max_grid[2] = {-1, -1};
+    using SM = TilePassSmem<P, MODE>;
+    const uint32_t cells = a.cells != nullptr ? 1u : 0u;
+    const uint32_t smem = SM::total + (cells ? SM::cells_bytes : 0u);
+    if (max_grid[cells] < 0) {
+        WFB_CK(cudaFuncSetAttribute(k_tile_pass<P, MODE>, cudaFuncAttributeMaxDynamicSharedMemorySize, static_cast<int>(SM::total + SM::cells_bytes)));
         int per_sm = 0;
         WFB_CK(cudaOccupancyMaxActiveBlocksPerMultiprocessor(&per_sm, k_tile_pass<P, MODE>, TP_THREADS, smem));
         if (per_sm < 1) per_sm = 1;
-        max_grid = per_sm * wfb::num_sms();
+        max_grid[cells] = per_sm * wfb::num_sms();
     }
-    uint32_t grid = std::max(1u, std::min(want_grid, static_cast<uint32_t>(max_grid)));
+    uint32_t grid = std::max(1u, std::min(want_grid, static_cast<uint32_t>(max_grid[cells])));
     if (a.max_ctas_per_sm) grid = std::max(1u, std::min(grid, a.max_ctas_per_sm * static_cast<uint32_t>(wfb::num_sms())));
     const typename P::params_t prm = load_params<P>(params);
     alignas(64) CUtensorMap tmap;
@@ -168,14 +171,29 @@
 
 template <class P>
 int ffat_buckets_dispatch(const FfatDev &ff, const unsigned char *lifted, const uint32_t *bk_slots, const uint32_t *bk_pos,
-                          const uint32_t *digit_counts, uint32_t shift, uint32_t moved, const uint32_t *batch_off, const DevBatch *batches,
+                          const uint32_t *digit_counts, const uint32_t *cells, uint32_t cells_stride, uint32_t nwide,
+                          uint32_t shift, uint32_t moved, const uint32_t *batch_off, const DevBatch *batches,
                           uint32_t nbatches, unsigned char *out_res, uint64_t *out_ts, uint32_t out_cap, uint32_t *n_out, cudaStream_t s,
                           const void *params)
 {
-    if (ff.lazy) k_ffat_update_buckets<P, true><<<OSW_DIGITS, BK_THREADS, 0, s>>>(ff, lifted, bk_slots, bk_pos, digit_counts, shift, moved, batch_off, batches,
-                                                                                 nbatches, out_res, out_ts, out_cap, n_out, load_params<P>(params));
-    else k_ffat_update_buckets<P, false><<<OSW_DIGITS, BK_THREADS, 0, s>>>(ff, lifted, bk_slots, bk_pos, digit_counts, shift, moved, batch_off, batches,
-                                                                          nbatches, out_res, out_ts, out_cap, n_out, load_params<P>(params));
+    const typename P::params_t prm = load_params<P>(params);
+    if (cells != nullptr) {
+        if (nwide == 0 || nwide > CELLS_MAX_WIDE || moved) return WFB_E_BADARG;
+        static bool attr = false;
+        if (!attr) {
+            WFB_CK(cudaFuncSetAttribute(k_ffat_update_buckets<P, true, true>, cudaFuncAttributeMaxDynamicSharedMemorySize, static_cast<int>(bk_cells_smem(CELLS_MAX_WIDE))));
+            WFB_CK(cudaFuncSetAttribute(k_ffat_update_buckets<P, false, true>, cudaFuncAttributeMaxDynamicSharedMemorySize, static_cast<int>(bk_cells_smem(CELLS_MAX_WIDE))));
+            attr = true;
+        }
+        const uint32_t dyn = bk_cells_smem(nwide);
+        if (ff.lazy) k_ffat_update_buckets<P, true, true><<<OSW_DIGITS, BK_THREADS, dyn, s>>>(ff, lifted, bk_slots, nullptr, nullptr, cells, cells_stride, nwide, shift, 0u,
+                                                                                            batch_off, batches, nbatches, out_res, out_ts, out_cap, n_out, prm);
+        else k_ffat_update_buckets<P, false, true><<<OSW_DIGITS, BK_THREADS, dyn, s>>>(ff, lifted, bk_slots, nullptr, nullptr, cells, cells_stride, nwide, shift, 0u,
+                                                                                      batch_off, batches, nbatches, out_res, out_ts, out_cap, n_out, prm);
+    } else if (ff.lazy) k_ffat_update_buckets<P, true, false><<<OSW_DIGITS, BK_THREADS, 0, s>>>(ff, lifted, bk_slots, bk_pos, digit_counts, nullptr, 0u, 0u, shift, moved,
+                                                                                           batch_off, batches, nbatches, out_res, out_ts, out_cap, n_out, prm);
+    else k_ffat_update_buckets<P, false, false><<<OSW_DIGITS, BK_THREADS, 0, s>>>(ff, lifted, bk_slots, bk_pos, digit_counts, nullptr, 0u, 0u, shift, moved,
+                                                                                 batch_off, batches, nbatches, out_res, out_ts, out_cap, n_out, prm);
     WFB_CK(cudaGetLastError());
     return 0;
 }
diff --git a/windflow_b200/csrc/wfb_lib.cu b/windflow_b200/csrc/wfb_lib.cu
--- a/windflow_b200/csrc/wfb_lib.cu
+++ b/windflow_b200/csrc/wfb_lib.cu
@@ -462,6 +462,8 @@
     DevBatch *d_batches = nullptr; uint32_t batch_cap = 0;
     uint32_t *n_total = nullptr;
     uint16_t *h16 = nullptr; uint32_t h16_tiles = 0;
+    uint32_t *cells = nullptr; uint32_t cells_cap = 0;
+    uint32_t cells_stride = 0, nwide = 0;
     const unsigned char *lifted_src = nullptr;
     uint32_t *seg_cnt = nullptr;
     Trigger *trig = nullptr; uint32_t *n_trig = nullptr; uint32_t trig_cap = 0;
@@ -476,7 +478,7 @@
     {
         cudaFree(lifted); cudaFree(lifted_sorted); cudaFree(slotsA); cudaFree(slotsB); cudaFree(posA); cudaFree(posB);
         cudaFree(batch_off); cudaFree(d_batches); cudaFree(n_total); cudaFree(seg_cnt); cudaFree(trig); cudaFree(sort_ctl);
-        cudaFree(res); cudaFree(res_ts); cudaFree(h16);
+        cudaFree(res); cudaFree(res_ts); cudaFree(h16); cudaFree(cells);
         if (ev_ingest) cudaEventDestroy(ev_ingest);
         if (ev_done) cudaEventDestroy(ev_done);
     }
@@ -1515,7 +1517,13 @@
     const uint32_t *sorted_slots, *sorted_pos;
     const uint64_t before = h->sorter.launches;
     int rc;
-    if (h->buckets) {
+    if (h->buckets && g.nwide != 0) {
+        h->mark(2, s);
+        rc = h->ops->ffat_buckets(ff, g.lifted_src, g.slotsA, nullptr, nullptr, g.cells, g.cells_stride, g.nwide, h->bucket_shift, 0u, g.batch_off, g.d_batches,
+                                  g.nbatches, out, out_ts, out_cap, n_out, s, h->pp());
+        if (rc) return rc;
+        h->launches += 1;
+    } else if (h->buckets) {
         const uint32_t *counts = nullptr;
         rc = h->sorter.sort_wide<uint32_t>(g.slotsA, g.slotsB, g.posB, nullptr, g.total, g.total, h->bucket_shift, s, g.sort_ctl, &counts,
                                            h->bucket_move ? g.lifted : nullptr, h->bucket_move ? g.lifted_sorted : nullptr,
@@ -1523,7 +1531,7 @@
         if (rc) return rc;
         h->launches += h->sorter.launches - before;
         h->mark(2, s);
-        rc = h->ops->ffat_buckets(ff, h->bucket_move ? g.lifted_sorted : g.lifted_src, g.slotsB, g.posB, counts, h->bucket_shift, h->bucket_move ? 1u : 0u, g.batch_off, g.d_batches, g.nbatches, out, out_ts,
+        rc = h->ops->ffat_buckets(ff, h->bucket_move ? g.lifted_sorted : g.lifted_src, g.slotsB, g.posB, counts, nullptr, 0u, 0u, h->bucket_shift, h->bucket_move ? 1u : 0u, g.batch_off, g.d_batches, g.nbatches, out, out_ts,
                                   out_cap, n_out, s, h->pp());
         if (rc) return rc;
         h->launches += 1;
@@ -1642,7 +1650,23 @@
         a.sparse = sparse ? 1u : 0u;
         a.count_keys = h->buckets ? 0u : 1u;
         uint32_t claims = tiles;
-        if (sparse) {
+        const uint32_t nwide = (g.total + OSW_TILE - 1) / OSW_TILE;
+        g.nwide = (sparse && !h->bucket_move && !a.inplace && nwide <= CELLS_MAX_WIDE) ? nwide : 0u;
+        if (g.nwide != 0) {
+            const uint32_t stride = (nwide + 15u) & ~15u;
+            if (OSW_DIGITS * stride > g.cells_cap) {
+                CK(cudaStreamSynchronize(s)); if (h->s2) CK(cudaStreamSynchronize(h->s2));
+                cudaFree(g.cells);
+                g.cells_cap = OSW_DIGITS * stride;
+                CK(cudaMalloc(&g.cells, sizeof(uint32_t) * g.cells_cap));
+            }
+            g.cells_stride = stride;
+            a.cells = g.cells; a.cells_stride = stride;
+            a.tiles_per_ticket = OSW_TILE_POS / TILE;
+            a.sort_ctl = nullptr;
+            a.pack_rank = 1;
+            claims = nwide;
+        } else if (sparse) {
             if (h->pipelined && (g.total + OSW_TILE - 1) / OSW_TILE > h->sorter.wide_tiles) CK(cudaStreamSynchronize(h->s2));
             rc = h->sorter.ensure_wide(g.total, s, &a.wide_h16); if (rc) return rc;
             if (h->pipelined) {
@@ -1732,7 +1756,7 @@
     k_mg_split<<<grid, MG_THREADS, 0, s>>>(bins, nsrc, bps, runs, recv_slots, slot_mask, shift2, nsub, off3, run_starts, g.slotsB, g.posB);
     CK(cudaGetLastError());
     h->mark(2, s);
-    rc = h->ops->ffat_buckets(ff, records, g.slotsB, g.posB, g.sort_ctl, shift2, 0u, g.batch_off, g.d_batches, nsrc, static_cast<unsigned char *>(out_results), out_ts,
+    rc = h->ops->ffat_buckets(ff, records, g.slotsB, g.posB, g.sort_ctl, nullptr, 0u, 0u, shift2, 0u, g.batch_off, g.d_batches, nsrc, static_cast<unsigned char *>(out_results), out_ts,
                               out_capacity, n_out_dev, s, h->pp());
     if (rc) return rc;
     rc = h->ops->ffat_windows(ff, g.batch_off, g.d_batches, nsrc, static_cast<unsigned char *>(out_results), out_ts, out_capacity, static_cast<uint32_t>(g_num_sms) * 4u, s,
```

Result: faster. 16.26 billion, median of 6 (+7.8%).
